# MarcoPolo/drand

Hardware: AMD Instinct MI355X
Metric: verified beacons/sec (whole node), quicknet G1 scheme (higher is better)
Workload: dtype u32 (Fp products on 14x28-bit limbs, 64-bit MAD accumulators; 12x32-bit Montgomery storage); 1 GPU; bls-unchained-g1-rfc9380 batch verify of a 1048576-round chain, 1048576 rounds per GPU; scheme=bls-unchained-g1-rfc9380, rounds_total=1048576, rounds_per_gpu=1048576, global_batch=1048576, parallelism=round-shard x1

## Files before the change

drand_amd/_lib.py:

```python
import ctypes
import os

HERE = os.path.dirname(os.path.abspath(__file__))
LIB_PATH = os.environ.get("DRANDHIP_LIB") or os.path.join(HERE, "libdrandhip.so")

DH_OK = 0
DH_EINVAL = -1
DH_EDEVICE = -2
DH_ENOMEM = -3
DH_EKEY = -4
DH_ERECOVER = -5
DH_EBUSY = -6
DH_EABANDONED = -7
DH_ECORRUPT = -8
DH_ENOBEACON = -9
DH_NODE_CHECKED = 2
DH_DEFERRED = 1
DH_STORE_TRIMMED, DH_STORE_UNTRIMMED, DH_STORE_AUTO = 0, 1, 2

_c = ctypes
_P = _c.c_void_p
SIGNATURES = {
    "dh_init": (_c.c_int, [_c.c_uint32]),
    "dh_shutdown": (None, []),
    "dh_scheme_from_name": (_c.c_int, [_c.c_char_p]),
    "dh_sig_len": (_c.c_int, [_c.c_int]),
    "dh_key_len": (_c.c_int, [_c.c_int]),
    "dh_verify_batch": (_c.c_int, [_c.c_int, _c.c_char_p, _c.c_size_t, _P, _P, _c.c_size_t, _P, _c.c_size_t, _P,
                                   _c.c_size_t, _P, _P, _c.c_uint64]),
    "dh_verify_batch_device": (_c.c_int, [_c.c_int, _c.c_char_p, _c.c_size_t, _P, _P, _c.c_size_t, _P, _c.c_size_t,
                                          _P, _c.c_size_t, _P, _P, _c.c_uint64, _P, _P]),
    "dh_verify_beacon": (_c.c_int, [_c.c_int, _c.c_char_p, _c.c_size_t, _c.c_uint64, _c.c_char_p, _c.c_size_t,
                                    _c.c_char_p, _c.c_size_t]),
    "dh_verify_recovered": (_c.c_int, [_c.c_int, _c.c_char_p, _c.c_size_t, _c.c_char_p, _c.c_char_p, _c.c_size_t]),
    "dh_verify_recovered_batch": (_c.c_int, [_c.c_int, _c.c_char_p, _c.c_size_t, _P, _P, _c.c_size_t, _c.c_size_t, _P,
                                             _c.c_uint64]),
    "dh_digest_batch": (_c.c_int, [_c.c_int, _P, _P, _c.c_size_t, _P, _c.c_size_t, _P]),
    "dh_randomness_batch": (_c.c_int, [_c.c_int, _P, _c.c_size_t, _c.c_size_t, _P]),
    "dh_recover_batch": (_c.c_int, [_c.c_int, _c.c_char_p, _c.c_int, _c.c_int, _P, _P, _P, _c.c_size_t, _P, _P]),
    "dh_verify_partials_batch": (_c.c_int, [_c.c_int, _c.c_char_p, _c.c_int, _c.c_int, _P, _P, _P, _c.c_size_t, _P]),
    "dh_bls_verify_batch": (_c.c_int, [_c.c_int, _P, _c.c_size_t, _P, _P, _P, _P, _c.c_size_t, _c.c_size_t, _P, _P,
                                       _c.c_uint64, _P]),
    "dh_identity_hash_batch": (_c.c_int, [_c.c_int, _P, _c.c_size_t, _P]),
    "dh_identity_verify_batch": (_c.c_int, [_c.c_int, _P, _P, _c.c_size_t, _c.c_size_t, _P]),
    "dh_schnorr_verify_batch": (_c.c_int, [_c.c_int, _P, _c.c_size_t, _P, _P, _P, _P, _c.c_size_t, _c.c_size_t, _P, _P]),
    "dh_schnorr_sig_len": (_c.c_int, [_c.c_int]),
    "dh_sign_batch": (_c.c_int, [_c.c_int, _c.c_char_p, _P, _P, _c.c_size_t, _P, _c.c_size_t, _P]),
    "dh_public_key": (_c.c_int, [_c.c_int, _c.c_char_p, _P]),
    "dh_partial_bytes": (_c.c_int, [_c.c_int]),
    "dh_set_split": (_c.c_int, [_c.c_uint64, _c.c_int]),
    "dh_hash_to_curve": (_c.c_int, [_c.c_int, _P, _P, _c.c_size_t, _c.c_char_p, _c.c_size_t, _P]),
    "dh_g1_round_prep_debug": (_c.c_int, [_P, _P, _c.c_size_t, _P, _P, _P]),
    "dh_batch_begin": (_c.c_int, [_c.c_int, _c.c_char_p, _c.c_size_t, _P, _P, _c.c_size_t, _P, _c.c_size_t, _P,
                                  _c.c_size_t, _P, _P, _c.c_uint64, _P, _c.POINTER(_P), _P]),
    "dh_batch_check": (_c.c_int, [_P, _P, _c.c_size_t, _P]),
    "dh_batch_stream": (_P, [_P]),
    "dh_check_partials": (_c.c_int, [_c.c_int, _c.c_char_p, _c.c_size_t, _P, _c.c_size_t, _c.POINTER(_c.c_int)]),
    "dh_batch_finish": (_c.c_int, [_P, _c.c_int, _P]),
    "dh_bolt_index": (_c.c_int, [_P, _c.c_size_t, _P, _P, _c.c_size_t, _P]),
    "dh_store_open_bolt": (_c.c_int, [_P, _c.c_size_t, _c.POINTER(_P)]),
    "dh_store_stat": (_c.c_int, [_P, _P]),
    "dh_store_columns_device": (_c.c_int, [_P, _c.c_uint64, _c.c_uint64, _c.c_size_t, _P, _P, _P, _c.c_size_t, _P, _P,
                                           _c.c_size_t, _P, _P]),
    "dh_store_check_past": (_c.c_int, [_P, _c.c_int, _c.c_char_p, _c.c_size_t, _c.c_uint64, _c.c_size_t, _c.c_uint64, _P,
                                       _c.c_size_t, _P, _P, _P]),
    "dh_store_close": (None, [_P]),
    "dh_store_open_bolt_format": (_c.c_int, [_P, _c.c_size_t, _c.c_int, _c.POINTER(_P)]),
    "dh_store_format_stat": (_c.c_int, [_P, _P]),
    "dh_store_beacons_device": (_c.c_int, [_P, _c.c_uint64, _c.c_uint64, _c.c_size_t, _c.c_size_t, _P, _P, _P, _P, _P, _P,
                                           _c.c_size_t, _P, _P, _c.c_size_t, _P, _P]),
    "dh_store_deferred": (_c.c_int, [_P, _c.c_uint64, _c.c_uint64, _P, _c.c_size_t, _P]),
    "dh_profile": (_c.c_int, [_c.c_int]),
    "dh_profile_read": (_c.c_int, [_c.c_char_p, _c.c_size_t]),
    "dh_last_error_string": (_c.c_char_p, []),
    "dh_version": (_c.c_char_p, []),
}

_lib = None


class LibraryMissing(RuntimeError):
    pass


def load():
    global _lib
    if _lib is not None:
        return _lib
    if not os.path.exists(LIB_PATH):
        raise LibraryMissing(
            "libdrandhip.so not found at %s: build it with `make -C drand_amd` or __graft_entry__.build()" % LIB_PATH)
    lib = ctypes.CDLL(LIB_PATH)
    for name, (res, args) in SIGNATURES.items():
        fn = getattr(lib, name)
        fn.restype = res
        fn.argtypes = args
    _lib = lib
    return lib


def last_error():
    return (load().dh_last_error_string() or b"").decode()
```

drand_amd/csrc/drandhip.cpp:

```cpp
#include <hip/hip_runtime.h>
#include <stdarg.h>
#include <stdio.h>
#include <string.h>
#include <sys/random.h>

#include <algorithm>
#include <atomic>
#include <condition_variable>
#include <cmath>
#include <functional>
#include <map>
#include <memory>
#include <chrono>
#include <mutex>
#include <string>
#include <thread>
#include <vector>

#include "../../include/drandhip.h"
#include "bolt.hpp"
#include "kernels.hpp"

namespace {

// ... 356 lines not shown
    v[12] ^= (uint64_t)done;
    if (last) v[14] = ~v[14];
    for (int r = 0; r < 12; r++) {
      const uint8_t* s = sigma[r];
      auto G = [&](int a, int b, int c, int d, uint64_t x, uint64_t y) {
        v[a] = v[a] + v[b] + x; v[d] = ror(v[d] ^ v[a], 32);
        v[c] = v[c] + v[d];     v[b] = ror(v[b] ^ v[c], 24);
        v[a] = v[a] + v[b] + y; v[d] = ror(v[d] ^ v[a], 16);
        v[c] = v[c] + v[d];     v[b] = ror(v[b] ^ v[c], 63);
      };
      G(0, 4, 8, 12, m[s[0]], m[s[1]]);
      G(1, 5, 9, 13, m[s[2]], m[s[3]]);
      G(2, 6, 10, 14, m[s[4]], m[s[5]]);
      G(3, 7, 11, 15, m[s[6]], m[s[7]]);
      G(0, 5, 10, 15, m[s[8]], m[s[9]]);
      G(1, 6, 11, 12, m[s[10]], m[s[11]]);
      G(2, 7, 8, 13, m[s[12]], m[s[13]]);
      G(3, 4, 9, 14, m[s[14]], m[s[15]]);
    }
    for (int i = 0; i < 8; i++) h[i] ^= v[i] ^ v[i + 8];
  }
  for (int i = 0; i < 32; i++) out[i] = (uint8_t)(h[i / 8] >> (8 * (i % 8)));
}

uint64_t splitmix64(uint64_t& x) {
  uint64_t z = (x += 0x9e3779b97f4a7c15ULL);
  z = (z ^ (z >> 30)) * 0xbf58476d1ce4e5b9ULL;
  z = (z ^ (z >> 27)) * 0x94d049bb133111ebULL;
  return z ^ (z >> 31);
}

int make_seed(uint64_t seed, uint32_t words[8]) {
  if (seed == 0) {
    uint8_t b[32];
    size_t got = 0;
    while (got < sizeof b) {
      ssize_t r = getrandom(b + got, sizeof b - got, 0);
      if (r <= 0) return fail(DH_EDEVICE, "getrandom failed");
      got += (size_t)r;
    }
    memcpy(words, b, 32);
  } else {
    uint64_t x = seed;
    for (int i = 0; i < 4; i++) {
      uint64_t v = splitmix64(x);
      words[2 * i] = (uint32_t)(v >> 32);
      words[2 * i + 1] = (uint32_t)v;
    }
  }
  return DH_OK;
}

static bool window_ok(int sbits, int c) {
  const int nw = (sbits + 1 + c - 1) / c, t = sbits - c * (nw - 1);
  return t >= c - 4;
}
dh::msm_geom geom_for(size_t gsize, int parts = 1) {
  const size_t npts = (size_t)parts * gsize;
  const int sbits = parts == 4 ? 31 : parts == 2 ? 63 : 127;
  int lg = 0;
  while (((size_t)1 << (lg + 1)) <= npts) lg++;
  int c = std::max(3, std::min(16, lg - 2));
  static const int c_env = [] {
    const char* e = getenv("DRANDHIP_MSM_C");
    const int v = e ? atoi(e) : 0;
    return v >= 4 && v <= 16 ? v : 0;
  }();
  if (c_env && gsize >= 65536) c = c_env;
  while (c > 3 && !window_ok(sbits, c)) c--;
  dh::msm_geom g;
  g.gsize = (uint32_t)gsize;
  g.c = c;
  g.nwin = (sbits + 1 + c - 1) / c;
  g.nbuck = (1u << (c - 1)) + 1;
  uint32_t nseg = std::max(1u, std::min(8192u, g.nbuck / 8));
  g.nseg = nseg;
  g.seglen = (g.nbuck - 1 + nseg - 1) / nseg;
  g.halves = (uint32_t)parts;
  g.half_stride = 0;
  return g;
}

static void fit_segments(dh::msm_geom& g, size_t ngroups, size_t nsets) {
  const size_t rows = std::max<size_t>(1, nsets * ngroups * (size_t)g.nwin);
  const size_t want = ((size_t)1 << 18) / rows + 1;
  size_t nseg = std::max<size_t>(1, std::min<size_t>({want, (size_t)g.nseg}));
  if (nseg > 512) nseg &= ~(size_t)511;
  g.nseg = (uint32_t)nseg;
  g.seglen = (g.nbuck - 1 + g.nseg - 1) / g.nseg;
}

constexpr size_t JAC_WORDS_G1 = 36, JAC_WORDS_G2 = 72;

struct prof_entry {
  uint64_t count = 0;
  double ms = 0;
  unsigned long long prods = 0;
};
struct prof_pending {
  const char* name;
  hipEvent_t a, b;
  unsigned long long prods;
};
struct profiler {
  std::mutex mu;
  std::atomic<bool> on{false};
  std::vector<std::pair<std::string, prof_entry>> table;
  std::vector<prof_pending> pending;
  void add(const char* name, float ms, unsigned long long prods = 0) {
    std::lock_guard<std::mutex> lk(mu);
    add_locked(name, ms, prods);
  }
  void add_locked(const char* name, float ms, unsigned long long prods) {
    for (auto& e : table)
      if (e.first == name) {
        e.second.count++;
        e.second.ms += ms;
        e.second.prods += prods;
        return;
      }
    prof_entry pe;
    pe.count = 1;
    pe.ms = ms;
    pe.prods = prods;
    table.emplace_back(name, pe);
  }
};
profiler g_prof;

static void prof_settle(const char* name, hipEvent_t a, hipEvent_t b, unsigned long long prods) {
  float ms = 0;
  if (hipEventSynchronize(b) == hipSuccess && hipEventElapsedTime(&ms, a, b) == hipSuccess) g_prof.add(name, ms, prods);
  (void)hipEventDestroy(a);
  (void)hipEventDestroy(b);
}
static void prof_drain_locked() {
  for (auto& r : g_prof.pending) {
    float ms = 0;
    if (hipEventSynchronize(r.b) == hipSuccess && hipEventElapsedTime(&ms, r.a, r.b) == hipSuccess)
      g_prof.add_locked(r.name, ms, r.prods);
    (void)hipEventDestroy(r.a);
    (void)hipEventDestroy(r.b);
  }
  g_prof.pending.clear();
}

#ifdef DH_COUNT_PRODUCTS
static unsigned long long count_take_all() {
  unsigned long long t = 0, v = 0;
  hipError_t (*take[])(unsigned long long*) = {dh::count_take_prep, dh::count_take_msm, dh::count_take_check,
                                               dh::count_take_sign, dh::count_take_recover, dh::count_take_vm,
                                               dh::count_take_schnorr};
  for (auto f : take)
    if (f(&v) == hipSuccess) t += v;
  return t;
}
#endif

struct timed_launches {
  struct rec {
    const char* name;
    hipEvent_t a, b;
    unsigned long long prods;
  };
  std::vector<rec> recs;
  hipStream_t st;
  explicit timed_launches(hipStream_t s) : st(s) {}
// ... 146 lines not shown
  if (gsize == m_prev && m_prev > 4096) return dense ? 256 : 1024;
  if (dense && (gsize == 256 || gsize == 32)) return gsize == 256 ? 32 : 4;
  if (dense && gsize == 4) return 1;
  const double f = (double)nfail / (double)ngroups;
  const double per_group = nfail == ngroups ? 5.0 : -std::log1p(-f);
  const double faults = std::max((double)nfail, per_group * (double)ngroups);
  const double density = std::min(1.0, faults / (double)std::max<size_t>(m_next, 1));
  size_t g = 1;
  descent_cost((double)m_next, density, gsize, &g);
  return g;
}

static bool prep_sync() {
  static const bool v = [] {
    const char* e = getenv("DRANDHIP_PREP_SYNC");
    return !(e && e[0] == '0');
  }();
  return v;
}

static bool skip_level0() {
  static const bool v = [] {
    const char* e = getenv("DRANDHIP_SKIP_LEVEL0");
    return !(e && e[0] == '0');
  }();
  return v;
}


enum verify_mode {
  VM_FULL = 0,
  VM_BEGIN = 1,
  VM_FINISH = 2,
  VM_FINISH_PASS = 3
};

struct prep_gate {
  hipEvent_t wait = nullptr;
  hipEvent_t done = nullptr;
  std::function<void()> recorded;
};

static bool subgroup_batch_on() {
  static const bool v = [] {
    const char* e = getenv("DRANDHIP_SUBGROUP_BATCH");
    return !(e && e[0] == '0');
  }();
  return v;
}
static size_t sub_batch_min() {
  static const size_t v = [] {
    const char* e = getenv("DRANDHIP_SUB_BATCH_MIN");
    const long long d = e ? atoll(e) : 0;
    return (size_t)(d >= 1 ? d : 131072);
  }();
  return v;
}
constexpr size_t SUB_BATCH_MIN_G2_DEFAULT = 393216;
static size_t sub_batch_min_g2() {
  static const size_t v = [] {
    const char* e = getenv("DRANDHIP_SUB_BATCH_MIN_G2");
    const long long d = e ? atoll(e) : 0;
    return (size_t)(d >= 1 ? d : SUB_BATCH_MIN_G2_DEFAULT);
  }();
  return v;
}
static int sub_backoff() {
  static const int v = [] {
    const char* e = getenv("DRANDHIP_SUB_BACKOFF");
    const long d = e ? atol(e) : -1;
    return (int)(d >= 0 && d <= 1 << 20 ? d : 15);
  }();
  return v;
}

static bool g1_ride_on() {
  static const bool v = [] {
    const char* e = getenv("DRANDHIP_G1_RIDE");
    return !(e && e[0] == '0');
  }();
  return v;
}

static int msm_workspace(worker* w, const dh::msm_geom& g, size_t m, size_t ngroups, size_t jw, dh::msm_ws& ws,
                         bool sub = false, bool g2 = false) {
  const size_t nk = ngroups * g.nwin * (size_t)g.nbuck;
  HIP_TRY(w->cnt.ensure(nk * 4));
  HIP_TRY(w->off.ensure((nk + 1) * 4));
  HIP_TRY(w->scan_tmp.ensure(((nk + 4095) / 4096 + 1) * 4));
  HIP_TRY(w->list.ensure(dh::msm_entries(g, m) * 4));
  HIP_TRY(w->buckets.ensure(2 * nk * jw * 4));
  const size_t segs_bytes = 2 * ngroups * g.nwin * g.nseg * jw * 4;
  HIP_TRY(w->segs.ensure(2 * segs_bytes));
  HIP_TRY(w->outA.ensure(ngroups * jw * 4));
  HIP_TRY(w->outB.ensure(ngroups * jw * 4));
  HIP_TRY(w->out2.ensure(2 * ngroups * jw * 4));
  HIP_TRY(w->pass.ensure(ngroups));
  HIP_TRY(w->part.ensure(dh::msm_part_bytes(dh::msm_entries(g, m), jw, 2)));
  HIP_TRY(w->meta.ensure(dh::msm_meta_bytes(dh::msm_entries(g, m))));
  ws = dh::msm_ws{w->cnt.as<uint32_t>(), w->off.as<uint32_t>(), w->scan_tmp.as<uint32_t>(), w->list.as<uint32_t>(),
                  w->buckets.as<uint32_t>(), w->segs.as<uint32_t>(), w->out2.as<uint32_t>(), w->part.as<uint32_t>(),
                  w->meta.as<uint32_t>(), 0, (uint32_t*)((uint8_t*)w->segs.p + segs_bytes)};
  if (sub) {
    HIP_TRY(w->sub_tmp.ensure(dh::sub_batch_tmp_bytes(g2, g)));
    HIP_TRY(w->sub_pass.ensure(8));
    ws.sub = w->sub_tmp.as<uint32_t>();
  }
  return DH_OK;
}

int verify_core(worker* w, int scheme, const uint8_t* pk, size_t pk_len, const uint64_t* d_rounds, const uint8_t* d_sigs,
                size_t sig_stride, const uint8_t* d_prevs, size_t prev_stride, const uint32_t* d_prev_lens, size_t n,
                uint8_t* d_verdict, uint8_t* d_rand, uint64_t seed, hipStream_t st, uint64_t* stats,
                const uint8_t* d_msgs32 = nullptr, int mode = VM_FULL, prep_gate* gate = nullptr) {
  const bool g2 = sig_on_g2(scheme);
  const int sig_len = g2 ? 96 : 48, key_len = g2 ? 48 : 96;
  if ((int)pk_len != key_len) return fail(DH_EINVAL, "public key must be %d bytes for scheme %d", key_len, scheme);
  if (sig_stride < (size_t)sig_len || sig_stride % 4) return fail(DH_EINVAL, "bad signature stride %zu", sig_stride);
  if (stats) memset(stats, 0, 4 * sizeof(uint64_t));
  if (n == 0) return DH_OK;
  const size_t jw = g2 ? JAC_WORDS_G2 : JAC_WORDS_G1;
  const size_t aw = jw * 2 / 3;
  const size_t wsw = g2 ? 96 : 48;

  timed_launches T(st);
  const bool one_stream = mode == VM_BEGIN && w->begin_one_stream;
  bool presorted = false;
  const bool skip0 = mode == VM_FULL && w->fault_density > 1.0 / 2000 && n > 4096 && skip_level0();
  const bool sub_eligible = mode == VM_FULL && !skip0 && n >= 2 && n >= (g2 ? sub_batch_min_g2() : sub_batch_min()) &&
                            subgroup_batch_on();
  const bool sub_batch = sub_eligible && w->sub_fused_left == 0;
  if (sub_eligible && w->sub_fused_left > 0) w->sub_fused_left--;
  const int parts = g2 && !sub_batch ? 4 : 2;
  if (n >= ((size_t)1 << 31) / parts) return fail(DH_EINVAL, "batch too large");
  dh::msm_geom g0{};
  dh::msm_ws ws0{};
  if (mode <= VM_BEGIN) {
    int rc = ensure_key(w, g2, pk, pk_len, st);
    if (rc) return rc;

    HIP_TRY(w->status.ensure(n));
    HIP_TRY(w->sig_aff.ensure(n * aw * 4));
    HIP_TRY(w->q_pts.ensure(n * jw * 4));
    HIP_TRY(w->scal.ensure(n * 16));
    HIP_TRY(w->entries.ensure(n * 4));
    uint32_t seedw[8];
    rc = make_seed(seed, seedw);
    if (rc) return rc;
    uint32_t* d_seed = (uint32_t*)((uint8_t*)w->key_ok.p + 32);
    presorted = w->tail && st == w->stream && !skip0 && !one_stream;
    if (presorted) {
      hipStream_t ts = w->tail;
      HIP_TRY(hipMemcpyAsync(d_seed, seedw, 32, hipMemcpyHostToDevice, ts));
      HIP_TRY(dh::launch_scalars(d_seed, n, nullptr, w->scal.as<uint4>(), parts, ts));
      HIP_TRY(dh::launch_iota(w->entries.as<uint32_t>(), n, ts));
      g0 = geom_for(n, parts);
      g0.half_stride = (uint32_t)n;
      rc = msm_workspace(w, g0, n, 1, wsw, ws0, sub_batch, g2);
      if (rc) return rc;
      HIP_TRY(dh::launch_msm_sort(g0, w->entries.as<uint32_t>(), nullptr, nullptr, n, 1, w->scal.as<uint4>(), ws0, ts));
    }
    if (gate && gate->wait) HIP_TRY(hipStreamWaitEvent(st, gate->wait, 0));
    const int chained = scheme == DH_SCHEME_CHAINED && d_prevs && !d_msgs32 ? 1 : 0;
    if (!g2 && sub_batch && g1_ride_on()) {
      HIP_TRY(T.run(d_msgs32 ? "k_prep_msg32<fp>" : "k_prep_msg<fp>", [&] {
        return dh::launch_round_g1_ride(d_rounds, d_prevs, prev_stride, d_prev_lens, d_msgs32, n, chained, dst_id(scheme), d_sigs,
                                        sig_stride, w->status.as<uint8_t>(), w->sig_aff.as<uint32_t>(), d_rand,
                                        w->q_pts.as<uint32_t>(), st);
      }));
    } else {
      HIP_TRY(T.run(g2 ? "k_prep_sig<fp2>" : "k_prep_sig<fp>", [&] {
        return dh::launch_prep(g2, d_sigs, sig_stride, n, w->status.as<uint8_t>(), w->sig_aff.as<uint32_t>(), d_rand, st,
                               sub_batch);
      }));
      HIP_TRY(w->h2c_tmp.ensure(dh::hash_tmp_bytes(g2, n)));
      HIP_TRY(T.run(d_msgs32 ? (g2 ? "k_prep_msg32<fp2>" : "k_prep_msg32<fp>") : (g2 ? "k_prep_msg<fp2>" : "k_prep_msg<fp>"), [&] {
        return dh::launch_hash(g2, d_rounds, d_prevs, prev_stride, d_prev_lens, d_msgs32, n, chained, dst_id(scheme),
                               w->status.as<uint8_t>(), w->q_pts.as<uint32_t>(), w->h2c_tmp.as<uint32_t>(), st);
      }));
    }
    if (!presorted) {
      HIP_TRY(hipMemcpyAsync(d_seed, seedw, 32, hipMemcpyHostToDevice, st));
      HIP_TRY(dh::launch_scalars(d_seed, n, w->status.as<uint8_t>(), w->scal.as<uint4>(), parts, st));
    }
    HIP_TRY(w->s28.ensure(parts * n * (g2 ? 64 : 32) * 4));
    HIP_TRY(w->q28.ensure(parts * n * (g2 ? 64 : 32) * 4));
    HIP_TRY(T.run(g2 ? "k_msm_prep28<fp2>" : "k_msm_prep28<fp>", [&] {
      return dh::launch_msm_prep28(g2, n, w->status.as<uint8_t>(), w->sig_aff.as<uint32_t>(), w->q_pts.as<uint32_t>(),
                                   w->s28.as<uint32_t>(), w->q28.as<uint32_t>(), st, 3, parts);
    }));
    HIP_TRY(hipMemsetAsync(d_verdict, 0, n, st));
    if (gate) {
      HIP_TRY(hipEventRecord(gate->done, st));
      gate->recorded();
    }
    if (mode == VM_FULL && w->tail && st == w->stream && !one_stream && prep_sync()) HIP_TRY(hipStreamSynchronize(st));
    if (!presorted) HIP_TRY(dh::launch_iota(w->entries.as<uint32_t>(), n, st));
  }
  if (w->tail && st == w->stream && !one_stream) {
    if (mode <= VM_BEGIN) {
      HIP_TRY(hipEventRecord(w->handoff, st));
      HIP_TRY(hipStreamWaitEvent(w->tail, w->handoff, 0));
    }
    st = w->tail;
    T.st = st;
  }

  size_t m = n;
  static const char* const msm_names[8] = {"msm_level0", "msm_bisect1", "msm_bisect2", "msm_bisect3",
                                           "msm_bisect4", "msm_bisect5", "msm_bisect6", "msm_bisect7+"};
  static const char* const chk_names[8] = {"k_group_check_level0", "k_group_check_bisect1", "k_group_check_bisect2",
                                           "k_group_check_bisect3", "k_group_check_bisect4", "k_group_check_bisect5",
                                           "k_group_check_bisect6", "k_group_check_bisect7+"};
  const std::vector<size_t>& fixed = fixed_ladder();
  size_t gsize = skip0 ? (fixed.empty() ? 256 : fixed[0]) : n;
  int level = skip0 ? 1 : 0;
  if (mode == VM_BEGIN && n < 2) {
    HIP_TRY(w->outA.ensure(jw * 4));
    HIP_TRY(w->outB.ensure(jw * 4));
    HIP_TRY(hipMemsetAsync(w->outA.p, 0, jw * 4, st));
    HIP_TRY(hipMemsetAsync(w->outB.p, 0, jw * 4, st));
    return DH_OK;
  }
  while (m > 0 && gsize > 1) {
    gsize = std::min(gsize, m);
    dh::msm_geom g = geom_for(gsize, parts);
    g.half_stride = (uint32_t)n;
    const size_t ngroups = (m + gsize - 1) / gsize;
    fit_segments(g, ngroups, 2);
    const bool pre = level == 0 && presorted;
    dh::msm_ws ws{};
    if (pre) {
      ws = ws0;
    } else {
      const int rc = msm_workspace(w, g, m, ngroups, wsw, ws, level == 0 && sub_batch, g2);
      if (rc) return rc;
    }
    if (!(level == 0 && mode >= VM_FINISH)) {
      HIP_TRY(T.run(msm_names[std::min(level, 7)], [&] {
        return dh::launch_msm28(g2, pre ? g0 : g, w->entries.as<uint32_t>(), m, ngroups, w->scal.as<uint4>(),
                                w->s28.as<uint32_t>(), w->q28.as<uint32_t>(), ws, w->outA.as<uint32_t>(),
                                w->outB.as<uint32_t>(), st, w->status.as<uint8_t>(), pre);
      }));
    }
    if (level == 0 && mode == VM_BEGIN) return DH_OK;
    if (level == 0 && mode == VM_FINISH_PASS) {
      HIP_TRY(hipMemsetAsync(w->pass.p, 1, 1, st));
    } else {
      HIP_TRY(T.run(chk_names[std::min(level, 7)], [&] {
        return group_check(w, g2, w->outA.as<uint32_t>(), w->outB.as<uint32_t>(), ngroups, w->key_cur, w->pass.as<uint8_t>(),
                           st, w->key_cur + 48);
      }));
    }
    const bool sub0 = level == 0 && sub_batch;
    if (sub0) {
      HIP_TRY(T.run("k_sub_batch_level0", [&] {
        return dh::launch_sub_batch(g2, pre ? g0 : g, ws, w->pass.as<uint8_t>(), w->sub_pass.as<uint8_t>(), st);
      }));
    }
    HIP_TRY(dh::launch_mark_groups(w->entries.as<uint32_t>(), m, gsize, w->pass.as<uint8_t>(), w->status.as<uint8_t>(),
                                   d_verdict, st));
    HIP_TRY(w->cflags.ensure(ngroups * 4));
    HIP_TRY(w->crank.ensure((ngroups + 1) * 4));
    HIP_TRY(w->cscan.ensure(((ngroups + 4095) / 4096 + 1) * 4));
    HIP_TRY(w->entries_alt.ensure(m * 4));
    HIP_TRY(dh::launch_compact_failing(w->entries.as<uint32_t>(), m, gsize, ngroups, w->pass.as<uint8_t>(),
                                       w->cflags.as<uint32_t>(), w->crank.as<uint32_t>(), w->cscan.as<uint32_t>(),
                                       w->entries_alt.as<uint32_t>(), st));
    uint32_t nfail32 = 0;
    uint8_t last_pass = 1;
    HIP_TRY(hipMemcpyAsync(&nfail32, w->crank.as<uint32_t>() + ngroups, 4, hipMemcpyDeviceToHost, st));
    HIP_TRY(hipMemcpyAsync(&last_pass, w->pass.as<uint8_t>() + ngroups - 1, 1, hipMemcpyDeviceToHost, st));
    uint8_t sub_pass = 1;
    if (sub0) HIP_TRY(hipMemcpyAsync(&sub_pass, w->sub_pass.p, 1, hipMemcpyDeviceToHost, st));
    HIP_TRY(hipStreamSynchronize(st));
    if (!sub_pass) {
      HIP_TRY(w->sub_bad.ensure(n));
      HIP_TRY(T.run("k_sub_exact", [&] {
        return dh::launch_sub_exact(g2, n, w->status.as<uint8_t>(), w->sig_aff.as<uint32_t>(), w->sub_bad.as<uint8_t>(),
                                    (uint32_t*)((uint8_t*)w->sub_pass.p + 4), st);
      }));
      uint32_t nbad = 0;
      HIP_TRY(hipMemcpyAsync(&nbad, (uint8_t*)w->sub_pass.p + 4, 4, hipMemcpyDeviceToHost, st));
      HIP_TRY(hipStreamSynchronize(st));
      if ((double)nbad * 2000 > (double)n) w->sub_fused_left = sub_backoff();
    }
    level++;
    const size_t nfail = nfail32;
    if (stats) stats[1] += nfail;
    if (level == 1 && nfail == 0) w->fault_density = 0;
    if (level == 2) {
      const double f = (double)nfail / (double)ngroups;
      w->fault_density = (f >= 1.0 ? 5.0 : -std::log1p(-f)) / (double)gsize;
    }
    if (nfail == 0) {
      m = 0;
      break;
    }
    std::swap(w->entries, w->entries_alt);
    const size_t m_prev = m;
    m = nfail * gsize - (last_pass ? 0 : ngroups * gsize - m_prev);
    gsize = fixed.empty() ? next_group_size(gsize, ngroups, nfail, m_prev, m, w->fault_density)
                          : (size_t)(level - 1 < (int)fixed.size() ? fixed[level - 1] : 1);
  }
  if (m > 0) {
    HIP_TRY(T.run("k_leaf_check", [&] {
      return leaf_check(w, g2, w->entries.as<uint32_t>(), m, w->sig_aff.as<uint32_t>(), w->q_pts.as<uint32_t>(),
                        w->key_cur, w->status.as<uint8_t>(), d_verdict, st, w->key_cur + 48);
    }));
    if (stats) stats[2] = m;
  }
  if (stats) {
    w->h_verdict.resize(n);
    HIP_TRY(hipMemcpyAsync(w->h_verdict.data(), d_verdict, n, hipMemcpyDeviceToHost, st));
  }
  HIP_TRY(hipStreamSynchronize(st));
  if (stats) {
    stats[0] = (uint64_t)level;
    size_t ok = 0;
    for (uint8_t v : w->h_verdict) ok += v ? 1 : 0;
    stats[3] = n - ok;
  }
  return DH_OK;
}

static size_t small_batch_max() {
  static const size_t v = [] {
    const char* e = getenv("DRANDHIP_SMALL_N");
    return e ? (size_t)atol(e) : (size_t)64;
  }();
  return v;
}

int verify_small(worker* w, int scheme, const uint8_t* pk, size_t pk_len, const uint64_t* d_rounds, const uint8_t* d_sigs,
                 size_t sig_stride, const uint8_t* d_prevs, size_t prev_stride, const uint32_t* d_prev_lens, size_t n,
                 uint8_t* d_verdict, uint8_t* d_rand, const uint8_t* d_msgs32, hipStream_t st, bool lens_checked) {
  const bool g2 = sig_on_g2(scheme);
  const int sig_len = g2 ? 96 : 48, key_len = g2 ? 48 : 96;
  if ((int)pk_len != key_len) return fail(DH_EINVAL, "public key must be %d bytes for scheme %d", key_len, scheme);
  if (sig_stride < (size_t)sig_len || sig_stride % 4) return fail(DH_EINVAL, "bad signature stride %zu", sig_stride);
  if (n == 0) return DH_OK;
  int rc = ensure_key(w, g2, pk, pk_len, st);
  if (rc) return rc;
  const size_t jw = g2 ? JAC_WORDS_G2 : JAC_WORDS_G1;
  const size_t aw = jw * 2 / 3;
  HIP_TRY(w->status.ensure(n));
  HIP_TRY(w->sig_aff.ensure(n * aw * 4));
  HIP_TRY(w->q_pts.ensure(n * jw * 4));
  HIP_TRY(w->entries.ensure(n * 4));
  HIP_TRY(w->h2c_tmp.ensure(dh::hash_small_tmp_bytes(g2, n)));
  const bool chained = scheme == DH_SCHEME_CHAINED && d_prevs && !d_msgs32;
  const bool fork = w->tail && !(chained && d_prev_lens && !lens_checked);
  HIP_TRY(w->sub_bad.ensure(n));
  hipStream_t hs = fork ? w->tail : st;
  if (fork) {
    HIP_TRY(hipEventRecord(w->handoff, st));
    HIP_TRY(hipStreamWaitEvent(hs, w->handoff, 0));
  }
  timed_launches T(st), TH(hs);
  HIP_TRY(T.run(g2 ? "k_dec_sig_small<fp2>" : "k_dec_sig_small<fp>", [&] {
    return dh::launch_dec_sig(g2, d_sigs, sig_stride, n, w->status.as<uint8_t>(), w->sig_aff.as<uint32_t>(), d_rand, st);
  }));
  if (fork) HIP_TRY(hipEventRecord(w->ev_dec, st));
  HIP_TRY(TH.run(d_msgs32 ? (g2 ? "k_prep_msg32<fp2>" : "k_prep_msg32<fp>") : (g2 ? "k_prep_msg<fp2>" : "k_prep_msg<fp>"), [&] {
    return dh::launch_hash_small(g2, d_rounds, d_prevs, prev_stride, d_prev_lens, d_msgs32, n, chained ? 1 : 0, dst_id(scheme),
                                 fork ? nullptr : w->status.as<uint8_t>(), w->q_pts.as<uint32_t>(), w->h2c_tmp.as<uint32_t>(), hs);
  }));
  HIP_TRY(T.run(g2 ? "k_sub_sig_small<fp2>" : "k_sub_sig_small<fp>", [&] {
// ... 1354 lines not shown
                          chained ? w->in_prevs.as<uint8_t>() : nullptr, prev_stride,
                          chained && prev_lens ? w->in_prev_lens.as<uint32_t>() : nullptr, nullptr, n, chained ? 1 : 0,
                          dst_id(scheme), w->in_sigs.as<uint8_t>(), w->q_pts.as<uint32_t>(), w->h2c_tmp.as<uint32_t>(), st));
  HIP_TRY(hipMemcpyAsync(sigs_out, w->in_sigs.p, n * sl, hipMemcpyDeviceToHost, st));
  HIP_TRY(hipStreamSynchronize(st));
  return DH_OK;
}

int dh_hash_to_curve(int group, const uint8_t* msgs, const uint32_t* msg_off, size_t n, const uint8_t* dst, size_t dst_len,
                     uint8_t* out) {
  if (group != 1 && group != 2) return fail(DH_EINVAL, "group must be 1 (G1) or 2 (G2)");
  if (!msg_off || !out || (n && !msgs) || !dst || dst_len == 0 || dst_len > 255)
    return fail(DH_EINVAL, "bad hash_to_curve arguments (DST must be 1..255 bytes)");
  if (n == 0) return DH_OK;
  size_t maxm = 0;
  for (size_t i = 0; i < n; i++) {
    if (msg_off[i + 1] < msg_off[i]) return fail(DH_EINVAL, "msg_off must be non-decreasing");
    maxm = std::max<size_t>(maxm, msg_off[i + 1] - msg_off[i]);
  }
  const size_t total = msg_off[n] - msg_off[0];
  const size_t stride = (64 + maxm + 4 + dst_len + 63) & ~(size_t)63;
  const size_t outlen = group == 1 ? 48 : 96;
  std::vector<uint32_t> off(n + 1);
  for (size_t i = 0; i <= n; i++) off[i] = msg_off[i] - msg_off[0];
  lease L;
  if (L.rc) return L.rc;
  worker* w = L.w;
  int rc = set_device_and_stream(w);
  if (rc) return rc;
  hipStream_t st = w->stream;
  HIP_TRY(w->in_sigs.ensure(total + 4));
  HIP_TRY(w->in_prev_lens.ensure((n + 1) * 4));
  HIP_TRY(w->key_raw.ensure(256));
  HIP_TRY(w->h2c_tmp.ensure(n * stride));
  HIP_TRY(w->out_rand.ensure(n * outlen));
  if (total) HIP_TRY(hipMemcpyAsync(w->in_sigs.p, msgs + msg_off[0], total, hipMemcpyHostToDevice, st));
  HIP_TRY(hipMemcpyAsync(w->in_prev_lens.p, off.data(), (n + 1) * 4, hipMemcpyHostToDevice, st));
  HIP_TRY(hipMemcpyAsync(w->key_raw.p, dst, dst_len, hipMemcpyHostToDevice, st));
  HIP_TRY(dh::launch_h2c_generic(group == 2, w->in_sigs.as<uint8_t>(), w->in_prev_lens.as<uint32_t>(), n,
                                 w->key_raw.as<uint8_t>(), (uint32_t)dst_len, w->h2c_tmp.as<uint8_t>(), stride,
                                 w->out_rand.as<uint8_t>(), st));
  HIP_TRY(hipMemcpyAsync(out, w->out_rand.p, n * outlen, hipMemcpyDeviceToHost, st));
  HIP_TRY(hipStreamSynchronize(st));
  return DH_OK;
}

static bool fp_bytes_canonical(const uint8_t* b) {
  static const uint8_t P[48] = {0x1a, 0x01, 0x11, 0xea, 0x39, 0x7f, 0xe6, 0x9a, 0x4b, 0x1b, 0xa7, 0xb6, 0x43, 0x4b, 0xac, 0xd7,
                                0x64, 0x77, 0x4b, 0x84, 0xf3, 0x85, 0x12, 0xbf, 0x67, 0x30, 0xd2, 0xa0, 0xf6, 0xb0, 0xf6, 0x24,
                                0x1e, 0xab, 0xff, 0xfe, 0xb1, 0x53, 0xff, 0xff, 0xb9, 0xfe, 0xff, 0xff, 0xff, 0xff, 0xaa, 0xab};
  return memcmp(b, P, 48) < 0;
}

int dh_g1_round_prep_debug(const uint8_t* us, const uint8_t* sigs, size_t n, uint8_t* status_out, uint8_t* sig_out,
                           uint8_t* hash_out) {
  if (!us || !sigs || !status_out || !sig_out || !hash_out) return fail(DH_EINVAL, "null argument");
  if (n == 0) return DH_OK;
  for (size_t i = 0; i < 2 * n; i++)
    if (!fp_bytes_canonical(us + 48 * i)) return fail(DH_EINVAL, "field element %zu is not below p", i);
  lease L;
  if (L.rc) return L.rc;
  worker* w = L.w;
  int rc = set_device_and_stream(w);
  if (rc) return rc;
  hipStream_t st = w->stream;
  HIP_TRY(w->in_prevs.ensure(n * 96));
  HIP_TRY(w->in_sigs.ensure(n * 48));
  HIP_TRY(w->status.ensure(n));
  HIP_TRY(w->sig_aff.ensure(n * JAC_WORDS_G1 * 2 / 3 * 4));
  HIP_TRY(w->q_pts.ensure(n * JAC_WORDS_G1 * 4));
  HIP_TRY(w->out_rand.ensure(n * 192));
  HIP_TRY(hipMemcpyAsync(w->in_prevs.p, us, n * 96, hipMemcpyHostToDevice, st));
  HIP_TRY(hipMemcpyAsync(w->in_sigs.p, sigs, n * 48, hipMemcpyHostToDevice, st));
  uint8_t* out = w->out_rand.as<uint8_t>();
  HIP_TRY(dh::launch_round_g1_ride_debug(w->in_prevs.as<uint8_t>(), w->in_sigs.as<uint8_t>(), n, w->status.as<uint8_t>(),
                                         w->sig_aff.as<uint32_t>(), w->q_pts.as<uint32_t>(), out, out + n * 96, st));
  HIP_TRY(hipMemcpyAsync(status_out, w->status.p, n, hipMemcpyDeviceToHost, st));
  HIP_TRY(hipMemcpyAsync(sig_out, out, n * 96, hipMemcpyDeviceToHost, st));
  HIP_TRY(hipMemcpyAsync(hash_out, out + n * 96, n * 96, hipMemcpyDeviceToHost, st));
  HIP_TRY(hipStreamSynchronize(st));
  return DH_OK;
}

int dh_public_key(int scheme, const uint8_t* sk32, uint8_t* key_out) {
  int kl = dh_key_len(scheme);
  if (kl < 0) return kl;
  if (!sk32 || !key_out) return fail(DH_EINVAL, "null argument");
  lease L;
  if (L.rc) return L.rc;
  worker* w = L.w;
  int rc = set_device_and_stream(w);
  if (rc) return rc;
  hipStream_t st = w->stream;
  uint32_t skw[8];
  sk_words(sk32, skw);
  HIP_TRY(w->key_ok.ensure(64));
  HIP_TRY(w->key_raw.ensure(96));
  HIP_TRY(hipMemcpyAsync(w->key_ok.p, skw, 32, hipMemcpyHostToDevice, st));
  HIP_TRY(dh::launch_pubkey(kl == 96, w->key_ok.as<uint32_t>(), w->key_raw.as<uint8_t>(), st));
  HIP_TRY(hipMemcpyAsync(key_out, w->key_raw.p, kl, hipMemcpyDeviceToHost, st));
  HIP_TRY(hipStreamSynchronize(st));
  return DH_OK;
}

}


static size_t store_max_bytes() {
  const char* e = getenv("DRANDHIP_STORE_MAX_BYTES");
  const long long v = e ? atoll(e) : 0;
  return v > 0 ? (size_t)v : (size_t)16 << 30;
}

struct prof_wall {
  const char* name;
  std::chrono::steady_clock::time_point t0;
  explicit prof_wall(const char* n) : name(n), t0(std::chrono::steady_clock::now()) {}
  ~prof_wall() {
    if (g_prof.on.load(std::memory_order_relaxed))
      g_prof.add(name, std::chrono::duration<float, std::milli>(std::chrono::steady_clock::now() - t0).count());
  }
};

struct dh_store {
  std::mutex mu;
  std::atomic<bool> retire{false};
  bool dead = false;
  size_t len = 0;
  uint32_t page_size = 0;
  uint64_t stat[6] = {0, 0, 0, 0, 0, 0};
  int format = DH_STORE_TRIMMED;
  uint64_t jstat[3] = {0, 0, 0};
  std::vector<dh::bolt::leaf_json> jinfo;
  std::vector<dh::bolt::leaf_info> info;
  std::vector<uint32_t> rleaf;
  hipStream_t st = nullptr;
  dbuf d_file, d_leaves, d_info, err, cnt, base, scan_tmp, rounds, rows, lens, miss_prev, gap, moff, missing, verdict, bad;
  dbuf d_jinfo, prevs, prev_lens, defer;
  std::vector<uint8_t> h_defer;
  std::vector<uint8_t> h_bad;
  std::vector<uint64_t> h_rounds, h_missing;
  void release() {
    for (dbuf* b : {&d_file, &d_leaves, &d_info, &err, &cnt, &base, &scan_tmp, &rounds, &rows, &lens, &miss_prev, &gap, &moff,
                    &missing, &verdict, &bad, &d_jinfo, &prevs, &prev_lens, &defer})
      b->release();
    if (st) (void)hipStreamDestroy(st);
    st = nullptr;
    dead = true;
  }
};
static std::mutex g_stores_mu;
static std::vector<dh_store*> g_stores;

static void stores_shutdown() {
  std::lock_guard<std::mutex> lk(g_stores_mu);
  for (dh_store* s : g_stores) {
    if (s->mu.try_lock()) {
      s->release();
      s->mu.unlock();
    } else {
      s->retire = true;
    }
  }
}

static int store_enter(dh_store* s) {
// ... 597 lines not shown
```

drand_amd/csrc/fp28.hpp:

```cpp
#pragma once
#include "fp.hpp"

namespace dh {

struct f28 {
  uint32_t l[14];
};

#define DH_FP28_CALL_CLOBBERS                                                                                  \
  "v32", "v33", "v34", "v35", "v36", "v37", "v38", "v39", "v48", "v49", "v50", "v51", "v52", "v53", "s0", "s1", \
      "s2", "s3", "s4", "s5", "s6", "s7", "s8", "s9", "s10", "s11", "s12", "s13", "s14", "s15", "s16", "s17", "s30", \
      "s31", "vcc", "scc"

DH_DEV fp28vec f28_vec(const f28& a) {
  fp28vec v;
#pragma unroll
  for (int i = 0; i < 14; i++) v[i] = a.l[i];
  v[14] = v[15] = 0;
  return v;
}
DH_DEV f28 f28_unvec(const fp28vec& v) {
  f28 a;
#pragma unroll
  for (int i = 0; i < 14; i++) a.l[i] = v[i];
// ... 128 lines not shown
    d |= r.l[i] ^ m28::P[i];
  }
  return z == 0 || d == 0;
}

DH_DEV f28 f28_from_fp(const fp& x) {
  f28 a, c;
  m28::split<0>(a.l, x.v);
  const uint32_t k[14] = {0x80e6299u, 0x3500034u, 0xeb12856u, 0xdeb2699u, 0xc988670u, 0x4ef6697u, 0x70983e8u,
                          0xa4e6fe9u, 0x3e8a053u, 0xecf271eu, 0xc20d323u, 0x6eb6385u, 0x47f1286u, 0x00156dau};
#pragma unroll
  for (int i = 0; i < 14; i++) c.l[i] = k[i];
  return f28_mul(a, c);
}

DH_DEV fp f28_to_fp(const f28& a) {
  f28 c;
  const uint32_t k[14] = {0x002fffdu, 0x0900000u, 0xc000276u, 0x000bc40u, 0x8baebf4u, 0x5753c75u, 0x55f4898u,
                          0x7052574u, 0x7ce5853u, 0x56ec6d7u, 0x71a97a2u, 0xe4935c0u, 0xec3fa80u, 0x0015f65u};
#pragma unroll
  for (int i = 0; i < 14; i++) c.l[i] = k[i];
  const f28 r = f28_mul(a, c);
  fp o;
  m28::join(o.v, r.l);
  m28::final_sub(o.v);
  return o;
}

DH_DEV f28 f28_c(const uint32_t* c) {
  f28 r;
#pragma unroll
  for (int i = 0; i < 14; i++) r.l[i] = c[i];
  return r;
}

struct j28 {
  f28 x, y, z;
  bool inf;
};

DH_DEV f28 f28_mul_inl(const f28& a, const f28& b) {
  DH_COUNT_PROD();
  f28 r;
  m28::mont_mul(r.l, a.l, b.l);
  return r;
}
DH_DEV f28 f28_sqr_inl(const f28& a) {
  DH_COUNT_PROD();
  f28 r;
  m28::mont_sqr(r.l, a.l);
  return r;
}

template <bool INL = false>
DH_DEV j28 j28_dbl(const j28& p) {
  auto sq = [](const f28& x) { return INL ? f28_sqr_inl(x) : f28_sqr(x); };
  auto mu = [](const f28& x, const f28& y) { return INL ? f28_mul_inl(x, y) : f28_mul(x, y); };
  const f28 a = sq(p.x);
  const f28 b = sq(p.y);
  const f28 c = sq(b);
  const f28 t = sq(INL ? f28_add_nc(p.x, b) : f28_add(p.x, b));
  const f28 d = f28_lin3<8>(t, 2, a, -2, c, -2);
  const f28 e = f28_scale(a, 3);
  const f28 f = sq(e);
  j28 r;
  r.x = f28_lin<24>(f, 1, d, -2);
  const f28 m = mu(e, INL ? f28_sub_nc<kp_above(26)>(d, r.x) : f28_sub<26>(d, r.x));
  r.y = f28_lin<16>(m, 1, c, -8);
  r.z = f28_scale(mu(p.y, p.z), 2);
  r.inf = p.inf;
  return r;
}

DH_DEV j28 j28_inf() {
  j28 r;
  r.x = f28_one();
  r.y = f28_one();
#pragma unroll
  for (int i = 0; i < 14; i++) r.z.l[i] = 0;
  r.inf = true;
  return r;
}

DH_DEV j28 j28_madd(const j28& p, const f28& qx, const f28& qy) {
  if (p.inf) return j28{qx, qy, f28_one(), false};
  const f28 z1z1 = f28_sqr(p.z);
  const f28 u2 = f28_mul(qx, z1z1);
  const f28 s2 = f28_mul(f28_mul(qy, p.z), z1z1);
  const f28 h = f28_sub<26>(u2, p.x);
  const f28 rr = f28_sub<18>(s2, p.y);
  if (f28_zero(h)) {
    if (f28_zero(rr)) return j28_dbl(p);
    return j28_inf();
  }
  const f28 hh = f28_sqr(h);
  const f28 i = f28_scale(hh, 4);
  const f28 j = f28_mul(h, i);
  const f28 r2 = f28_scale(rr, 2);
  const f28 v = f28_mul(p.x, i);
  j28 r;
  r.inf = false;
  r.x = f28_lin3<6>(f28_sqr(r2), 1, j, -1, v, -2);
  const f28 m = f28_mul(r2, f28_sub<8>(v, r.x));
  r.y = f28_lin<4>(m, 1, f28_mul(p.y, j), -2);
  r.z = f28_lin3<4>(f28_sqr(f28_add(p.z, h)), 1, z1z1, -1, hh, -1);
  return r;
}

DH_DEV j28 j28_add(const j28& p, const j28& q) {
  if (p.inf) return q;
  if (q.inf) return p;
  const f28 z1z1 = f28_sqr(p.z), z2z2 = f28_sqr(q.z);
  const f28 u1 = f28_mul(p.x, z2z2), u2 = f28_mul(q.x, z1z1);
  const f28 s1 = f28_mul(f28_mul(p.y, q.z), z2z2);
  const f28 s2 = f28_mul(f28_mul(q.y, p.z), z1z1);
  const f28 h = f28_sub<2>(u2, u1);
  const f28 rr = f28_sub<2>(s2, s1);
  if (f28_zero(h)) {
    if (f28_zero(rr)) return j28_dbl(p);
    return j28_inf();
  }
  const f28 i = f28_sqr(f28_scale(h, 2));
  const f28 j = f28_mul(h, i);
  const f28 r2 = f28_scale(rr, 2);
  const f28 v = f28_mul(u1, i);
  j28 r;
  r.inf = false;
  r.x = f28_lin3<6>(f28_sqr(r2), 1, j, -1, v, -2);
  const f28 m = f28_mul(r2, f28_sub<8>(v, r.x));
  r.y = f28_lin<4>(m, 1, f28_mul(s1, j), -2);
  const f28 zz = f28_lin3<4>(f28_sqr(f28_add(p.z, q.z)), 1, z1z1, -1, z2z2, -1);
  r.z = f28_mul(zz, h);
  return r;
}

DH_DEV j28 j28_madd_fast(const j28& p, const f28& qx, const f28& qy) {
  if (p.inf) return j28{qx, qy, f28_one(), false};
  const f28 z1z1 = f28_sqr(p.z);
  const f28 u2 = f28_mul(qx, z1z1);
  const f28 s2 = f28_mul(f28_mul(qy, p.z), z1z1);
  const f28 h = f28_sub<26>(u2, p.x);
  const f28 rr = f28_sub<18>(s2, p.y);
  const f28 hh = f28_sqr(h);
  const f28 i = f28_scale(hh, 4);
  const f28 j = f28_mul(h, i);
  const f28 r2 = f28_scale(rr, 2);
  const f28 v = f28_mul(p.x, i);
  j28 r;
  r.inf = false;
  r.x = f28_lin3<6>(f28_sqr(r2), 1, j, -1, v, -2);
  const f28 m = f28_mul(r2, f28_sub<8>(v, r.x));
  r.y = f28_lin<4>(m, 1, f28_mul(p.y, j), -2);
  r.z = f28_lin3<4>(f28_sqr(f28_add(p.z, h)), 1, z1z1, -1, hh, -1);
  return r;
}
DH_DEV j28 j28_add_fast(const j28& p, const j28& q) {
  if (p.inf) return q;
  if (q.inf) return p;
  const f28 z1z1 = f28_sqr(p.z), z2z2 = f28_sqr(q.z);
  const f28 u1 = f28_mul(p.x, z2z2), u2 = f28_mul(q.x, z1z1);
  const f28 s1 = f28_mul(f28_mul(p.y, q.z), z2z2);
  const f28 s2 = f28_mul(f28_mul(q.y, p.z), z1z1);
  const f28 h = f28_sub<2>(u2, u1);
  const f28 rr = f28_sub<2>(s2, s1);
  const f28 i = f28_sqr(f28_scale(h, 2));
  const f28 j = f28_mul(h, i);
  const f28 r2 = f28_scale(rr, 2);
  const f28 v = f28_mul(u1, i);
  j28 r;
  r.inf = false;
  r.x = f28_lin3<6>(f28_sqr(r2), 1, j, -1, v, -2);
  const f28 m = f28_mul(r2, f28_sub<8>(v, r.x));
  r.y = f28_lin<4>(m, 1, f28_mul(s1, j), -2);
  const f28 zz = f28_lin3<4>(f28_sqr(f28_add(p.z, q.z)), 1, z1z1, -1, z2z2, -1);
  r.z = f28_mul(zz, h);
  return r;
}
DH_DEV bool j28_poisoned(const j28& p) { return !p.inf && f28_zero(p.z); }
DH_DEV f28 f28_neg2(const f28& y) { return f28_lin<2>(y, -1, y, 0); }

template <class LD>
DH_DEV bool g1_in_subgroup28(LD ld) {
  j28 t;
  {
    const aff<fp> p = ld();
    const f28 x = f28_from_fp(p.x), y = f28_from_fp(p.y);
    j28 acc{x, y, f28_one(), false};
#pragma unroll 1
    for (int b = 62; b >= 0; b--) {
      acc = j28_dbl<true>(acc);
      if ((cst::U_ABS >> b) & 1) acc = j28_madd(acc, x, y);
    }
    t = acc;
  }
  j28 acc = t;
#pragma unroll 1
  for (int b = 62; b >= 0; b--) {
    acc = j28_dbl<true>(acc);
    if ((cst::U_ABS >> b) & 1) acc = j28_add(acc, t);
  }
  if (acc.inf) return false;
  asm volatile("" ::: "memory");
// ... 34 lines not shown
```

drand_amd/csrc/h2c.hpp:

```cpp
#pragma once
#include "curve.hpp"
#include "sha256.hpp"
#include "fp28.hpp"

namespace dh {

DH_DEV fp fp_from_be512(const uint32_t hi[8], const uint32_t lo[8]) {
  fp h, l;
#pragma unroll
  for (int k = 0; k < 8; k++) {
    h.v[k] = hi[7 - k];
    l.v[k] = lo[7 - k];
  }
#pragma unroll
  for (int k = 8; k < 12; k++) h.v[k] = l.v[k] = 0;
  return fp_add(fp_mul(h, fp_c(cst::K256R)), fp_mul(l, fp_c(cst::R2)));
}

DH_DEV bool fp_sqrt_ratio(fp& y, const fp& u, const fp& v) {
  fp tv1 = fp_sqr(v);
  fp tv2 = fp_mul(u, v);
  tv1 = fp_mul(tv1, tv2);
  fp y1 = fp_pow_sched(tv1, cst::SCHED_SR1_C1, cst::SCHED_SR1_C1_LEN);
  y1 = fp_mul(y1, tv2);
// ... 47 lines not shown
    if (j < ISO11_XNUM_LEN) xn = f28_add(f28_mul(xn, X), f28_mul(f28_c(ISO11_XNUM_28[ISO11_XNUM_LEN - 1 - j]), zp));
    if (j < ISO11_H_LEN) {
      const f28 t = f28_mul(f28_c(ISO11_H_28[ISO11_H_LEN - 1 - j]), zp);
      h = f28_add(j > 1 ? f28_mul(h, X) : h, t);
    }
  }
  jac<fp> r;
  r.x = f28_to_fp(xn);
  r.y = f28_to_fp(f28_mul(f28_from_fp(p.y), yn));
  r.z = f28_to_fp(f28_mul(Zp, h));
  return r;
}

template <class F>
DH_DEV jac<F> swu_jac(const swu_out<F>& s) {
  jac<F> r;
  r.z = s.xd;
  r.x = f_mul(s.xn, s.xd);
  r.y = f_mul(s.y, f_mul(f_sqr(s.xd), s.xd));
  return r;
}

template <class F>
DH_DEV bool jac_add_distinct(jac<F>& r, const jac<F>& p, const jac<F>& q) {
  F z1z1 = f_sqr(p.z);
  F z2z2 = f_sqr(q.z);
  F u1 = f_mul(p.x, z2z2);
  F u2 = f_mul(q.x, z1z1);
  F s1 = f_mul(f_mul(p.y, q.z), z2z2);
  F s2 = f_mul(f_mul(q.y, p.z), z1z1);
  F h = f_sub(u2, u1);
  if (f_is_zero(h)) return false;
  F rr = f_dbl(f_sub(s2, s1));
  F i = f_sqr(f_dbl(h));
  F j = f_mul(h, i);
  F v = f_mul(u1, i);
  r.x = f_sub(f_sub(f_sqr(rr), j), f_dbl(v));
  r.y = f_sub(f_mul(rr, f_sub(v, r.x)), f_dbl(f_mul(s1, j)));
  r.z = f_mul(f_sub(f_sub(f_sqr(f_add(p.z, q.z)), z1z1), z2z2), h);
  return true;
}

DH_DEV jac<fp> h2c_g1_map(const fp& u0, const fp& u1) {
  const jac<fp> p0 = swu_jac(sswu_g1(u0));
  const jac<fp> p1 = swu_jac(sswu_g1(u1));
  jac<fp> s;
  if (jac_add_distinct(s, p0, p1)) return iso11_jac(s);
  return jac_add(iso11_jac(p0), iso11_jac(p1));
}

DH_DEV bool fp_sqrt_ride(fp& y, fp& inv_c, const fp& a, const fp& c) {
  const fp ac = fp_mul(a, c);
  const fp w = fp_pow_sched(fp_mul(ac, c), cst::SCHED_SR1_C1, cst::SCHED_SR1_C1_LEN);
  y = fp_mul(w, ac);
  const fp ic = fp_mul(fp_sqr(w), ac);
  const bool qr = fp_eq(fp_sqr(y), a);
  inv_c = fp_select(qr, ic, fp_neg(ic));
  return qr;
}

struct g1_sum_mid {
  fp n, s, a, dyd2, y0;
};
DH_DEV bool g1_sum_pre(g1_sum_mid& m, fp& c, const swu_out<fp>& p0, const swu_out<fp>& p1) {
  m.a = fp_mul(p0.xn, p1.xd);
  const fp b = fp_mul(p1.xn, p0.xd);
  const fp d = fp_mul(p0.xd, p1.xd);
  m.n = fp_sub(b, m.a);
  m.s = fp_add(b, m.a);
  c = fp_mul(m.n, d);
  m.dyd2 = fp_mul(fp_sub(p1.y, p0.y), fp_sqr(d));
  m.y0 = p0.y;
  return !fp_is_zero(m.n);
}
DH_DEV aff<fp> g1_sum_post(const g1_sum_mid& m, const fp& inv_c) {
  const fp inv_d = fp_mul(m.n, inv_c);
  const fp lam = fp_mul(m.dyd2, inv_c);
  aff<fp> r;
  r.x = fp_sub(fp_sqr(lam), fp_mul(m.s, inv_d));
  r.y = fp_sub(fp_mul(lam, fp_sub(fp_mul(m.a, inv_d), r.x)), m.y0);
  return r;
}

DH_DEV jac<fp> iso11_aff(const aff<fp>& p) {
  using namespace cst;
  const f28 X = f28_from_fp(p.x);
  f28 xn = f28_c(ISO11_XNUM_28[ISO11_XNUM_LEN - 1]);
  f28 yn = f28_c(ISO11_YNUM_28[ISO11_YNUM_LEN - 1]);
  f28 h = X;
#pragma unroll 1
  for (int j = 1; j < ISO11_YNUM_LEN; j++) {
    yn = f28_add(f28_mul(yn, X), f28_c(ISO11_YNUM_28[ISO11_YNUM_LEN - 1 - j]));
    if (j < ISO11_XNUM_LEN) xn = f28_add(f28_mul(xn, X), f28_c(ISO11_XNUM_28[ISO11_XNUM_LEN - 1 - j]));
    if (j < ISO11_H_LEN) h = f28_add(j > 1 ? f28_mul(h, X) : h, f28_c(ISO11_H_28[ISO11_H_LEN - 1 - j]));
  }
  jac<fp> r;
  r.x = f28_to_fp(xn);
  r.y = f28_to_fp(f28_mul(f28_from_fp(p.y), yn));
  r.z = f28_to_fp(h);
  return r;
}

DH_DEV jac<fp> h2c_g1_noclear(const sha_h& digest, int dst_id) {
  uint32_t b[4][8];
  xmd32<4>(b, digest, dst_id);
  return h2c_g1_map(fp_from_be512(b[0], b[1]), fp_from_be512(b[2], b[3]));
}

DH_DEV jac<fp> h2c_clear_g1(const jac<fp>& p) { return jac_add(jac_mul_uabs_j(p), p); }

DH_DEV swu_out<fp2> sswu_g2(const fp2& u) {
  const fp2 A = fp2_c(cst::SSWU2_A), B = fp2_c(cst::SSWU2_B), Z = fp2_c(cst::SSWU2_Z);
  fp2 tv1 = fp2_mul(Z, fp2_sqr(u));
  fp2 tv2 = fp2_add(fp2_sqr(tv1), tv1);
  fp2 tv3 = fp2_mul(B, fp2_add(tv2, fp2_one()));
  fp2 tv4 = fp2_mul(A, fp2_select(fp2_is_zero(tv2), Z, fp2_neg(tv2)));
  fp2 t2 = fp2_sqr(tv3);
  fp2 tv6 = fp2_sqr(tv4);
  t2 = fp2_add(t2, fp2_mul(A, tv6));
  t2 = fp2_mul(t2, tv3);
  tv6 = fp2_mul(tv6, tv4);
  t2 = fp2_add(t2, fp2_mul(B, tv6));
  fp2 x = fp2_mul(tv1, tv3);
  fp2 y1;
  bool gx1_sq = fp2_sqrt_ratio_cm(y1, t2, tv6);
  fp2 y = fp2_mul(fp2_mul(tv1, u), y1);
  x = fp2_select(gx1_sq, tv3, x);
  y = fp2_select(gx1_sq, y1, y);
  bool e1 = fp2_sgn0(u) == fp2_sgn0(y);
  y = fp2_select(e1, y, fp2_neg(y));
  return {x, tv4, y};
}

DH_DEV jac<fp2> iso3_jac(const jac<fp2>& p) {
  using namespace cst;
  static_assert(ISO3_XNUM_LEN == ISO3_YNUM_LEN && ISO3_H_LEN == 2, "iso3_jac: degrees 3, 3 and 1");
  const fp2 D = fp2_sqr(p.z);
  fp2 xn = fp2_c(ISO3_XNUM[ISO3_XNUM_LEN - 1]);
  fp2 yn = fp2_c(ISO3_YNUM[ISO3_YNUM_LEN - 1]);
  fp2 zp = D;
#pragma unroll 1
  for (int j = 1; j < ISO3_YNUM_LEN; j++) {
    if (j > 1) zp = fp2_mul(zp, D);
    yn = fp2_add(fp2_mul(yn, p.x), fp2_mul(fp2_c(ISO3_YNUM[ISO3_YNUM_LEN - 1 - j]), zp));
    xn = fp2_add(fp2_mul(xn, p.x), fp2_mul(fp2_c(ISO3_XNUM[ISO3_XNUM_LEN - 1 - j]), zp));
  }
  jac<fp2> r;
  r.x = xn;
  r.y = fp2_mul(p.y, yn);
  r.z = fp2_mul(p.z, fp2_add(p.x, fp2_mul(fp2_c(ISO3_H[0]), D)));
  return r;
}
DH_DEV jac<fp2> iso3_jac_lean(const jac<fp2>& p) { return iso3_jac(p); }

DH_DEV jac<fp2> h2c_g2_map(const fp2& u0, const fp2& u1) {
  const jac<fp2> p0 = swu_jac(sswu_g2(u0));
  const jac<fp2> p1 = swu_jac(sswu_g2(u1));
  jac<fp2> s;
  if (jac_add_distinct(s, p0, p1)) return iso3_jac(s);
  return jac_add(iso3_jac(p0), iso3_jac(p1));
}

DH_DEV jac<fp2> h2c_g2_noclear(const sha_h& digest, int dst_id) {
  uint32_t b[8][8];
  xmd32<8>(b, digest, dst_id);
  return h2c_g2_map({fp_from_be512(b[0], b[1]), fp_from_be512(b[2], b[3])}, {fp_from_be512(b[4], b[5]), fp_from_be512(b[6], b[7])});
// ... 27 lines not shown
```

drand_amd/csrc/k_msm.hip:

```cpp
#include "kcommon.hpp"

namespace dh {

DH_DEV uint32_t scalar_digit(const uint4& s, int bit, int c) {
  const uint32_t w[4] = {s.x, s.y, s.z, s.w};
  int wi = bit >> 5, sh = bit & 31;
  uint64_t lo = wi < 4 ? w[wi] : 0;
  uint64_t hi = wi + 1 < 4 ? w[wi + 1] : 0;
  uint64_t v = (lo | (hi << 32)) >> sh;
  return (uint32_t)v & ((1u << c) - 1);
}

constexpr uint32_t NEG_BIT = 0x80000000u;
DH_DEV int32_t signed_digit(const uint4& s, int w, const msm_geom& g, uint32_t& carry) {
  const uint32_t v = scalar_digit(s, w * g.c, g.c) + carry;
  const uint32_t half = 1u << (g.c - 1);
  if (w + 1 < g.nwin && v >= half) {
    carry = 1;
    return (int32_t)v - (int32_t)(1u << g.c);
  }
  carry = 0;
  return (int32_t)v;
}

DH_DEV size_t entry_group(const uint32_t* grp, size_t e, uint32_t gsize) { return grp ? grp[e] : e / gsize; }

DH_DEV uint4 half_scalar(const uint4& s, uint32_t h, const msm_geom& g) {
  if (g.halves == 1) return s;
  if (g.halves == 4) return make_uint4(h == 0 ? s.x : h == 1 ? s.y : h == 2 ? s.z : s.w, 0, 0, 0);
  return h ? make_uint4(s.z, s.w, 0, 0) : make_uint4(s.x, s.y, 0, 0);
}
DH_DEV uint32_t round_of(uint32_t idx, uint32_t nround) { return idx < nround ? idx : idx % nround; }

__global__ void k_msm_hist(const uint32_t* __restrict__ pidx, const uint32_t* __restrict__ sidx,
                           const uint32_t* __restrict__ grp, size_t m, const uint4* __restrict__ scal, msm_geom g,
                           uint32_t* __restrict__ cnt) {
  size_t e = gtid();
  if (e >= m) return;
  const uint4 s = scal[sidx ? sidx[e] : pidx[e]];
  const size_t gi = entry_group(grp, e, g.gsize);
  for (uint32_t h = 0; h < g.halves; h++) {
    const uint4 sh = half_scalar(s, h, g);
    uint32_t carry = 0;
    for (int w = 0; w < g.nwin; w++) {
      const int32_t d = signed_digit(sh, w, g, carry);
      if (d) atomicAdd(&cnt[(gi * g.nwin + w) * g.nbuck + (uint32_t)(d < 0 ? -d : d)], 1u);
    }
  }
}

__global__ void k_msm_scatter(const uint32_t* __restrict__ pidx, const uint32_t* __restrict__ sidx,
                              const uint32_t* __restrict__ grp, size_t m, const uint4* __restrict__ scal, msm_geom g,
                              uint32_t* __restrict__ cursor, uint32_t* __restrict__ list) {
  size_t e = gtid();
  if (e >= m) return;
  const uint32_t idx0 = pidx[e];
  const uint4 s = scal[sidx ? sidx[e] : idx0];
  const size_t gi = entry_group(grp, e, g.gsize);
  for (uint32_t h = 0; h < g.halves; h++) {
    const uint4 sh = half_scalar(s, h, g);
    const uint32_t idx = idx0 + h * g.half_stride;
    uint32_t carry = 0;
    for (int w = 0; w < g.nwin; w++) {
      const int32_t d = signed_digit(sh, w, g, carry);
      if (d) {
        uint32_t pos = atomicAdd(&cursor[(gi * g.nwin + w) * g.nbuck + (uint32_t)(d < 0 ? -d : d)], 1u);
        list[pos] = d < 0 ? (idx | NEG_BIT) : idx;
      }
    }
  }
}

constexpr uint32_t SORT_T = 1024, SLAB_MAX = 36864;

template <bool SCATTER>
__global__ __launch_bounds__(SORT_T) void k_msm_sort_lds(const uint32_t* __restrict__ pidx, const uint32_t* __restrict__ sidx,
                                                         const uint32_t* __restrict__ grp, size_t m, const uint4* __restrict__ scal,
                                                         msm_geom g, size_t nk, uint32_t tile, uint32_t slab,
                                                         uint32_t* __restrict__ gcnt, uint32_t* __restrict__ list) {
  extern __shared__ uint32_t h[];
  const size_t e0 = (size_t)blockIdx.x * tile, e1 = min(m, e0 + tile);
  const size_t rowkeys = (size_t)g.nwin * g.nbuck;
  const size_t kb = grp ? 0 : (e0 / g.gsize) * rowkeys, ke = grp ? nk : min(nk, ((e1 - 1) / g.gsize + 1) * rowkeys);
  const size_t K0 = kb + (size_t)blockIdx.y * slab;
  if (K0 >= ke) return;
  const uint32_t ns = (uint32_t)min((size_t)slab, ke - K0);
  for (uint32_t k = threadIdx.x; k < ns; k += SORT_T) h[k] = 0;
  __syncthreads();
  auto each = [&](auto&& f) {
    for (size_t e = e0 + threadIdx.x; e < e1; e += SORT_T) {
      const uint32_t idx0 = pidx[e];
      const uint4 s = scal[sidx ? sidx[e] : idx0];
      const size_t gi = entry_group(grp, e, g.gsize);
      for (uint32_t hh = 0; hh < g.halves; hh++) {
        const uint4 sh = half_scalar(s, hh, g);
        const uint32_t idx = idx0 + hh * g.half_stride;
        uint32_t carry = 0;
        for (int w = 0; w < g.nwin; w++) {
          const int32_t d = signed_digit(sh, w, g, carry);
          const size_t key = (gi * g.nwin + w) * g.nbuck + (uint32_t)(d < 0 ? -d : d);
          if (d && key - K0 < ns) f((uint32_t)(key - K0), d < 0 ? (idx | NEG_BIT) : idx);
        }
      }
    }
  };
  each([&](uint32_t k, uint32_t) { atomicAdd(&h[k], 1u); });
  __syncthreads();
  if constexpr (!SCATTER) {
    for (uint32_t k = threadIdx.x; k < ns; k += SORT_T)
      if (h[k]) atomicAdd(&gcnt[K0 + k], h[k]);
  } else {
    for (uint32_t k = threadIdx.x; k < ns; k += SORT_T)
      if (h[k]) h[k] = atomicAdd(&gcnt[K0 + k], h[k]);
    __syncthreads();
    each([&](uint32_t k, uint32_t v) { list[atomicAdd(&h[k], 1u)] = v; });
  }
}

constexpr int SCAN_T = 256, SCAN_I = 16, SCAN_B = SCAN_T * SCAN_I;

__global__ __launch_bounds__(SCAN_T) void k_scan_reduce(const uint32_t* __restrict__ in, size_t n,
                                                        uint32_t* __restrict__ block_sums) {
  __shared__ uint32_t sh[SCAN_T];
  size_t base = (size_t)blockIdx.x * SCAN_B + threadIdx.x * SCAN_I;
  uint32_t s = 0;
  for (int k = 0; k < SCAN_I; k++)
    if (base + k < n) s += in[base + k];
  sh[threadIdx.x] = s;
  __syncthreads();
  for (int off = SCAN_T / 2; off > 0; off >>= 1) {
    if (threadIdx.x < off) sh[threadIdx.x] += sh[threadIdx.x + off];
    __syncthreads();
  }
  if (threadIdx.x == 0) block_sums[blockIdx.x] = sh[0];
}

__global__ __launch_bounds__(SCAN_T) void k_scan_small(uint32_t* __restrict__ a, size_t n, uint32_t* __restrict__ total) {
  __shared__ uint32_t sh[SCAN_T];
  uint32_t v[SCAN_I];
  size_t base = threadIdx.x * SCAN_I;
  uint32_t s = 0;
  for (int k = 0; k < SCAN_I; k++) {
    v[k] = base + k < n ? a[base + k] : 0;
    s += v[k];
  }
  sh[threadIdx.x] = s;
  __syncthreads();
  for (int off = 1; off < SCAN_T; off <<= 1) {
    uint32_t t = threadIdx.x >= off ? sh[threadIdx.x - off] : 0;
    __syncthreads();
    sh[threadIdx.x] += t;
    __syncthreads();
  }
  uint32_t run = sh[threadIdx.x] - s;
  for (int k = 0; k < SCAN_I; k++) {
    if (base + k < n) a[base + k] = run;
    run += v[k];
  }
  if (threadIdx.x == SCAN_T - 1 && total) *total = sh[SCAN_T - 1];
}

__global__ __launch_bounds__(SCAN_T) void k_scan_final(const uint32_t* __restrict__ in, size_t n,
                                                       const uint32_t* __restrict__ block_off, uint32_t* __restrict__ out) {
  __shared__ uint32_t sh[SCAN_T];
  size_t base = (size_t)blockIdx.x * SCAN_B + threadIdx.x * SCAN_I;
  uint32_t v[SCAN_I];
  uint32_t s = 0;
  for (int k = 0; k < SCAN_I; k++) {
    v[k] = base + k < n ? in[base + k] : 0;
    s += v[k];
  }
  sh[threadIdx.x] = s;
  __syncthreads();
  for (int off = 1; off < SCAN_T; off <<= 1) {
    uint32_t t = threadIdx.x >= off ? sh[threadIdx.x - off] : 0;
    __syncthreads();
    sh[threadIdx.x] += t;
    __syncthreads();
  }
  uint32_t run = block_off[blockIdx.x] + sh[threadIdx.x] - s;
  for (int k = 0; k < SCAN_I; k++) {
    if (base + k < n) out[base + k] = run;
    run += v[k];
  }
}

constexpr uint32_t NO_KEY = 0xffffffffu;

template <class F>
__global__ __launch_bounds__(64) void k_sum_partials(const uint32_t* __restrict__ parts, size_t k, size_t rec_words,
                                                     uint32_t* __restrict__ outA, uint32_t* __restrict__ outB,
                                                     uint8_t* __restrict__ flag) {
  const int t = threadIdx.x;
  constexpr size_t JW = 3 * npw<F>::N;
  if (t == 2) {
    uint32_t any = 0;
    for (size_t i = 0; i < k; i++) any |= parts[i * rec_words + 2 * JW];
    if (flag) flag[0] = any ? 1 : 0;
  }
  if (t > 1) return;
  jac<F> acc = jac_inf<F>();
  for (size_t i = 0; i < k; i++) acc = jac_add(acc, ld_jac_aos<F>(parts + i * rec_words, t));
  st_jac_aos<F>(t ? outB : outA, 0, acc);
}

hipError_t launch_sum_partials(int sig_g2, const uint32_t* parts, size_t k, size_t rec_words, uint32_t* outA, uint32_t* outB,
                               uint8_t* flag, hipStream_t st) {
  if (sig_g2) hipLaunchKernelGGL(k_sum_partials<fp2>, dim3(1), dim3(64), 0, st, parts, k, rec_words, outA, outB, flag);
  else hipLaunchKernelGGL(k_sum_partials<fp>, dim3(1), dim3(64), 0, st, parts, k, rec_words, outA, outB, flag);
  return hipGetLastError();
}

__global__ void k_node_mark(size_t n, uint8_t* __restrict__ res, const uint8_t* __restrict__ status,
                            uint8_t* __restrict__ verdict) {
  const size_t i = gtid();
  const uint8_t r = res[0] ? 2 : (res[1] == 1 ? 1 : 0);
  if (i == 0) res[2] = r;
  if (i < n && r == 1) verdict[i] = status[i] == DEC_OK ? 1 : 0;
}

hipError_t launch_node_mark(size_t n, uint8_t* res, const uint8_t* status, uint8_t* verdict, hipStream_t st) {
  hipLaunchKernelGGL(k_node_mark, dim3(nblk(n ? n : 1, 256)), dim3(256), 0, st, n, res, status, verdict);
  return hipGetLastError();
}

__global__ void k_mark_groups(const uint32_t* __restrict__ entries, size_t m, size_t gsize, const uint8_t* __restrict__ pass,
                              const uint8_t* __restrict__ status, uint8_t* __restrict__ verdict) {
  size_t e = gtid();
  if (e >= m) return;
  uint32_t i = entries[e];
  if (pass[e / gsize]) verdict[i] = status[i] == DEC_OK ? 1 : 0;
}

__global__ void k_iota(uint32_t* __restrict__ v, size_t n) {
  size_t i = gtid();
  if (i < n) v[i] = (uint32_t)i;
}


hipError_t launch_iota(uint32_t* v, size_t n, hipStream_t st) {
  if (!n) return hipSuccess;
  hipLaunchKernelGGL(k_iota, dim3(nblk(n, 256)), dim3(256), 0, st, v, n);
  return hipGetLastError();
}


hipError_t launch_scan(const uint32_t* cnt, size_t nk, uint32_t* off, uint32_t* tmp, hipStream_t st) {
  size_t nb = (nk + SCAN_B - 1) / SCAN_B;
  if (nb > (size_t)SCAN_B) return hipErrorInvalidValue;
  hipLaunchKernelGGL(k_scan_reduce, dim3((unsigned)nb), dim3(SCAN_T), 0, st, cnt, nk, tmp);
  hipLaunchKernelGGL(k_scan_small, dim3(1), dim3(SCAN_T), 0, st, tmp, nb, off + nk);
  hipLaunchKernelGGL(k_scan_final, dim3((unsigned)nb), dim3(SCAN_T), 0, st, cnt, nk, tmp, off);
  return hipGetLastError();
}


hipError_t launch_msm_sort(const msm_geom& g, const uint32_t* pidx, const uint32_t* sidx, const uint32_t* grp, size_t m,
                           size_t ngroups, const uint4* scal, msm_ws& ws, hipStream_t st) {
  size_t nk = ngroups * g.nwin * (size_t)g.nbuck;
  ws.max_entries = msm_entries(g, m);
  hipError_t e = hipMemsetAsync(ws.cnt, 0, nk * sizeof(uint32_t), st);
  if (e != hipSuccess) return e;
  static const bool global_env = [] {
    const char* v = getenv("DRANDHIP_SORT_GLOBAL");
    return v && atoi(v) == 1;
  }();
  const bool global_sort = global_env || (grp && nk > 16 * (size_t)SLAB_MAX);
  dim3 grid;
  uint32_t tile = 0, slab = 0;
  if (m && !global_sort) {
    static const size_t density = [] {
      const char* v = getenv("DRANDHIP_SORT_DENSITY");
      const long d = v ? atol(v) : 0;
      return (size_t)(d >= 1 && d <= 256 ? d : 8);
    }();
    const size_t digits = (size_t)g.halves * g.nwin, rowkeys = (size_t)g.nwin * g.nbuck;
    static const size_t slab_max = [] {
      const char* v = getenv("DRANDHIP_SORT_SLAB");
      const long d = v ? atol(v) : 0;
      return (size_t)(d >= 1024 && d <= SLAB_MAX ? d : SLAB_MAX);
    }();
    static const hipError_t lds_attr = [] {
      hipError_t a = hipFuncSetAttribute((const void*)k_msm_sort_lds<false>, hipFuncAttributeMaxDynamicSharedMemorySize, SLAB_MAX * 4);
      hipError_t b = hipFuncSetAttribute((const void*)k_msm_sort_lds<true>, hipFuncAttributeMaxDynamicSharedMemorySize, SLAB_MAX * 4);
      return a != hipSuccess ? a : b;
    }();
    if (lds_attr != hipSuccess) return lds_attr;
    const size_t t = std::min(m, std::max<size_t>(SORT_T, density * std::min<size_t>(nk, slab_max) / digits));
    const size_t span = grp ? nk : std::min(nk, std::min<size_t>(ngroups, (t - 1) / g.gsize + 2) * rowkeys);
    const size_t nslab = (span + slab_max - 1) / slab_max;
    tile = (uint32_t)t;
    slab = (uint32_t)((span + nslab - 1) / nslab);
    grid = dim3((unsigned)((m + t - 1) / t), (unsigned)nslab);
  }
  if (m && global_sort) hipLaunchKernelGGL(k_msm_hist, dim3(nblk(m, 256)), dim3(256), 0, st, pidx, sidx, grp, m, scal, g, ws.cnt);
  if (m && !global_sort)
    hipLaunchKernelGGL(k_msm_sort_lds<false>, grid, dim3(SORT_T), slab * 4, st, pidx, sidx, grp, m, scal, g, nk, tile, slab, ws.cnt, ws.list);
  if ((e = launch_scan(ws.cnt, nk, ws.off, ws.scan_tmp, st)) != hipSuccess) return e;
  if ((e = hipMemcpyAsync(ws.cnt, ws.off, nk * sizeof(uint32_t), hipMemcpyDeviceToDevice, st)) != hipSuccess) return e;
  if (m && global_sort)
    hipLaunchKernelGGL(k_msm_scatter, dim3(nblk(m, 256)), dim3(256), 0, st, pidx, sidx, grp, m, scal, g, ws.cnt, ws.list);
  if (m && !global_sort)
    hipLaunchKernelGGL(k_msm_sort_lds<true>, grid, dim3(SORT_T), slab * 4, st, pidx, sidx, grp, m, scal, g, nk, tile, slab, ws.cnt, ws.list);
  return hipGetLastError();
}

constexpr int W28 = 16;
DH_DEV f28 ld28(const uint32_t* p) {
  const uint4* q = (const uint4*)p;
  f28 a;
#pragma unroll
  for (int i = 0; i < 4; i++) {
    const uint4 t = q[i];
    a.l[4 * i] = t.x;
    a.l[4 * i + 1] = t.y;
    if (4 * i + 2 < 14) a.l[4 * i + 2] = t.z;
    if (4 * i + 3 < 14) a.l[4 * i + 3] = t.w;
  }
  return a;
}
DH_DEV void st28(uint32_t* p, const f28& a) {
  uint4* q = (uint4*)p;
#pragma unroll
  for (int i = 0; i < 4; i++)
    q[i] = make_uint4(a.l[4 * i], a.l[4 * i + 1], 4 * i + 2 < 14 ? a.l[4 * i + 2] : 0u, 4 * i + 3 < 14 ? a.l[4 * i + 3] : 0u);
}
DH_DEV void ld28(f28& a, const uint32_t* p) { a = ld28(p); }
DH_DEV void st28(uint32_t* p, const f28& a, int) { st28(p, a); }
DH_DEV void ld28(f228& a, const uint32_t* p) {
  a.c0 = ld28(p);
  a.c1 = ld28(p + W28);
}
DH_DEV void st28(uint32_t* p, const f228& a, int) {
  st28(p, a.c0);
  st28(p + W28, a.c1);
}
DH_DEV bool z_all_zero(const f28& z) {
  uint32_t nz = 0;
#pragma unroll
  for (int k = 0; k < 14; k++) nz |= z.l[k];
  return nz == 0;
}
DH_DEV bool z_all_zero(const f228& z) { return z_all_zero(z.c0) && z_all_zero(z.c1); }
DH_DEV void set_zero(f28& z) {
#pragma unroll
  for (int k = 0; k < 14; k++) z.l[k] = 0;
}
DH_DEV void set_zero(f228& z) {
  set_zero(z.c0);
  set_zero(z.c1);
}

struct c28_g1 {
  static constexpr int OCC = 2;
  static constexpr bool IS_G2 = false;
  static constexpr int PARTS = 2;
  static constexpr size_t LCAP = 32;
  using E = f28;
  using P = j28;
  using F = fp;
  static constexpr int EW = W28;
  DH_DEV static P inf() { return j28_inf(); }
  DH_DEV static P madd_fast(const P& a, const E& x, const E& y) { return j28_madd_fast(a, x, y); }
  DH_DEV static P madd(const P& a, const E& x, const E& y) { return j28_madd(a, x, y); }
  DH_DEV static P add_fast(const P& a, const P& b) { return j28_add_fast(a, b); }
  DH_DEV static P add(const P& a, const P& b) { return j28_add(a, b); }
  template <bool EXACT>
  DH_DEV static P add_mem(const P& a, const uint32_t* q) {
    j28 b;
    b.x = ld28(q);
    b.y = ld28(q + W28);
    b.z = ld28(q + 2 * W28);
    b.inf = z_all_zero(b.z);
    return EXACT ? j28_add(a, b) : j28_add_fast(a, b);
  }
  template <bool EXACT>
  DH_DEV static P addx(const P& a, const P& b) { return EXACT ? j28_add(a, b) : j28_add_fast(a, b); }
  DH_DEV static P dbl(const P& a) { return j28_dbl(a); }
  DH_DEV static bool poisoned(const P& a) { return j28_poisoned(a); }
  DH_DEV static E neg(const E& y) { return f28_neg2(y); }
  DH_DEV static fp out(const E& a) { return f28_to_fp(a); }
  DH_DEV static E in(const fp& a) { return f28_from_fp(a); }
  DH_DEV static E mulr(const E& a, const E& b) { return f28_mul(a, b); }
  DH_DEV static E sqrr(const E& a) { return f28_sqr(a); }
  DH_DEV static E one() { return f28_one(); }
  DH_DEV static E inv(const E& a) { return f28_from_fp(fp_inv_vt(f28_to_fp(a))); }
  DH_DEV static bool is_zero(const fp& a) { return fp_is_zero(a); }
  DH_DEV static E endo_x(const E& x);
  DH_DEV static E endo_y(const E& y) { return y; }
};
struct c28_g2 {
  static constexpr int OCC = 1;
  static constexpr bool IS_G2 = true;
  static constexpr int PARTS = 4;
  static constexpr size_t LCAP = 64;
  using E = f228;
  using P = j228;
  using F = fp2;
  static constexpr int EW = 2 * W28;
  DH_DEV static P inf() { return j228_inf(); }
  DH_DEV static P madd_fast(const P& a, const E& x, const E& y) { return j228_madd<false, true>(a, x, y); }
  DH_DEV static P madd(const P& a, const E& x, const E& y) { return j228_madd<true>(a, x, y); }
  DH_DEV static P add_fast(const P& a, const P& b) { return j228_add<false>(a, b); }
  DH_DEV static P add(const P& a, const P& b) { return j228_add<true>(a, b); }
  template <bool EXACT>
  DH_DEV static P add_mem(const P& a, const uint32_t* q) {
    f228 z;
    ld28(z, q + 2 * EW);
    return j228_add_ld<EXACT>(a, z_all_zero(z), [&](int k) { f228 c; ld28(c, q + k * EW); return c; });
  }
  template <bool EXACT>
  DH_DEV static P addx(const P& a, const P& b) { return j228_add<EXACT>(a, b); }
  DH_DEV static P dbl(const P& a) { return j228_dbl(a); }
  DH_DEV static bool poisoned(const P& a) { return j228_poisoned(a); }
  DH_DEV static E neg(const E& y) { return f2_neg3(y); }
  DH_DEV static fp2 out(const E& a) { return f2_to_fp2(a); }
  DH_DEV static E in(const fp2& a) { return f2_from_fp2(a); }
  DH_DEV static E mulr(const E& a, const E& b) { return f2_red(f2_mul(a, b)); }
  DH_DEV static E sqrr(const E& a) { return f2_red(f2_sqr<2>(a)); }
  DH_DEV static E one() { return f2_one(); }
  DH_DEV static E inv(const E& a) { return f2_from_fp2(fp2_inv_vt(f2_to_fp2(a))); }
  DH_DEV static bool is_zero(const fp2& a) { return fp2_is_zero(a); }
  DH_DEV static E endo_x(const E& x) { return f2_red(f2_mul(f2_conj(x), f2_c28(PSI_X28))); }
  DH_DEV static E endo_y(const E& y) { return f2_red(f2_mul(f2_conj(y), f2_c28(PSI_Y28))); }
  DH_DEV static E psi2_x(const E& x) { return f2_red({f28_mul(x.c0, f28_c(PSI2_X28)), f28_mul(x.c1, f28_c(PSI2_X28))}); }
  DH_DEV static E psi2_y(const E& y) { return f2_red({f28_mul(y.c0, f28_c(PSI2_Y28)), f28_mul(y.c1, f28_c(PSI2_Y28))}); }
};

template <class C>
DH_DEV typename C::P ldj28(const uint32_t* base, size_t i) {
  const uint32_t* p = base + (size_t)3 * C::EW * i;
  typename C::P r;
  ld28(r.x, p);
  ld28(r.y, p + C::EW);
  ld28(r.z, p + 2 * C::EW);
  r.inf = z_all_zero(r.z);
  return r;
}
template <class C>
DH_DEV void stj28(uint32_t* base, size_t i, const typename C::P& a) {
  uint32_t* p = base + (size_t)3 * C::EW * i;
  st28(p, a.x, 0);
  st28(p + C::EW, a.y, 0);
  typename C::E z = a.z;
  if (a.inf) set_zero(z);
  st28(p + 2 * C::EW, z, 0);
}

__device__ __constant__ uint32_t BETA28[14] = {0xa75929au, 0x681b798u, 0x22a3e9du, 0xabc02bfu, 0x4e5bb45u, 0x55e6e7eu, 0x4814117u,
                                               0x6d04f1bu, 0xae3387du, 0x54acb0cu, 0x0a4c74bu, 0x56138b5u, 0xb64e066u, 0x00076f2u};

DH_DEV f28 c28_g1::endo_x(const f28& x) { return f28_mul(x, f28_c(BETA28)); }

constexpr uint32_t PREP28_KMAX = 16;
template <class C>
DH_DEV void prep28_images(uint32_t* __restrict__ out, size_t n, size_t i, const typename C::E& x, const typename C::E& y,
                          uint32_t parts) {
  constexpr int EW = C::EW;
  st28(out + 2 * EW * (n + i), C::endo_x(x), 0);
  st28(out + 2 * EW * (n + i) + EW, C::endo_y(y), 0);
  if constexpr (C::PARTS == 4) {
    if (parts != 4) return;
    const typename C::E x2 = C::psi2_x(x), y2 = C::psi2_y(y);
    st28(out + 2 * EW * (2 * n + i), x2, 0);
    st28(out + 2 * EW * (2 * n + i) + EW, y2, 0);
    st28(out + 2 * EW * (3 * n + i), C::endo_x(x2), 0);
    st28(out + 2 * EW * (3 * n + i) + EW, C::endo_y(y2), 0);
  }
}
static uint32_t prep28_k(size_t n) {
  uint32_t k = 1;
  while (k < PREP28_KMAX && n / (2 * k) >= 131072) k *= 2;
  return k;
}
template <class C, bool BACK>
DH_DEV typename C::E block_product_scan(typename C::E v, typename C::E* sh) {
  const int t = threadIdx.x;
#pragma unroll 1
  for (int off = 1; off < 256; off <<= 1) {
    sh[t] = v;
    __syncthreads();
    const int src = BACK ? t + off : t - off;
    const bool has = BACK ? src < 256 : src >= 0;
    typename C::E o;
    if (has) o = sh[src];
    __syncthreads();
    if (has) v = C::mulr(v, o);
  }
  return v;
}
template <class C>
__global__ __launch_bounds__(256, 2) void k_msm_prep28(size_t n, uint32_t K, uint8_t* __restrict__ status,
                                                       const uint32_t* __restrict__ sig_aff, const uint32_t* __restrict__ q_pts,
                                                       uint32_t* __restrict__ S, uint32_t* __restrict__ Q, uint32_t sets,
                                                       uint32_t parts) {
  using E = typename C::E;
  using F = typename C::F;
  constexpr int EW = C::EW, FW = npw<F>::N;
  __shared__ E sh[256];
  const size_t lo = gtid() * K;
  const size_t hi = lo < n ? min(n, lo + K) : lo;
#pragma unroll 1
  for (size_t i = lo; i < hi && (sets & 1); i++) {
    if (status[i] != DEC_OK) continue;
    const aff<F> a = ld_aff_aos<F>(sig_aff, i);
    const E x = C::in(a.x), y = C::in(a.y);
    st28(S + 2 * EW * i, x, 0);
    st28(S + 2 * EW * i + EW, y, 0);
    prep28_images<C>(S, n, i, x, y, parts);
  }
// ... 147 lines not shown
  typename C::P acc = fix_run<C, false>(part, meta, t, nch);
  if (C::poisoned(acc)) acc = fix_run<C, true>(part, meta, t, nch);
  stj28<C>(buckets, key, acc);
}

template <class C, bool EXACT>
DH_DEV void seg_run(const uint32_t* __restrict__ buckets, const uint32_t* __restrict__ off, size_t krow, size_t brow, uint32_t a,
                    uint32_t last, typename C::P& run, typename C::P& tot) {
  run = C::inf();
  tot = C::inf();
#pragma unroll 1
  for (int d = (int)last - 1; d >= (int)a; d--) {
    if (off[krow + d + 1] != off[krow + d]) run = C::template add_mem<EXACT>(run, buckets + (size_t)3 * C::EW * (brow + d));
    tot = C::template addx<EXACT>(tot, run);
  }
}
DH_DEV void lds_put(uint32_t* buf, int nthr, int i, int k0, const f28& a) {
#pragma unroll
  for (int k = 0; k < 14; k++) buf[(k0 + k) * nthr + i] = a.l[k];
}
DH_DEV void lds_get(const uint32_t* buf, int nthr, int i, int k0, f28& a) {
#pragma unroll
  for (int k = 0; k < 14; k++) a.l[k] = buf[(k0 + k) * nthr + i];
}
DH_DEV void lds_put(uint32_t* buf, int nthr, int i, int k0, const f228& a) {
  lds_put(buf, nthr, i, k0, a.c0);
  lds_put(buf, nthr, i, k0 + 14, a.c1);
}
DH_DEV void lds_get(const uint32_t* buf, int nthr, int i, int k0, f228& a) {
  lds_get(buf, nthr, i, k0, a.c0);
  lds_get(buf, nthr, i, k0 + 14, a.c1);
}
template <class C>
constexpr int lds_words() { return 3 * 14 * (C::EW / W28); }
template <class C>
DH_DEV void lds_put_pt(uint32_t* buf, int nthr, int i, const typename C::P& a) {
  constexpr int EL = 14 * (C::EW / W28);
  lds_put(buf, nthr, i, 0, a.x);
  lds_put(buf, nthr, i, EL, a.y);
  typename C::E z = a.z;
  if (a.inf) set_zero(z);
  lds_put(buf, nthr, i, 2 * EL, z);
}
template <class C>
DH_DEV typename C::P lds_get_pt(const uint32_t* buf, int nthr, int i) {
  constexpr int EL = 14 * (C::EW / W28);
  typename C::P r;
  lds_get(buf, nthr, i, 0, r.x);
  lds_get(buf, nthr, i, EL, r.y);
  lds_get(buf, nthr, i, 2 * EL, r.z);
  r.inf = z_all_zero(r.z);
  return r;
}
template <class C, bool EXACT>
DH_DEV typename C::P add_lds(const typename C::P& a, const uint32_t* buf, int nthr, int i) {
  if constexpr (C::IS_G2) {
    constexpr int EL = 28;
    f228 z;
    lds_get(buf, nthr, i, 2 * EL, z);
    return j228_add_ld<EXACT>(a, z_all_zero(z), [&](int k) { f228 c; lds_get(buf, nthr, i, k * EL, c); return c; });
  } else {
    return C::template addx<EXACT>(a, lds_get_pt<C>(buf, nthr, i));
  }
}
template <class C, bool EXACT>
DH_DEV typename C::P run_mem(const uint32_t* __restrict__ p, uint32_t cnt) {
  typename C::P acc = C::inf();
#pragma unroll 1
  for (uint32_t k = 0; k < cnt; k++) acc = C::template add_mem<EXACT>(acc, p + (size_t)3 * C::EW * k);
  return acc;
}
template <class C, bool EXACT>
DH_DEV typename C::P run_mem(const uint32_t* __restrict__ base, size_t first, uint32_t parts) {
  typename C::P acc = C::inf();
#pragma unroll 1
  for (uint32_t k = threadIdx.x; k < parts; k += 64) acc = C::template add_mem<EXACT>(acc, base + (size_t)3 * C::EW * (first + k));
  return acc;
}
template <class C>
__attribute__((noinline)) DH_DEV typename C::P add_lds_exact(const uint32_t* buf, int nthr, int i, int j) {
  return add_lds<C, true>(lds_get_pt<C>(buf, nthr, i), buf, nthr, j);
}
template <class C>
DH_DEV typename C::P wave_tree(typename C::P acc, uint32_t* buf, uint32_t span) {
  const int nthr = blockDim.x, i = threadIdx.x, lane = i & 63;
#pragma unroll 1
  for (uint32_t step = 1; step < span; step <<= 1) {
    if ((lane & (step - 1)) == 0) lds_put_pt<C>(buf, nthr, i, acc);
    __syncthreads();
    if ((lane & (2 * step - 1)) == 0) {
      typename C::P s = add_lds<C, false>(acc, buf, nthr, i + (int)step);
      if (C::poisoned(s)) {
        if constexpr (C::IS_G2) s = add_lds_exact<C>(buf, nthr, i, i + (int)step);
        else s = add_lds<C, true>(lds_get_pt<C>(buf, nthr, i), buf, nthr, i + (int)step);
      }
      acc = s;
    }
    __syncthreads();
  }
  return acc;
}

template <class C>
__global__ __launch_bounds__(256, C::OCC) void k_msm_segsum28(const uint32_t* __restrict__ buckets, const uint32_t* __restrict__ off,
                                                              msm_geom g, size_t ngw, size_t rows_per_set, uint32_t* __restrict__ segs,
                                                              uint32_t* __restrict__ runs) {
  const size_t t = gtid();
  if (t >= ngw * g.nseg) return;
  const size_t gw = t / g.nseg;
  const uint32_t s = t % g.nseg;
  const uint32_t a = 1 + s * g.seglen;
  uint32_t last = a + g.seglen;
  if (last > g.nbuck) last = g.nbuck;
  const size_t krow = (gw % rows_per_set) * g.nbuck, brow = gw * g.nbuck;
  typename C::P run, tot;
  seg_run<C, false>(buckets, off, krow, brow, a, last, run, tot);
  if (C::poisoned(run) || C::poisoned(tot)) seg_run<C, true>(buckets, off, krow, brow, a, last, run, tot);
  stj28<C>(segs, t, tot);
  stj28<C>(runs, t, run);
}
template <class C, bool EXACT>
DH_DEV typename C::P seg_off(const uint32_t* __restrict__ run, uint32_t k, const uint32_t* __restrict__ tot) {
  typename C::P acc = C::inf();
#pragma unroll 1
  for (int bit = 31 - __builtin_clz(k); bit >= 0; bit--) {
    acc = C::dbl(acc);
    if ((k >> bit) & 1) acc = C::template add_mem<EXACT>(acc, run);
  }
  return C::template add_mem<EXACT>(acc, tot);
}
template <class C>
__global__ __launch_bounds__(256, C::OCC) void k_msm_segoff28(msm_geom g, size_t ngw, uint32_t* __restrict__ segs,
                                                              const uint32_t* __restrict__ runs) {
  const size_t t = gtid();
  if (t >= ngw * g.nseg) return;
  const uint32_t k = (t % g.nseg) * g.seglen;
  if (!k) return;
  const uint32_t* run = runs + (size_t)3 * C::EW * t;
  if (ldj28<C>(runs, t).inf) return;
  uint32_t* tot = segs + (size_t)3 * C::EW * t;
  typename C::P r = seg_off<C, false>(run, k, tot);
  if (C::poisoned(r)) r = seg_off<C, true>(run, k, tot);
  stj28<C>(segs, t, r);
}

template <class C>
__global__ __launch_bounds__(256, C::OCC) void k_msm_rowtree28(const uint32_t* __restrict__ segs, uint32_t nseg, uint32_t G,
                                                               size_t ngw, uint32_t lpr, uint32_t span, uint32_t* __restrict__ out) {
  __shared__ uint32_t buf[lds_words<C>() * 256];
  const size_t t = gtid();
  typename C::P acc = C::inf();
  if (t < ngw * lpr) {
    const size_t row = t / lpr;
    const uint32_t s0 = (uint32_t)(t % lpr) * G;
    const uint32_t* p = segs + (size_t)3 * C::EW * (row * nseg + s0);
    const uint32_t cnt = s0 >= nseg ? 0 : min(G, nseg - s0);
    acc = run_mem<C, false>(p, cnt);
    if (C::poisoned(acc)) acc = run_mem<C, true>(p, cnt);
  }
  acc = wave_tree<C>(acc, buf, span);
  if (t < ngw * lpr && (t & (span - 1)) == 0) stj28<C>(out, t / span, acc);
}
template <class C>
__global__ __launch_bounds__(64) void k_msm_rowred28(const uint32_t* __restrict__ parts_in, uint32_t parts, uint32_t span,
                                                     uint32_t* __restrict__ rowsum) {
  __shared__ uint32_t buf[lds_words<C>() * 64];
  const size_t row = blockIdx.x;
  typename C::P acc = run_mem<C, false>(parts_in, row * parts, parts);
  if (C::poisoned(acc)) acc = run_mem<C, true>(parts_in, row * parts, parts);
  acc = wave_tree<C>(acc, buf, span);
  if (threadIdx.x == 0) stj28<C>(rowsum, row, acc);
}

template <class C, bool EXACT>
DH_DEV typename C::P horner28(const uint32_t* __restrict__ rowsum, const msm_geom& g, size_t t) {
  typename C::P acc = ldj28<C>(rowsum, t * g.nwin + g.nwin - 1);
#pragma unroll 1
  for (int w = g.nwin - 2; w >= 0; w--) {
#pragma unroll 1
    for (int k = 0; k < g.c; k++) acc = C::dbl(acc);
    acc = C::template add_mem<EXACT>(acc, rowsum + (size_t)3 * C::EW * (t * g.nwin + w));
  }
  return acc;
}

template <class C>
__global__ __launch_bounds__(64) void k_msm_windows28(const uint32_t* __restrict__ rowsum, msm_geom g, size_t ngroups,
                                                      uint32_t* __restrict__ out) {
  const size_t t = gtid();
  if (t >= ngroups) return;
  typename C::P acc = horner28<C, false>(rowsum, g, t);
  if (C::poisoned(acc)) acc = horner28<C, true>(rowsum, g, t);
  jac<typename C::F> r = jac_inf<typename C::F>();
  if (!acc.inf) {
    r.x = C::out(acc.x);
    r.y = C::out(acc.y);
    r.z = C::out(acc.z);
  }
  st_jac_aos<typename C::F>(out, t, r);
}

hipError_t launch_msm_prep28(int sig_g2, size_t n, uint8_t* status, const uint32_t* sig_aff, const uint32_t* q_pts,
                             uint32_t* S, uint32_t* Q, hipStream_t st, uint32_t sets, int parts) {
  if (!n) return hipSuccess;
  if (parts == 0) parts = sig_g2 ? c28_g2::PARTS : c28_g1::PARTS;
  if (parts != 2 && !(sig_g2 && parts == 4)) return hipErrorInvalidValue;
  const uint32_t K = prep28_k(n);
  const size_t nt = (n + K - 1) / K;
  if (sig_g2)
    hipLaunchKernelGGL(k_msm_prep28<c28_g2>, dim3(nblk(nt, 256)), dim3(256), 0, st, n, K, status, sig_aff, q_pts, S, Q, sets,
                       (uint32_t)parts);
  else
    hipLaunchKernelGGL(k_msm_prep28<c28_g1>, dim3(nblk(nt, 256)), dim3(256), 0, st, n, K, status, sig_aff, q_pts, S, Q, sets,
                       (uint32_t)parts);
  return hipGetLastError();
}

static unsigned few_waves_block(size_t nthreads) { return nthreads <= 256 * 64 ? 64u : 256u; }

template <class C>
static hipError_t msm28(const msm_geom& g, size_t ngroups, const uint32_t* S, const uint32_t* Q, msm_ws& ws, hipStream_t st,
                        const uint8_t* skip, int nsets = 2) {
  const size_t nk = ngroups * g.nwin * (size_t)g.nbuck;
  constexpr size_t jw = 3 * C::EW;
  uint32_t* bB = ws.buckets + nk * jw;
  uint32_t* pB = ws.part + msm_nchunks(ws.max_entries) * 2 * jw;
  if (ws.max_entries) {
    const uint32_t L = msm_chunk_len(ws.max_entries, C::LCAP, (size_t)C::OCC * 131072);
    const size_t nch = (ws.max_entries + L - 1) / L;
    hipLaunchKernelGGL((k_msm_bucket28<C, true>), dim3(nblk(nch, 256)), dim3(256), 0, st, ws.off, ws.list, nk, L, S, ws.buckets,
                       ws.part, ws.meta, skip, g.half_stride);
    hipLaunchKernelGGL(k_msm_bucket_fix28<C>, dim3(nblk(nch, 256)), dim3(256), 0, st, ws.off, nk, L, ws.meta, ws.part, ws.buckets);
    if (nsets == 2) {
      hipLaunchKernelGGL((k_msm_bucket28<C, true>), dim3(nblk(nch, 256)), dim3(256), 0, st, ws.off, ws.list, nk, L, Q, bB, pB,
                         ws.meta, skip, g.half_stride);
      hipLaunchKernelGGL(k_msm_bucket_fix28<C>, dim3(nblk(nch, 256)), dim3(256), 0, st, ws.off, nk, L, ws.meta, pB, bB);
    }
  }
  const size_t rows = ngroups * g.nwin, ngw = (size_t)nsets * rows;
  const unsigned sb = few_waves_block(ngw * g.nseg);
  hipLaunchKernelGGL(k_msm_segsum28<C>, dim3(nblk(ngw * g.nseg, sb)), dim3(sb), 0, st, ws.buckets, ws.off, g, ngw, rows, ws.segs,
                     ws.runs);
  if (g.nseg > 1)
    hipLaunchKernelGGL(k_msm_segoff28<C>, dim3(nblk(ngw * g.nseg, sb)), dim3(sb), 0, st, g, ngw, ws.segs, ws.runs);
  uint32_t G = g.nseg <= 64 ? 1 : (ngw * g.nseg >= ((size_t)1 << 17) ? 8 : 2);
  if (G == 2 && g.nseg / 2 > 64 && (g.nseg / 2) % 64) G = 8;
  uint32_t lpr = (g.nseg + G - 1) / G, span = 64;
  if (lpr <= 64) {
    for (span = 1; span < lpr;) span *= 2;
    lpr = span;
  } else if (lpr % 64) {
    lpr = (lpr + 63) / 64 * 64;
  }
  const uint32_t* rowsum = ws.runs;
  if (g.nseg > 1)
    hipLaunchKernelGGL(k_msm_rowtree28<C>, dim3(nblk(ngw * lpr, few_waves_block(ngw * lpr))), dim3(few_waves_block(ngw * lpr)), 0,
                       st, ws.segs, g.nseg, G, ngw, lpr, span, ws.runs);
  else
    rowsum = ws.segs;
  if (lpr > 64) {
    const uint32_t parts = lpr / 64;
    uint32_t pspan = 1;
    while (pspan < parts) pspan *= 2;
    hipLaunchKernelGGL(k_msm_rowred28<C>, dim3((unsigned)ngw), dim3(64), 0, st, ws.runs, parts, pspan, ws.segs);
    rowsum = ws.segs;
  }
  hipLaunchKernelGGL(k_msm_windows28<C>, dim3(nblk(nsets * ngroups, 64)), dim3(64), 0, st, rowsum, g, nsets * ngroups, ws.out2);
  return hipGetLastError();
}

hipError_t launch_msm28(int sig_g2, const msm_geom& g, const uint32_t* entries, size_t m, size_t ngroups, const uint4* scal,
                        const uint32_t* S, const uint32_t* Q, msm_ws& ws, uint32_t* outA, uint32_t* outB, hipStream_t st,
                        const uint8_t* skip, bool presorted) {
  hipError_t e = hipSuccess;
  if (!presorted && (e = launch_msm_sort(g, entries, nullptr, nullptr, m, ngroups, scal, ws, st)) != hipSuccess) return e;
  e = sig_g2 ? msm28<c28_g2>(g, ngroups, S, Q, ws, st, skip) : msm28<c28_g1>(g, ngroups, S, Q, ws, st, skip);
  if (e != hipSuccess) return e;
  const size_t ow = sig_g2 ? 72 : 36, bytes = ngroups * ow * 4;
  if ((e = hipMemcpyAsync(outA, ws.out2, bytes, hipMemcpyDeviceToDevice, st)) != hipSuccess) return e;
  return hipMemcpyAsync(outB, ws.out2 + ngroups * ow, bytes, hipMemcpyDeviceToDevice, st);
}

hipError_t launch_msm28_set(int sig_g2, const msm_geom& g, const uint32_t* pidx, const uint32_t* sidx, const uint32_t* grp,
                            size_t m, size_t ngroups, const uint4* scal, const uint32_t* P, msm_ws& ws, uint32_t* out,
                            hipStream_t st) {
  hipError_t e = launch_msm_sort(g, pidx, sidx, grp, m, ngroups, scal, ws, st);
  if (e != hipSuccess) return e;
  e = sig_g2 ? msm28<c28_g2>(g, ngroups, P, nullptr, ws, st, nullptr, 1) : msm28<c28_g1>(g, ngroups, P, nullptr, ws, st, nullptr, 1);
  if (e != hipSuccess) return e;
  return hipMemcpyAsync(out, ws.out2, ngroups * (sig_g2 ? 72 : 36) * 4, hipMemcpyDeviceToDevice, st);
}

constexpr uint32_t SUB_G = 8;
DH_DEV uint32_t sub_digit(uint32_t j, uint32_t b) { return ((j >> b) << (b + 1)) | (1u << b) | (j & ((1u << b) - 1)); }
template <class C, bool EXACT>
DH_DEV typename C::P sub_run(const uint32_t* __restrict__ buckets, const uint32_t* __restrict__ off, size_t row0, uint32_t b,
                             uint32_t j0, uint32_t j1) {
  typename C::P acc = C::inf();
#pragma unroll 1
  for (uint32_t j = j0; j < j1; j++) {
    const size_t k = row0 + sub_digit(j, b);
    if (off[k + 1] != off[k]) acc = C::template add_mem<EXACT>(acc, buckets + (size_t)3 * C::EW * k);
  }
  return acc;
}
template <class C>
__global__ __launch_bounds__(256, C::OCC) void k_sub_bits28(const uint32_t* __restrict__ buckets, const uint32_t* __restrict__ off,
                                                            msm_geom g, uint32_t lpp, uint32_t* __restrict__ out) {
  __shared__ uint32_t buf[lds_words<C>() * 256];
  const size_t t = gtid();
  const size_t nlanes = (size_t)g.nwin * g.c * lpp;
  typename C::P acc = C::inf();
  if (t < nlanes) {
    const uint32_t pair = (uint32_t)(t / lpp), w = pair / g.c, b = pair % g.c;
    const uint32_t cnt = b + 1 == (uint32_t)g.c ? 1u : 1u << (g.c - 2);
    const uint32_t j0 = min(cnt, (uint32_t)(t % lpp) * SUB_G), j1 = min(cnt, j0 + SUB_G);
    const size_t row0 = (size_t)w * g.nbuck;
    acc = sub_run<C, false>(buckets, off, row0, b, j0, j1);
    if (C::poisoned(acc)) acc = sub_run<C, true>(buckets, off, row0, b, j0, j1);
  }
  acc = wave_tree<C>(acc, buf, 64);
  if (t < nlanes && (t & 63) == 0) stj28<C>(out, t / 64, acc);
}
template <class C>
__global__ __launch_bounds__(64) void k_sub_test28(const uint32_t* __restrict__ tpts, uint32_t npairs, uint8_t* __restrict__ pass,
                                                   uint8_t* __restrict__ sub_pass) {
  const size_t i = gtid();
  if (i >= npairs) return;
  bool in;
  if constexpr (C::IS_G2) in = g2_jac_in_subgroup28([&] { return ldj28<C>(tpts, i); });
  else in = g1_jac_in_subgroup28([&] { return ldj28<C>(tpts, i); }, f28_c(BETA28));
  if (!in) {
    pass[0] = 0;
    sub_pass[0] = 0;
  }
}

static uint32_t sub_lanes_per_pair(const msm_geom& g) {
  const uint32_t cnt = 1u << (g.c - 2);
  return ((cnt + SUB_G - 1) / SUB_G + 63) / 64 * 64;
}
size_t sub_batch_tmp_bytes(int sig_g2, const msm_geom& g) {
  const size_t npairs = (size_t)g.nwin * g.c;
  return (npairs * (sub_lanes_per_pair(g) / 64) + npairs) * 3 * (sig_g2 ? c28_g2::EW : c28_g1::EW) * 4;
}
template <class C>
static hipError_t sub_batch(const msm_geom& g, const msm_ws& ws, uint8_t* pass, uint8_t* sub_pass, hipStream_t st) {
  if (g.c < 3 || g.halves != 2 || !ws.sub) return hipErrorInvalidValue;
  hipError_t e = hipMemsetAsync(sub_pass, 1, 1, st);
  if (e != hipSuccess) return e;
  const uint32_t npairs = (uint32_t)g.nwin * g.c, lpp = sub_lanes_per_pair(g), parts = lpp / 64;
  uint32_t* tpts = ws.sub + (size_t)npairs * parts * 3 * C::EW;
  const size_t nlanes = (size_t)npairs * lpp;
  const unsigned blk = few_waves_block(nlanes);
  hipLaunchKernelGGL(k_sub_bits28<C>, dim3(nblk(nlanes, blk)), dim3(blk), 0, st, ws.buckets, ws.off, g, lpp, ws.sub);
  uint32_t pspan = 1;
  while (pspan < parts) pspan *= 2;
  hipLaunchKernelGGL(k_msm_rowred28<C>, dim3(npairs), dim3(64), 0, st, ws.sub, parts, pspan, tpts);
  hipLaunchKernelGGL(k_sub_test28<C>, dim3(nblk(npairs, 64)), dim3(64), 0, st, tpts, npairs, pass, sub_pass);
  return hipGetLastError();
}
hipError_t launch_sub_batch(int sig_g2, const msm_geom& g, const msm_ws& ws, uint8_t* pass, uint8_t* sub_pass, hipStream_t st) {
  return sig_g2 ? sub_batch<c28_g2>(g, ws, pass, sub_pass, st) : sub_batch<c28_g1>(g, ws, pass, sub_pass, st);
}

__global__ void k_fail_flags(const uint8_t* __restrict__ pass, size_t ngroups, uint32_t* __restrict__ flags) {
  const size_t g = gtid();
  if (g < ngroups) flags[g] = pass[g] ? 0u : 1u;
}
__global__ void k_compact_failing(const uint32_t* __restrict__ entries, size_t m, size_t gsize, const uint8_t* __restrict__ pass,
                                  const uint32_t* __restrict__ rank, uint32_t* __restrict__ out) {
  const size_t e = gtid();
  if (e >= m) return;
  const size_t g = e / gsize;
  if (!pass[g]) out[(size_t)rank[g] * gsize + (e - g * gsize)] = entries[e];
}
hipError_t launch_compact_failing(const uint32_t* entries, size_t m, size_t gsize, size_t ngroups, const uint8_t* pass,
                                  uint32_t* flags, uint32_t* rank, uint32_t* scan_tmp, uint32_t* out, hipStream_t st) {
  if (!m) return hipSuccess;
  hipLaunchKernelGGL(k_fail_flags, dim3(nblk(ngroups, 256)), dim3(256), 0, st, pass, ngroups, flags);
  hipError_t e = launch_scan(flags, ngroups, rank, scan_tmp, st);
  if (e != hipSuccess) return e;
  hipLaunchKernelGGL(k_compact_failing, dim3(nblk(m, 256)), dim3(256), 0, st, entries, m, gsize, pass, rank, out);
  return hipGetLastError();
}

hipError_t launch_mark_groups(const uint32_t* entries, size_t m, size_t gsize, const uint8_t* pass, const uint8_t* status,
                              uint8_t* verdict, hipStream_t st) {
  if (!m) return hipSuccess;
  hipLaunchKernelGGL(k_mark_groups, dim3(nblk(m, 256)), dim3(256), 0, st, entries, m, gsize, pass, status, verdict);
  return hipGetLastError();
}


DH_COUNTER_ACCESSOR(msm)

}
```

drand_amd/csrc/k_prep.hip:

```cpp
#include "kcommon.hpp"

namespace dh {

template <class F>
__global__ __launch_bounds__(256, occ<F>::W) void k_prep_sig(const uint8_t* __restrict__ sigs, size_t stride, size_t n,
                                                  uint8_t* __restrict__ status, uint32_t* __restrict__ sig_aff,
                                                  uint8_t* __restrict__ rand_out) {
  size_t i = gtid();
  if (i >= n) return;
  const uint8_t* s = sigs + i * stride;
  aff<F> a;
  uint8_t st;
  if constexpr (sizeof(F) == sizeof(fp)) {
    st = g1_decompress(a, s, false);
    if (st == DEC_OK) st_aff_aos<F>(sig_aff, i, a);
    if (rand_out) st_digest(rand_out + 32 * i, sha256_aligned<48>(s));
    if (st == DEC_OK && !g1_in_subgroup28([&] { return ld_aff_aos<fp>(sig_aff, i); })) st = DEC_BAD;
    if (st == DEC_OK) {
      status[i] = st;
      return;
    }
  } else {
    st = g2_decompress(a, s, true);
    if (rand_out) st_digest(rand_out + 32 * i, sha256_aligned<96>(s));
// ... 104 lines not shown
  if (sub_bad[i]) verdict[i] = 0;
}

__global__ __launch_bounds__(64) void k_h2f_g1_small(const uint64_t* __restrict__ rounds, const uint8_t* __restrict__ prevs,
                                                     size_t prev_stride, const uint32_t* __restrict__ prev_lens,
                                                     const uint8_t* __restrict__ msgs32, size_t n, int chained, int dst_id,
                                                     uint8_t* __restrict__ status, uint32_t* __restrict__ u_out) {
  const size_t i = gtid();
  if (i >= n) return;
  const sha_h d = message_of(rounds, prevs, prev_stride, prev_lens, msgs32, chained, i, status);
  uint32_t b[4][8];
  xmd32<4>(b, d, dst_id);
  st_f<fp>(u_out + 24 * i, fp_from_be512(b[0], b[1]));
  st_f<fp>(u_out + 24 * i + 12, fp_from_be512(b[2], b[3]));
}

__global__ __launch_bounds__(64) void k_sswu_g1_small(const uint32_t* __restrict__ u, size_t m, uint32_t* __restrict__ pts) {
  const size_t j = blockIdx.x;
  if (j >= m || threadIdx.x) return;
  fp x;
  ld_f<fp>(x, u + 12 * j);
  st_jac_aos<fp>(pts, j, swu_jac(sswu_g1(x)));
}

__global__ __launch_bounds__(64) void k_add_iso_g1_small(const uint32_t* __restrict__ pts, size_t n, uint32_t* __restrict__ q_out) {
  const size_t i = gtid();
  if (i >= n) return;
  const jac<fp> p0 = ld_jac_aos<fp>(pts, 2 * i), p1 = ld_jac_aos<fp>(pts, 2 * i + 1);
  jac<fp> s;
  const jac<fp> q = jac_add_distinct(s, p0, p1) ? iso11_jac(s) : jac_add(iso11_jac(p0), iso11_jac(p1));
  st_jac_aos<fp>(q_out, i, q);
}

size_t hash_small_tmp_bytes(int sig_g2, size_t n) {
  return sig_g2 ? hash_tmp_bytes(1, n) : n * (24 + 72) * 4;
}

hipError_t launch_hash_small(int sig_g2, const uint64_t* rounds, const uint8_t* prevs, size_t prev_stride, const uint32_t* prev_lens,
                             const uint8_t* msgs32, size_t n, int chained, int dst_id, uint8_t* status, uint32_t* q_out,
                             uint32_t* tmp, hipStream_t st) {
  if (!n) return hipSuccess;
  if (sig_g2) return launch_hash(1, rounds, prevs, prev_stride, prev_lens, msgs32, n, chained, dst_id, status, q_out, tmp, st);
  uint32_t* pts = tmp + 24 * n;
  hipLaunchKernelGGL(k_h2f_g1_small, dim3(nblk(n, 64)), dim3(64), 0, st, rounds, prevs, prev_stride, prev_lens, msgs32, n,
                     chained, dst_id, status, tmp);
  hipLaunchKernelGGL(k_sswu_g1_small, dim3((unsigned)(2 * n)), dim3(64), 0, st, (const uint32_t*)tmp, 2 * n, pts);
  hipLaunchKernelGGL(k_add_iso_g1_small, dim3(nblk(n, 64)), dim3(64), 0, st, (const uint32_t*)pts, n, q_out);
  return hipGetLastError();
}

hipError_t launch_dec_sig(int sig_g2, const uint8_t* sigs, size_t stride, size_t n, uint8_t* status, uint32_t* sig_aff,
                          uint8_t* rand_out, hipStream_t st) {
  if (!n) return hipSuccess;
  if (sig_g2)
    hipLaunchKernelGGL(k_dec_sig_g2, dim3(nblk(n, 256)), dim3(256), 0, st, sigs, stride, n, status, sig_aff, rand_out);
  else
    hipLaunchKernelGGL(k_dec_sig_g1, dim3(nblk(n, 64)), dim3(64), 0, st, sigs, stride, n, status, sig_aff, rand_out);
  return hipGetLastError();
}

hipError_t launch_sub_flag(int sig_g2, size_t n, const uint8_t* status, const uint32_t* sig_aff, uint8_t* sub_bad, hipStream_t st) {
  if (!n) return hipSuccess;
  if (sig_g2) hipLaunchKernelGGL(k_sub_flag<fp2>, dim3(nblk(n, 64)), dim3(64), 0, st, n, status, sig_aff, sub_bad);
  else hipLaunchKernelGGL(k_sub_flag<fp>, dim3(nblk(n, 64)), dim3(64), 0, st, n, status, sig_aff, sub_bad);
  return hipGetLastError();
}

hipError_t launch_and_subgroup(size_t n, const uint8_t* sub_bad, uint8_t* verdict, hipStream_t st) {
  if (!n) return hipSuccess;
  hipLaunchKernelGGL(k_and_subgroup, dim3(nblk(n, 64)), dim3(64), 0, st, n, sub_bad, verdict);
  return hipGetLastError();
}

__global__ __launch_bounds__(256, occ<fp>::W) void k_prep_msg_g1(const uint64_t* __restrict__ rounds, const uint8_t* __restrict__ prevs,
                                                            size_t prev_stride, const uint32_t* __restrict__ prev_lens,
                                                            const uint8_t* __restrict__ msgs32, size_t n, int chained, int dst_id,
                                                            uint8_t* __restrict__ status, uint32_t* __restrict__ q_out) {
  size_t i = gtid();
  if (i >= n) return;
  const sha_h d = message_of(rounds, prevs, prev_stride, prev_lens, msgs32, chained, i, status);
  st_jac_aos<fp>(q_out, i, h2c_g1_noclear(d, dst_id));
}

DH_DEV void round_g1_ride(const fp& u0, const fp& u1, bool msg_ok, const uint8_t* __restrict__ s, size_t i,
                          uint8_t* __restrict__ status, uint32_t* __restrict__ sig_aff, uint8_t* __restrict__ rand_out,
                          uint32_t* __restrict__ q_out) {
  st_f<fp>(q_out + 36 * i, u0);
  st_f<fp>(q_out + 36 * i + 12, u1);
  g1_sum_mid m;
  fp c;
  const bool distinct = g1_sum_pre(m, c, sswu_g1(u0), sswu_g1(u1));
  c = fp_select(distinct, c, fp_one());
  fp inv_c;
  {
    aff<fp> a;
    uint8_t st = g1_decompress_ride(a, inv_c, s, c);
    if (rand_out) st_digest(rand_out + 32 * i, sha256_aligned<48>(s));
    if (st != DEC_OK) {
      a.x = fp{};
      a.y = fp{};
      st = DEC_BAD;
    }
    status[i] = msg_ok ? st : (uint8_t)DEC_BAD;
    st_aff_aos<fp>(sig_aff, i, a);
  }
  if (distinct) {
    st_jac_aos<fp>(q_out, i, iso11_aff(g1_sum_post(m, inv_c)));
  } else {
    fp v0, v1;
    ld_f<fp>(v0, q_out + 36 * i);
    ld_f<fp>(v1, q_out + 36 * i + 12);
    st_jac_aos<fp>(q_out, i, h2c_g1_map(v0, v1));
  }
}

__global__ __launch_bounds__(256, occ<fp>::W) void k_round_g1_ride(const uint64_t* __restrict__ rounds, const uint8_t* __restrict__ prevs,
                                                              size_t prev_stride, const uint32_t* __restrict__ prev_lens,
                                                              const uint8_t* __restrict__ msgs32, size_t n, int chained, int dst_id,
                                                              const uint8_t* __restrict__ sigs, size_t stride,
                                                              uint8_t* __restrict__ status, uint32_t* __restrict__ sig_aff,
                                                              uint8_t* __restrict__ rand_out, uint32_t* __restrict__ q_out) {
  size_t i = gtid();
  if (i >= n) return;
  sha_h d;
  bool msg_ok = true;
  if (msgs32) d = message_of(nullptr, nullptr, 0, nullptr, msgs32, 0, i, nullptr);
  else msg_ok = beacon_digest(d, rounds, prevs, prev_stride, prev_lens, chained, i);
  uint32_t b[4][8];
  xmd32<4>(b, d, dst_id);
  round_g1_ride(fp_from_be512(b[0], b[1]), fp_from_be512(b[2], b[3]), msg_ok, sigs + i * stride, i, status, sig_aff, rand_out,
                q_out);
}

__global__ __launch_bounds__(256, occ<fp>::W) void k_round_g1_ride_debug(const uint8_t* __restrict__ u, size_t n,
                                                                    const uint8_t* __restrict__ sigs, size_t stride,
                                                                    uint8_t* __restrict__ status, uint32_t* __restrict__ sig_aff,
                                                                    uint32_t* __restrict__ q_out) {
  size_t i = gtid();
  if (i >= n) return;
  fp u0, u1;
  be48_words(u0.v, u + 96 * i, false);
  be48_words(u1.v, u + 96 * i + 48, false);
  round_g1_ride(fp_to_mont(u0), fp_to_mont(u1), true, sigs + i * stride, i, status, sig_aff, nullptr, q_out);
}
__global__ __launch_bounds__(64) void k_round_g1_debug_out(size_t n, const uint32_t* __restrict__ sig_aff,
                                                           const uint32_t* __restrict__ q_pts, uint8_t* __restrict__ sig_out,
                                                           uint8_t* __restrict__ q_out) {
  size_t i = gtid();
  if (i >= n) return;
  const aff<fp> s = ld_aff_aos<fp>(sig_aff, i);
  st_be48(sig_out + 96 * i, fp_from_mont(s.x));
  st_be48(sig_out + 96 * i + 48, fp_from_mont(s.y));
  const jac<fp> q = ld_jac_aos<fp>(q_pts, i);
  aff<fp> a{fp{}, fp{}};
  if (!jac_is_inf(q)) a = jac_to_aff(q);
  st_be48(q_out + 96 * i, fp_from_mont(a.x));
  st_be48(q_out + 96 * i + 48, fp_from_mont(a.y));
}

__global__ __launch_bounds__(256) void k_h2f_g2(const uint64_t* __restrict__ rounds, const uint8_t* __restrict__ prevs,
                                                size_t prev_stride, const uint32_t* __restrict__ prev_lens,
                                                const uint8_t* __restrict__ msgs32, size_t n, int chained, int dst_id,
                                                uint8_t* __restrict__ status, uint32_t* __restrict__ u_out) {
  size_t i = gtid();
  if (i >= n) return;
  const sha_h d = message_of(rounds, prevs, prev_stride, prev_lens, msgs32, chained, i, status);
  uint32_t b[8][8];
  xmd32<8>(b, d, dst_id);
  const fp2 u0 = {fp_from_be512(b[0], b[1]), fp_from_be512(b[2], b[3])};
  const fp2 u1 = {fp_from_be512(b[4], b[5]), fp_from_be512(b[6], b[7])};
  st_f<fp2>(u_out + 48 * i, u0);
  st_f<fp2>(u_out + 48 * i + 24, u1);
}

__global__ __launch_bounds__(256, 2) void k_sswu_g2(const uint32_t* __restrict__ u, size_t m, uint32_t* __restrict__ pts) {
  size_t j = gtid();
  if (j >= m) return;
  fp2 x;
  ld_f<fp2>(x, u + 24 * j);
  st_jac_aos<fp2>(pts, j, swu_jac(sswu_g2(x)));
}

__global__ __launch_bounds__(256, 2) void k_add_iso_g2(const uint32_t* __restrict__ pts, size_t n, uint32_t* __restrict__ q_out,
                                                       uint32_t* __restrict__ exc) {
  size_t i = gtid();
  if (i >= n) return;
  jac<fp2> s;
  if (!jac_add_distinct_mem(s, pts + 144 * i, pts + 144 * i + 72)) {
    exc[1 + atomicAdd(exc, 1u)] = (uint32_t)i;
    return;
  }
  st_jac_aos<fp2>(q_out, i, iso3_jac_lean(s));
}

constexpr unsigned EXC_THREADS = 64;
__global__ __launch_bounds__(EXC_THREADS, 1) void k_add_iso_g2_exc(const uint32_t* __restrict__ pts, const uint32_t* __restrict__ exc,
                                                                   uint32_t* __restrict__ q_out) {
  const uint32_t cnt = exc[0];
  for (uint32_t k = threadIdx.x; k < cnt; k += EXC_THREADS) {
    const uint32_t i = exc[1 + k];
    const jac<fp2> p0 = ld_jac_aos<fp2>(pts, 2 * (size_t)i), p1 = ld_jac_aos<fp2>(pts, 2 * (size_t)i + 1);
    st_jac_aos<fp2>(q_out, i, jac_add(iso3_jac(p0), iso3_jac(p1)));
  }
}

__global__ __launch_bounds__(256, occ<fp>::W) void k_prep_msgv_g1(const uint8_t* __restrict__ msgs, const uint32_t* __restrict__ msg_off,
                                                             size_t n, int dst_id, uint32_t* __restrict__ q_out) {
  size_t i = gtid();
  if (i >= n) return;
  const uint32_t lo = msg_off[i];
  uint32_t b[4][8];
  xmd_any<4>(b, msgs + lo, msg_off[i + 1] - lo, dst_id);
  st_jac_aos<fp>(q_out, i, h2c_g1_map(fp_from_be512(b[0], b[1]), fp_from_be512(b[2], b[3])));
}

__global__ __launch_bounds__(256) void k_h2fv_g2(const uint8_t* __restrict__ msgs, const uint32_t* __restrict__ msg_off, size_t n,
                                                 int dst_id, uint32_t* __restrict__ u_out) {
  size_t i = gtid();
  if (i >= n) return;
  const uint32_t lo = msg_off[i];
  uint32_t b[8][8];
  xmd_any<8>(b, msgs + lo, msg_off[i + 1] - lo, dst_id);
  const fp2 u0 = {fp_from_be512(b[0], b[1]), fp_from_be512(b[2], b[3])};
  const fp2 u1 = {fp_from_be512(b[4], b[5]), fp_from_be512(b[6], b[7])};
  st_f<fp2>(u_out + 48 * i, u0);
  st_f<fp2>(u_out + 48 * i + 24, u1);
}

__global__ __launch_bounds__(256) void k_scalars(const uint32_t* __restrict__ seed_words, size_t n,
                                                 const uint8_t* __restrict__ status, int parts, uint4* __restrict__ scal) {
  size_t i = gtid();
  if (i >= n) return;
  uint32_t w[16];
#pragma unroll
  for (int j = 0; j < 8; j++) w[j] = seed_words[j];
  w[8] = (uint32_t)((uint64_t)i >> 32);
  w[9] = (uint32_t)i;
  w[10] = 0x80000000u;
#pragma unroll
  for (int j = 11; j < 15; j++) w[j] = 0;
// ... 45 lines not shown
  }
  __syncthreads();
  if (t == 0) {
    const uint8_t st = (uint8_t)st_sh == DEC_OK && !sub_sh ? (uint8_t)DEC_BAD : (uint8_t)st_sh;
    *ok = st;
    if (st != DEC_OK) st_aff_aos<K>(key_aff, 0, aff<K>{K{}, K{}});
  }
}


hipError_t launch_prep(int sig_g2, const uint8_t* sigs, size_t stride, size_t n, uint8_t* status, uint32_t* sig_aff,
                       uint8_t* rand_out, hipStream_t st, bool defer_sub) {
  if (!n) return hipSuccess;
  if (sig_g2) {
    hipLaunchKernelGGL(k_dec_sig_g2, dim3(nblk(n, 256)), dim3(256), 0, st, sigs, stride, n, status, sig_aff, rand_out);
    if (!defer_sub) hipLaunchKernelGGL(k_sub_sig_g2, dim3(nblk(n, 256)), dim3(256), 0, st, n, status, sig_aff);
  } else if (defer_sub)
    hipLaunchKernelGGL(k_dec_sig_g1_batch, dim3(nblk(n, 256)), dim3(256), 0, st, sigs, stride, n, status, sig_aff, rand_out);
  else
    hipLaunchKernelGGL(k_prep_sig<fp>, dim3(nblk(n, 256)), dim3(256), 0, st, sigs, stride, n, status, sig_aff, rand_out);
  return hipGetLastError();
}

hipError_t launch_sub_exact(int sig_g2, size_t n, uint8_t* status, uint32_t* sig_aff, uint8_t* sub_bad, uint32_t* nbad,
                            hipStream_t st) {
  hipError_t e = hipMemsetAsync(nbad, 0, 4, st);
  if (e != hipSuccess || !n) return e;
  if (sig_g2) {
    hipLaunchKernelGGL(k_sub_flag_batch_g2, dim3(nblk(n, 256)), dim3(256), 0, st, n, (const uint8_t*)status,
                       (const uint32_t*)sig_aff, sub_bad);
    hipLaunchKernelGGL(k_sub_reject<fp2>, dim3(nblk(n, 256)), dim3(256), 0, st, n, (const uint8_t*)sub_bad, status, sig_aff, nbad);
    return hipGetLastError();
  }
  hipLaunchKernelGGL(k_sub_flag_batch, dim3(nblk(n, 256)), dim3(256), 0, st, n, (const uint8_t*)status, (const uint32_t*)sig_aff,
                     sub_bad);
  hipLaunchKernelGGL(k_sub_reject<fp>, dim3(nblk(n, 256)), dim3(256), 0, st, n, (const uint8_t*)sub_bad, status, sig_aff, nbad);
  return hipGetLastError();
}


hipError_t launch_scalars(const uint32_t* seed_words, size_t n, const uint8_t* status, uint4* scal, int parts, hipStream_t st) {
  if (!n) return hipSuccess;
  hipLaunchKernelGGL(k_scalars, dim3(nblk(n, 256)), dim3(256), 0, st, seed_words, n, status, parts, scal);
  return hipGetLastError();
}

hipError_t launch_decode_key(int key_g2, const uint8_t* pk, uint32_t* key_aff, uint8_t* ok, hipStream_t st) {
  if (key_g2) hipLaunchKernelGGL(k_decode_key<fp2>, dim3(1), dim3(128), 0, st, pk, key_aff, ok);
  else hipLaunchKernelGGL(k_decode_key<fp>, dim3(1), dim3(128), 0, st, pk, key_aff, ok);
  return hipGetLastError();
}


size_t hash_tmp_bytes(int sig_g2, size_t n) { return sig_g2 ? n * 2 * 72 * 4 + (n + 1) * 4 : 0; }

static hipError_t hash_g2_map(size_t n, uint32_t* q_out, uint32_t* tmp, hipStream_t st) {
  hipLaunchKernelGGL(k_sswu_g2, dim3(nblk(2 * n, 256)), dim3(256), 0, st, (const uint32_t*)q_out, 2 * n, tmp);
  uint32_t* exc = tmp + n * 2 * 72;
  hipError_t e = hipMemsetAsync(exc, 0, 4, st);
  if (e != hipSuccess) return e;
  hipLaunchKernelGGL(k_add_iso_g2, dim3(nblk(n, 256)), dim3(256), 0, st, (const uint32_t*)tmp, n, q_out, exc);
  hipLaunchKernelGGL(k_add_iso_g2_exc, dim3(1), dim3(EXC_THREADS), 0, st, (const uint32_t*)tmp, (const uint32_t*)exc, q_out);
  return hipGetLastError();
}

hipError_t launch_hash(int sig_g2, const uint64_t* rounds, const uint8_t* prevs, size_t prev_stride, const uint32_t* prev_lens,
                       const uint8_t* msgs32, size_t n, int chained, int dst_id, uint8_t* status, uint32_t* q_out, uint32_t* tmp,
                       hipStream_t st) {
  if (!n) return hipSuccess;
  if (!sig_g2) {
    hipLaunchKernelGGL(k_prep_msg_g1, dim3(nblk(n, 256)), dim3(256), 0, st, rounds, prevs, prev_stride, prev_lens, msgs32, n,
                       chained, dst_id, status, q_out);
    return hipGetLastError();
  }
  hipLaunchKernelGGL(k_h2f_g2, dim3(nblk(n, 256)), dim3(256), 0, st, rounds, prevs, prev_stride, prev_lens, msgs32, n, chained,
                     dst_id, status, q_out);
  return hash_g2_map(n, q_out, tmp, st);
}

hipError_t launch_round_g1_ride(const uint64_t* rounds, const uint8_t* prevs, size_t prev_stride, const uint32_t* prev_lens,
                                const uint8_t* msgs32, size_t n, int chained, int dst_id, const uint8_t* sigs, size_t stride,
                                uint8_t* status, uint32_t* sig_aff, uint8_t* rand_out, uint32_t* q_out, hipStream_t st) {
  if (!n) return hipSuccess;
  hipLaunchKernelGGL(k_round_g1_ride, dim3(nblk(n, 256)), dim3(256), 0, st, rounds, prevs, prev_stride, prev_lens, msgs32, n,
                     chained, dst_id, sigs, stride, status, sig_aff, rand_out, q_out);
  return hipGetLastError();
}

hipError_t launch_round_g1_ride_debug(const uint8_t* u, const uint8_t* sigs, size_t n, uint8_t* status, uint32_t* sig_aff,
                                      uint32_t* q_pts, uint8_t* sig_out, uint8_t* q_out, hipStream_t st) {
  if (!n) return hipSuccess;
  hipLaunchKernelGGL(k_round_g1_ride_debug, dim3(nblk(n, 256)), dim3(256), 0, st, u, n, sigs, (size_t)48, status, sig_aff, q_pts);
  hipLaunchKernelGGL(k_round_g1_debug_out, dim3(nblk(n, 64)), dim3(64), 0, st, n, (const uint32_t*)sig_aff,
                     (const uint32_t*)q_pts, sig_out, q_out);
  return hipGetLastError();
}

hipError_t launch_hash_var(int sig_g2, const uint8_t* msgs, const uint32_t* msg_off, size_t n, int dst_id, uint32_t* q_out,
                           uint32_t* tmp, hipStream_t st) {
  if (!n) return hipSuccess;
  if (!sig_g2) {
    hipLaunchKernelGGL(k_prep_msgv_g1, dim3(nblk(n, 256)), dim3(256), 0, st, msgs, msg_off, n, dst_id, q_out);
    return hipGetLastError();
  }
  hipLaunchKernelGGL(k_h2fv_g2, dim3(nblk(n, 256)), dim3(256), 0, st, msgs, msg_off, n, dst_id, q_out);
  return hash_g2_map(n, q_out, tmp, st);
}

DH_COUNTER_ACCESSOR(prep)

}
```

drand_amd/csrc/kcommon.hpp:

```cpp
#pragma once
#include <hip/hip_runtime.h>
#include "pairing.hpp"
#include "h2c.hpp"
#include "codec.hpp"
#include "kernels.hpp"

namespace dh {

template <class F>
struct npw {
  static constexpr int N = limbs_of<F>::N;
};

template <class F>
DH_DEV void ld_f(F& a, const uint32_t* p);
template <>
DH_DEV void ld_f<fp>(fp& a, const uint32_t* p) {
  const uint4* q = (const uint4*)p;
#pragma unroll
  for (int i = 0; i < 3; i++) {
    uint4 t = q[i];
    a.v[4 * i] = t.x; a.v[4 * i + 1] = t.y; a.v[4 * i + 2] = t.z; a.v[4 * i + 3] = t.w;
  }
}
template <>
DH_DEV void ld_f<fp2>(fp2& a, const uint32_t* p) {
  ld_f<fp>(a.c0, p);
  ld_f<fp>(a.c1, p + 12);
}
template <class F>
DH_DEV void st_f(uint32_t* p, const F& a);
template <>
DH_DEV void st_f<fp>(uint32_t* p, const fp& a) {
  uint4* q = (uint4*)p;
#pragma unroll
  for (int i = 0; i < 3; i++) q[i] = make_uint4(a.v[4 * i], a.v[4 * i + 1], a.v[4 * i + 2], a.v[4 * i + 3]);
}
template <>
DH_DEV void st_f<fp2>(uint32_t* p, const fp2& a) {
  st_f<fp>(p, a.c0);
  st_f<fp>(p + 12, a.c1);
}
template <class F>
DH_DEV jac<F> ld_jac_aos(const uint32_t* base, size_t i) {
  constexpr int N = npw<F>::N;
  const uint32_t* p = base + (size_t)3 * N * i;
  jac<F> r;
  ld_f<F>(r.x, p);
  ld_f<F>(r.y, p + N);
  ld_f<F>(r.z, p + 2 * N);
  return r;
}
template <class F>
DH_DEV void st_jac_aos(uint32_t* base, size_t i, const jac<F>& a) {
  constexpr int N = npw<F>::N;
  uint32_t* p = base + (size_t)3 * N * i;
  st_f<F>(p, a.x);
  st_f<F>(p + N, a.y);
  st_f<F>(p + 2 * N, a.z);
}
template <class F>
DH_DEV aff<F> ld_aff_aos(const uint32_t* base, size_t i) {
  constexpr int N = npw<F>::N;
  const uint32_t* p = base + (size_t)2 * N * i;
  aff<F> r;
  ld_f<F>(r.x, p);
  ld_f<F>(r.y, p + N);
  return r;
}
template <class F>
DH_DEV void st_aff_aos(uint32_t* base, size_t i, const aff<F>& a) {
  constexpr int N = npw<F>::N;
  uint32_t* p = base + (size_t)2 * N * i;
  st_f<F>(p, a.x);
  st_f<F>(p + N, a.y);
}

DH_DEV bool jac_add_distinct_mem(jac<fp2>& r, const uint32_t* P, const uint32_t* Q) {
  fp2 c1, c2, zz, u1, h;
  {
    fp2 z1, z2;
    ld_f<fp2>(z1, P + 48);
    ld_f<fp2>(z2, Q + 48);
    const fp2 z1z1 = fp2_sqr(z1), z2z2 = fp2_sqr(z2);
    c1 = fp2_mul(z1, z1z1);
    c2 = fp2_mul(z2, z2z2);
    zz = fp2_mul(z1, z2);
    fp2 x;
    ld_f<fp2>(x, P);
    u1 = fp2_mul(x, z2z2);
    ld_f<fp2>(x, Q);
    h = fp2_sub(fp2_mul(x, z1z1), u1);
  }
  if (fp2_is_zero(h)) return false;
  fp2 s1, rr;
  {
    fp2 y;
    ld_f<fp2>(y, P + 24);
    s1 = fp2_mul(y, c2);
    ld_f<fp2>(y, Q + 24);
    rr = fp2_dbl(fp2_sub(fp2_mul(y, c1), s1));
  }
  const fp2 i = fp2_sqr(fp2_dbl(h));
  const fp2 j = fp2_mul(h, i);
  const fp2 v = fp2_mul(u1, i);
  r.x = fp2_sub(fp2_sub(fp2_sqr(rr), j), fp2_dbl(v));
  r.y = fp2_sub(fp2_mul(rr, fp2_sub(v, r.x)), fp2_dbl(fp2_mul(s1, j)));
  r.z = fp2_dbl(fp2_mul(zz, h));
  return true;
}

template <class F>
struct other;
template <>
struct other<fp> {
  using T = fp2;
};
template <>
struct other<fp2> {
  using T = fp;
};

template <class F>
struct occ {
  static constexpr int W = 2;
};
template <>
struct occ<fp2> {
  static constexpr int W = 2;
};

DH_DEV size_t gtid() { return (size_t)blockIdx.x * blockDim.x + threadIdx.x; }

DH_DEV jac<fp> g1_gen() { return {fp_c(cst::G1X), fp_c(cst::G1Y), fp_one()}; }
DH_DEV jac<fp2> g2_gen() { return {fp2_c(cst::G2X), fp2_c(cst::G2Y), fp2_one()}; }

static inline unsigned nblk(size_t n, unsigned t) { return (unsigned)((n + t - 1) / t); }

DH_DEV bool beacon_digest(sha_h& d, const uint64_t* __restrict__ rounds, const uint8_t* __restrict__ prevs, size_t prev_stride,
                          const uint32_t* __restrict__ prev_lens, int chained, size_t i) {
  if (!chained) {
    d = digest_unchained(rounds[i]);
    return true;
  }
  const uint64_t pl = prev_lens ? (uint64_t)prev_lens[i] : (uint64_t)prev_stride;
  if (pl > prev_stride) {
    d = digest_unchained(rounds[i]);
    return false;
  }
  const uint8_t* p = prevs + i * prev_stride;
  if (pl <= 96 && (pl & 3) == 0 && (((uintptr_t)p) & 3) == 0) d = digest_chained(p, (uint32_t)pl, rounds[i]);
  else d = digest_chained_any(p, (uint32_t)pl, rounds[i]);
  return true;
}

DH_DEV sha_h message_of(const uint64_t* __restrict__ rounds, const uint8_t* __restrict__ prevs, size_t prev_stride,
                        const uint32_t* __restrict__ prev_lens, const uint8_t* __restrict__ msgs32, int chained, size_t i,
                        uint8_t* __restrict__ status) {
// ... 13 lines not shown
```

drand_amd/csrc/kernels.hpp:

```cpp
#pragma once
#include <cstdlib>
#include <hip/hip_runtime.h>
#include <stddef.h>
#include <stdint.h>

namespace dh {

struct msm_geom {
  uint32_t gsize;
  int c;
  int nwin;
  uint32_t nbuck;
  uint32_t nseg;
  uint32_t seglen;
  uint32_t halves;
  uint32_t half_stride;
};
inline size_t msm_entries(const msm_geom& g, size_t m) { return m * (size_t)g.nwin * g.halves; }

struct msm_ws {
  uint32_t* cnt;
  uint32_t* off;
  uint32_t* scan_tmp;
  uint32_t* list;
  uint32_t* buckets;
  uint32_t* segs;
  uint32_t* out2;
  uint32_t* part;
  uint32_t* meta;
  size_t max_entries;
  uint32_t* runs = nullptr;
  uint32_t* sub = nullptr;
};

inline uint32_t msm_chunk_len(size_t max_entries, size_t cap = 32, size_t target_chunks = 262144) {
  static const size_t lmin = [] {
    const char* e = getenv("DRANDHIP_MSM_LMIN");
    const long v = e ? atol(e) : 0;
    return (size_t)(v >= 1 && v <= 64 ? v : 8);
  }();
  size_t L = max_entries / target_chunks;
  if (L < lmin) L = lmin;
  return (uint32_t)(L > cap ? cap : L);
}
inline size_t msm_nchunks(size_t max_entries) { return max_entries / msm_chunk_len(max_entries) + 2; }
inline size_t msm_part_bytes(size_t max_entries, size_t jac_words, int nsets) {
  return msm_nchunks(max_entries) * 2 * jac_words * 4 * (size_t)nsets;
}
inline size_t msm_meta_bytes(size_t max_entries) { return msm_nchunks(max_entries) * 2 * 4; }

hipError_t launch_prep(int sig_g2, const uint8_t* sigs, size_t stride, size_t n, uint8_t* status, uint32_t* sig_aff,
                       uint8_t* rand_out, hipStream_t st, bool defer_sub = false);
hipError_t launch_sub_exact(int sig_g2, size_t n, uint8_t* status, uint32_t* sig_aff, uint8_t* sub_bad, uint32_t* nbad, hipStream_t st);
hipError_t launch_dec_sig(int sig_g2, const uint8_t* sigs, size_t stride, size_t n, uint8_t* status, uint32_t* sig_aff,
                          uint8_t* rand_out, hipStream_t st);
hipError_t launch_sub_flag(int sig_g2, size_t n, const uint8_t* status, const uint32_t* sig_aff, uint8_t* sub_bad, hipStream_t st);
hipError_t launch_and_subgroup(size_t n, const uint8_t* sub_bad, uint8_t* verdict, hipStream_t st);
size_t hash_small_tmp_bytes(int sig_g2, size_t n);
hipError_t launch_hash_small(int sig_g2, const uint64_t* rounds, const uint8_t* prevs, size_t prev_stride, const uint32_t* prev_lens,
                             const uint8_t* msgs32, size_t n, int chained, int dst_id, uint8_t* status, uint32_t* q_out,
                             uint32_t* tmp, hipStream_t st);
size_t hash_tmp_bytes(int sig_g2, size_t n);
hipError_t launch_hash(int sig_g2, const uint64_t* rounds, const uint8_t* prevs, size_t prev_stride, const uint32_t* prev_lens,
                       const uint8_t* msgs32, size_t n, int chained, int dst_id, uint8_t* status, uint32_t* q_out, uint32_t* tmp,
                       hipStream_t st);
hipError_t launch_round_g1_ride(const uint64_t* rounds, const uint8_t* prevs, size_t prev_stride, const uint32_t* prev_lens,
                                const uint8_t* msgs32, size_t n, int chained, int dst_id, const uint8_t* sigs, size_t stride,
                                uint8_t* status, uint32_t* sig_aff, uint8_t* rand_out, uint32_t* q_out, hipStream_t st);
hipError_t launch_round_g1_ride_debug(const uint8_t* u, const uint8_t* sigs, size_t n, uint8_t* status, uint32_t* sig_aff,
                                      uint32_t* q_pts, uint8_t* sig_out, uint8_t* q_out, hipStream_t st);
hipError_t launch_hash_var(int sig_g2, const uint8_t* msgs, const uint32_t* msg_off, size_t n, int dst_id, uint32_t* q_out,
                           uint32_t* tmp, hipStream_t st);
hipError_t launch_scalars(const uint32_t* seed_words, size_t n, const uint8_t* status, uint4* scal, int parts, hipStream_t st);
hipError_t launch_decode_key(int key_g2, const uint8_t* pk, uint32_t* key_aff, uint8_t* ok, hipStream_t st);
hipError_t launch_iota(uint32_t* v, size_t n, hipStream_t st);
hipError_t launch_scan(const uint32_t* cnt, size_t nk, uint32_t* off, uint32_t* tmp, hipStream_t st);
hipError_t launch_msm_prep28(int sig_g2, size_t n, uint8_t* status, const uint32_t* sig_aff, const uint32_t* q_pts,
                             uint32_t* S, uint32_t* Q, hipStream_t st, uint32_t sets = 3, int parts = 0);
hipError_t launch_msm28_set(int sig_g2, const msm_geom& g, const uint32_t* pidx, const uint32_t* sidx, const uint32_t* grp,
                            size_t m, size_t ngroups, const uint4* scal, const uint32_t* P, msm_ws& ws, uint32_t* out,
                            hipStream_t st);
hipError_t launch_msm28(int sig_g2, const msm_geom& g, const uint32_t* entries, size_t m, size_t ngroups, const uint4* scal,
                        const uint32_t* S, const uint32_t* Q, msm_ws& ws, uint32_t* outA, uint32_t* outB, hipStream_t st,
                        const uint8_t* skip, bool presorted);
size_t sub_batch_tmp_bytes(int sig_g2, const msm_geom& g);
hipError_t launch_sub_batch(int sig_g2, const msm_geom& g, const msm_ws& ws, uint8_t* pass, uint8_t* sub_pass, hipStream_t st);
hipError_t launch_msm_sort(const msm_geom& g, const uint32_t* pidx, const uint32_t* sidx, const uint32_t* grp, size_t m,
                           size_t ngroups, const uint4* scal, msm_ws& ws, hipStream_t st);
hipError_t launch_group_check(int sig_g2, const uint32_t* A, const uint32_t* B, size_t ngroups, const uint32_t* key_aff,
                              uint8_t* pass, hipStream_t st);
hipError_t launch_sum_partials(int sig_g2, const uint32_t* parts, size_t k, size_t rec_words, uint32_t* outA, uint32_t* outB,
                               uint8_t* flag, hipStream_t st);
hipError_t launch_node_mark(size_t n, uint8_t* res, const uint8_t* status, uint8_t* verdict, hipStream_t st);
hipError_t launch_mark_groups(const uint32_t* entries, size_t m, size_t gsize, const uint8_t* pass, const uint8_t* status,
                              uint8_t* verdict, hipStream_t st);
hipError_t launch_compact_failing(const uint32_t* entries, size_t m, size_t gsize, size_t ngroups, const uint8_t* pass,
                                  uint32_t* flags, uint32_t* rank, uint32_t* scan_tmp, uint32_t* out, hipStream_t st);
hipError_t launch_leaf_check(int sig_g2, const uint32_t* entries, size_t m, const uint32_t* sig_aff, const uint32_t* q_pts,
                             const uint32_t* key_aff, const uint8_t* status, uint8_t* verdict, hipStream_t st);

hipError_t launch_group_check_vm(int sig_g2, const uint32_t* A, const uint32_t* B, size_t ngroups, const uint32_t* key_aff,
                                 const uint32_t* key_h,
                                 uint32_t* pairs, uint8_t* live, uint8_t* pass, hipStream_t st);
size_t group_check_c_pair_words();
hipError_t launch_group_check_vm_c(const uint32_t* A, const uint32_t* B, size_t ngroups, const uint32_t* key_aff, uint32_t* pairs,
                                   uint8_t* live, uint8_t* done, uint8_t* pass, hipStream_t st);
hipError_t launch_leaf_check_vm(int sig_g2, const uint32_t* entries, size_t m, const uint32_t* sig_aff, const uint32_t* q_pts,
                                const uint32_t* key_aff, const uint32_t* key_h, const uint8_t* status, uint32_t* pairs,
                                uint8_t* live, uint8_t* done, uint8_t* verdict, hipStream_t st);

hipError_t launch_leaf_check_vm_c(const uint32_t* entries, size_t m, const uint32_t* sig_aff, const uint32_t* q_pts,
                                  const uint32_t* key_aff, const uint8_t* status, uint32_t* pairs, uint8_t* live, uint8_t* done,
                                  uint8_t* verdict, hipStream_t st);

hipError_t launch_group_check_g1j(const uint32_t* A, const uint32_t* B, size_t ngroups, const uint32_t* key_h, uint8_t* pass,
                                  hipStream_t st);
hipError_t launch_leaf_check_g1j(const uint32_t* entries, size_t m, const uint32_t* sig_aff, const uint32_t* q_pts,
                                 const uint32_t* key_h, const uint8_t* status, uint8_t* verdict, hipStream_t st);

hipError_t launch_multi_pairing_vm(const uint32_t* P, const uint32_t* Q, size_t n, uint32_t* pairs, uint8_t* live,
                                   uint32_t* f_tmp, uint8_t* pass, hipStream_t st);

hipError_t launch_sign(int sig_g2, const uint32_t* sk, const uint64_t* rounds, const uint8_t* prevs, size_t prev_stride,
                       const uint32_t* prev_lens, const uint8_t* msgs32, size_t n, int chained, int dst_id, uint8_t* out,
                       uint32_t* q_tmp, uint32_t* h_tmp, hipStream_t st);
hipError_t launch_h2c_generic(int g2, const uint8_t* msgs, const uint32_t* off, size_t n, const uint8_t* dst, uint32_t dlen,
                              uint8_t* scratch, size_t sstride, uint8_t* out, hipStream_t st);
hipError_t launch_pubkey(int key_g2, const uint32_t* sk, uint8_t* out, hipStream_t st);

hipError_t launch_repack_partials(const uint8_t* raw, size_t n, int sig_len, uint8_t* sigs, uint32_t* idx, hipStream_t st);
hipError_t launch_pubpoly_eval(int key_g2, const uint32_t* commits, int t, int n_nodes, uint32_t* out, hipStream_t st);
hipError_t launch_pair_check(const uint32_t* P, const uint32_t* Q, size_t npairs, int clear_p, int clear_q,
                             const uint8_t* live, uint32_t* f_tmp, uint8_t* skip_tmp, uint8_t* pass, hipStream_t st);
hipError_t launch_partial_leaf(int sig_g2, const uint32_t* list, size_t m, const uint32_t* sig_aff, const uint8_t* status,
                               const uint32_t* share_idx, const uint32_t* round_of, const uint32_t* q_pts,
                               const uint32_t* shares, int n_nodes, uint8_t* ok_out, hipStream_t st);
hipError_t launch_partial_meta(const uint32_t* off, size_t n_rounds, const uint32_t* share_idx, int n_nodes, uint32_t* round_of,
                               uint8_t* status, hipStream_t st);
hipError_t launch_clamp_group(const uint32_t* share_idx, size_t np, uint32_t hi, uint32_t* grp, hipStream_t st);
hipError_t launch_ok_from_status(const uint8_t* status, size_t np, uint8_t* ok, hipStream_t st);
size_t lam_words();
hipError_t launch_select_lagrange(const uint32_t* off, const uint8_t* ok, const uint32_t* share_idx, int t, size_t n_rounds,
                                  uint32_t* sel, uint32_t* key, uint32_t* den, uint32_t* lam, uint32_t* lam_set, uint8_t* rok,
                                  uint32_t* own, int g1, hipStream_t st);
hipError_t launch_mark_selected(const uint32_t* sel, const uint8_t* rok, int t, size_t n_rounds, size_t np, uint8_t* need,
                                hipStream_t st);
hipError_t launch_wnaf_table_g2(const uint32_t* paff, const uint8_t* ok, size_t n, int entries, uint32_t* tbl, uint32_t* zs,
                                hipStream_t st);
size_t wnaf_table_scratch_bytes(size_t n, int entries);
hipError_t launch_lagrange(int sig_g2, const uint32_t* sel, const uint32_t* lam, const uint32_t* lam_set, const uint8_t* ok,
                           int t, size_t n_rounds, const uint32_t* sig_aff, const uint32_t* tbl, int entries, uint32_t* out,
                           uint32_t* tmp, hipStream_t st);
size_t lagrange_tmp_bytes(int sig_g2);
// ... 61 lines not shown
```

include/drandhip.h:

```cpp
#ifndef DRANDHIP_H
#define DRANDHIP_H

#include <stddef.h>
#include <stdint.h>

#ifdef __cplusplus
extern "C" {
#endif

#define DH_OK 0
#define DH_EINVAL (-1)
#define DH_EDEVICE (-2)
#define DH_ENOMEM (-3)
#define DH_EKEY (-4)
#define DH_ERECOVER (-5)
#define DH_EBUSY (-6)
#define DH_EABANDONED (-7)
#define DH_ECORRUPT (-8)
#define DH_ENOBEACON (-9)

#define DH_SCHEME_CHAINED 0
#define DH_SCHEME_UNCHAINED 1
#define DH_SCHEME_G1_LEGACY 2
#define DH_SCHEME_G1_RFC9380 3
// ... 19 lines not shown
int dh_verify_beacon(int scheme, const uint8_t* pk, size_t pk_len, uint64_t round, const uint8_t* sig, size_t sig_len,
                     const uint8_t* prev, size_t prev_len);

int dh_verify_recovered(int scheme, const uint8_t* pk, size_t pk_len, const uint8_t* msg32, const uint8_t* sig,
                        size_t sig_len);

int dh_verify_recovered_batch(int scheme, const uint8_t* pk, size_t pk_len, const uint8_t* msgs32, const uint8_t* sigs,
                              size_t sig_stride, size_t n, uint8_t* verdict_out, uint64_t seed);

int dh_digest_batch(int scheme, const uint64_t* rounds, const uint8_t* prevs, size_t prev_stride,
                    const uint32_t* prev_lens, size_t n, uint8_t* out);

int dh_randomness_batch(int scheme, const uint8_t* sigs, size_t sig_stride, size_t n, uint8_t* out);

int dh_recover_batch(int scheme, const uint8_t* commits, int t, int n_nodes, const uint8_t* msgs32,
                     const uint8_t* partials, const uint32_t* part_off, size_t n_rounds, uint8_t* sig_out,
                     uint8_t* status_out);

int dh_verify_partials_batch(int scheme, const uint8_t* commits, int t, int n_nodes, const uint8_t* msgs32,
                             const uint8_t* partials, const uint32_t* part_off, size_t n_rounds, uint8_t* ok_out);

int dh_bls_verify_batch(int scheme, const uint8_t* keys, size_t n_keys, const uint32_t* key_idx, const uint8_t* msgs,
                        const uint32_t* msg_off, const uint8_t* sigs, size_t sig_stride, size_t n, uint8_t* verdict_out,
                        uint8_t* key_ok_out, uint64_t seed, uint64_t stats_out[4]);

int dh_identity_hash_batch(int scheme, const uint8_t* keys, size_t n, uint8_t* out32);

int dh_identity_verify_batch(int scheme, const uint8_t* keys, const uint8_t* sigs, size_t sig_stride, size_t n,
                             uint8_t* verdict_out);

int dh_schnorr_verify_batch(int scheme, const uint8_t* keys, size_t n_keys, const uint32_t* key_idx, const uint8_t* msgs,
                            const uint32_t* msg_off, const uint8_t* sigs, size_t sig_stride, size_t n, uint8_t* verdict_out,
                            uint8_t* key_ok_out);
int dh_schnorr_sig_len(int scheme);

typedef struct dh_batch dh_batch;
#define DH_NODE_CHECKED 2
int dh_partial_bytes(int scheme);
int dh_batch_begin(int scheme, const uint8_t* pk, size_t pk_len, const uint64_t* d_rounds, const uint8_t* d_sigs,
                   size_t sig_stride, const uint8_t* d_prevs, size_t prev_stride, const uint32_t* d_prev_lens, size_t n,
                   uint8_t* d_verdict_out, uint8_t* d_rand_out, uint64_t seed, void* hip_stream, dh_batch** batch_out,
                   uint8_t* d_partials_out);
void* dh_batch_stream(dh_batch* batch);
int dh_batch_check(dh_batch* batch, const uint8_t* d_partials, size_t k, void* hip_stream);
int dh_check_partials(int scheme, const uint8_t* pk, size_t pk_len, const uint8_t* d_partials, size_t k, int* pass_out);
int dh_batch_finish(dh_batch* batch, int node_pass, uint64_t stats_out[4]);

int dh_bolt_index(const uint8_t* file, size_t len, uint32_t* page_size_out, uint64_t* leaf_off_out, size_t cap,
                  size_t* n_leaves_out);

typedef struct dh_store dh_store;
int dh_store_open_bolt(const uint8_t* file, size_t len, dh_store** out);
int dh_store_stat(const dh_store* store, uint64_t out[6]);
int dh_store_columns_device(dh_store* store, uint64_t first, uint64_t last, size_t row_stride, uint64_t* d_rounds,
                            uint8_t* d_rows, uint32_t* d_lens, size_t cap_rows, size_t* n_rows_out, uint64_t* d_missing,
                            size_t cap_missing, size_t* n_missing_out, void* hip_stream);
int dh_store_check_past(dh_store* store, int scheme, const uint8_t* pk, size_t pk_len, uint64_t up_to, size_t window,
                        uint64_t seed, uint64_t* faulty_out, size_t cap, size_t* n_faulty_out,
                        void (*cb)(uint64_t round, uint64_t up_to, void* arg), void* cb_arg);
void dh_store_close(dh_store* store);

#define DH_STORE_TRIMMED 0
#define DH_STORE_UNTRIMMED 1
#define DH_STORE_AUTO 2
#define DH_DEFERRED 1
int dh_store_open_bolt_format(const uint8_t* file, size_t len, int format, dh_store** out);
int dh_store_format_stat(const dh_store* store, uint64_t out[4]);
int dh_store_beacons_device(dh_store* store, uint64_t first, uint64_t last, size_t sig_stride, size_t prev_stride,
                            uint64_t* d_rounds, uint8_t* d_sigs, uint32_t* d_sig_lens, uint8_t* d_prevs, uint32_t* d_prev_lens,
                            uint8_t* d_deferred, size_t cap_rows, size_t* n_rows_out, uint64_t* d_missing, size_t cap_missing,
                            size_t* n_missing_out, void* hip_stream);
int dh_store_deferred(dh_store* store, uint64_t first, uint64_t last, uint64_t* out, size_t cap, size_t* n_out);

int dh_sign_batch(int scheme, const uint8_t* sk32, const uint64_t* rounds, const uint8_t* prevs, size_t n,
                  const uint32_t* prev_lens, size_t prev_stride, uint8_t* sigs_out);
int dh_public_key(int scheme, const uint8_t* sk32, uint8_t* key_out);

int dh_hash_to_curve(int group, const uint8_t* msgs, const uint32_t* msg_off, size_t n, const uint8_t* dst, size_t dst_len,
                     uint8_t* out);

int dh_g1_round_prep_debug(const uint8_t* us, const uint8_t* sigs, size_t n, uint8_t* status_out, uint8_t* sig_out,
                           uint8_t* hash_out);

int dh_profile(int enable);
int dh_profile_read(char* buf, size_t cap);

const char* dh_last_error_string(void);

const char* dh_version(void);

#ifdef __cplusplus
}
#endif
#endif
```

Measured before the change: 49.86 million beacons/s.

## Defer G1 11-isogeny past the batch MSM by bucketing hashes on isogenous curve

After: 51.36 million beacons/s, median of 6. 1.03x the previous value.

```diff
diff --git a/drand_amd/_lib.py b/drand_amd/_lib.py
--- a/drand_amd/_lib.py
+++ b/drand_amd/_lib.py
@@ -51,6 +51,7 @@
     "dh_set_split": (_c.c_int, [_c.c_uint64, _c.c_int]),
     "dh_hash_to_curve": (_c.c_int, [_c.c_int, _P, _P, _c.c_size_t, _c.c_char_p, _c.c_size_t, _P]),
     "dh_g1_round_prep_debug": (_c.c_int, [_P, _P, _c.c_size_t, _P, _P, _P]),
+    "dh_g1_round_prep_late_debug": (_c.c_int, [_P, _P, _c.c_size_t, _P, _P, _P]),
     "dh_batch_begin": (_c.c_int, [_c.c_int, _c.c_char_p, _c.c_size_t, _P, _P, _c.c_size_t, _P, _c.c_size_t, _P,
                                   _c.c_size_t, _P, _P, _c.c_uint64, _P, _c.POINTER(_P), _P]),
     "dh_batch_check": (_c.c_int, [_P, _P, _c.c_size_t, _P]),
diff --git a/drand_amd/csrc/drandhip.cpp b/drand_amd/csrc/drandhip.cpp
--- a/drand_amd/csrc/drandhip.cpp
+++ b/drand_amd/csrc/drandhip.cpp
@@ -462,7 +462,7 @@
 }
 
 static void fit_segments(dh::msm_geom& g, size_t ngroups, size_t nsets) {
-  const size_t rows = std::max<size_t>(1, nsets * ngroups * (size_t)g.nwin);
+  const size_t rows = std::max<size_t>(1, nsets * ngroups * (size_t)dh::msm_rows(g));
   const size_t want = ((size_t)1 << 18) / rows + 1;
   size_t nseg = std::max<size_t>(1, std::min<size_t>({want, (size_t)g.nseg}));
   if (nseg > 512) nseg &= ~(size_t)511;
@@ -775,15 +775,23 @@
   return v;
 }
 
+static bool g1_iso_late_on() {
+  static const bool v = [] {
+    const char* e = getenv("DRANDHIP_G1_ISO_LATE");
+    return !(e && e[0] == '0');
+  }();
+  return v;
+}
+
 static int msm_workspace(worker* w, const dh::msm_geom& g, size_t m, size_t ngroups, size_t jw, dh::msm_ws& ws,
                          bool sub = false, bool g2 = false) {
-  const size_t nk = ngroups * g.nwin * (size_t)g.nbuck;
+  const size_t nk = ngroups * dh::msm_rows(g) * (size_t)g.nbuck;
   HIP_TRY(w->cnt.ensure(nk * 4));
   HIP_TRY(w->off.ensure((nk + 1) * 4));
   HIP_TRY(w->scan_tmp.ensure(((nk + 4095) / 4096 + 1) * 4));
   HIP_TRY(w->list.ensure(dh::msm_entries(g, m) * 4));
   HIP_TRY(w->buckets.ensure(2 * nk * jw * 4));
-  const size_t segs_bytes = 2 * ngroups * g.nwin * g.nseg * jw * 4;
+  const size_t segs_bytes = 2 * ngroups * dh::msm_rows(g) * g.nseg * jw * 4;
   HIP_TRY(w->segs.ensure(2 * segs_bytes));
   HIP_TRY(w->outA.ensure(ngroups * jw * 4));
   HIP_TRY(w->outB.ensure(ngroups * jw * 4));
@@ -825,6 +833,8 @@
   const bool sub_batch = sub_eligible && w->sub_fused_left == 0;
   if (sub_eligible && w->sub_fused_left > 0) w->sub_fused_left--;
   const int parts = g2 && !sub_batch ? 4 : 2;
+  const bool g1_ride = !g2 && sub_batch && g1_ride_on();
+  const bool iso_late = g1_ride && g1_iso_late_on();
   if (n >= ((size_t)1 << 31) / parts) return fail(DH_EINVAL, "batch too large");
   dh::msm_geom g0{};
   dh::msm_ws ws0{};
@@ -849,13 +859,22 @@
       HIP_TRY(dh::launch_iota(w->entries.as<uint32_t>(), n, ts));
       g0 = geom_for(n, parts);
       g0.half_stride = (uint32_t)n;
+      g0.split = iso_late ? 1 : 0;
       rc = msm_workspace(w, g0, n, 1, wsw, ws0, sub_batch, g2);
       if (rc) return rc;
       HIP_TRY(dh::launch_msm_sort(g0, w->entries.as<uint32_t>(), nullptr, nullptr, n, 1, w->scal.as<uint4>(), ws0, ts));
     }
     if (gate && gate->wait) HIP_TRY(hipStreamWaitEvent(st, gate->wait, 0));
     const int chained = scheme == DH_SCHEME_CHAINED && d_prevs && !d_msgs32 ? 1 : 0;
-    if (!g2 && sub_batch && g1_ride_on()) {
+    HIP_TRY(w->s28.ensure(parts * n * (g2 ? 64 : 32) * 4));
+    HIP_TRY(w->q28.ensure(parts * n * (g2 ? 64 : 32) * 4));
+    if (iso_late) {
+      HIP_TRY(T.run(d_msgs32 ? "k_prep_msg32<fp>" : "k_prep_msg<fp>", [&] {
+        return dh::launch_round_g1_ride_late(d_rounds, d_prevs, prev_stride, d_prev_lens, d_msgs32, n, chained, dst_id(scheme),
+                                             d_sigs, sig_stride, w->status.as<uint8_t>(), w->sig_aff.as<uint32_t>(), d_rand,
+                                             w->q_pts.as<uint32_t>(), w->s28.as<uint32_t>(), w->q28.as<uint32_t>(), st);
+      }));
+    } else if (g1_ride) {
       HIP_TRY(T.run(d_msgs32 ? "k_prep_msg32<fp>" : "k_prep_msg<fp>", [&] {
         return dh::launch_round_g1_ride(d_rounds, d_prevs, prev_stride, d_prev_lens, d_msgs32, n, chained, dst_id(scheme), d_sigs,
                                         sig_stride, w->status.as<uint8_t>(), w->sig_aff.as<uint32_t>(), d_rand,
@@ -876,12 +895,12 @@
       HIP_TRY(hipMemcpyAsync(d_seed, seedw, 32, hipMemcpyHostToDevice, st));
       HIP_TRY(dh::launch_scalars(d_seed, n, w->status.as<uint8_t>(), w->scal.as<uint4>(), parts, st));
     }
-    HIP_TRY(w->s28.ensure(parts * n * (g2 ? 64 : 32) * 4));
-    HIP_TRY(w->q28.ensure(parts * n * (g2 ? 64 : 32) * 4));
-    HIP_TRY(T.run(g2 ? "k_msm_prep28<fp2>" : "k_msm_prep28<fp>", [&] {
-      return dh::launch_msm_prep28(g2, n, w->status.as<uint8_t>(), w->sig_aff.as<uint32_t>(), w->q_pts.as<uint32_t>(),
-                                   w->s28.as<uint32_t>(), w->q28.as<uint32_t>(), st, 3, parts);
-    }));
+    if (!iso_late) {
+      HIP_TRY(T.run(g2 ? "k_msm_prep28<fp2>" : "k_msm_prep28<fp>", [&] {
+        return dh::launch_msm_prep28(g2, n, w->status.as<uint8_t>(), w->sig_aff.as<uint32_t>(), w->q_pts.as<uint32_t>(),
+                                     w->s28.as<uint32_t>(), w->q28.as<uint32_t>(), st, 3, parts);
+      }));
+    }
     HIP_TRY(hipMemsetAsync(d_verdict, 0, n, st));
     if (gate) {
       HIP_TRY(hipEventRecord(gate->done, st));
@@ -919,6 +938,7 @@
     gsize = std::min(gsize, m);
     dh::msm_geom g = geom_for(gsize, parts);
     g.half_stride = (uint32_t)n;
+    g.split = level == 0 && iso_late ? 1 : 0;
     const size_t ngroups = (m + gsize - 1) / gsize;
     fit_segments(g, ngroups, 2);
     const bool pre = level == 0 && presorted;
@@ -977,6 +997,14 @@
       HIP_TRY(hipMemcpyAsync(&nbad, (uint8_t*)w->sub_pass.p + 4, 4, hipMemcpyDeviceToHost, st));
       HIP_TRY(hipStreamSynchronize(st));
       if ((double)nbad * 2000 > (double)n) w->sub_fused_left = sub_backoff();
+    }
+    if (level == 0 && iso_late && nfail32) {
+      HIP_TRY(T.run("k_msm_prep28<fp>", [&] {
+        hipError_t e = dh::launch_iso_late_fallback(n, w->status.as<uint8_t>(), w->q28.as<uint32_t>(), w->q_pts.as<uint32_t>(), st);
+        if (e != hipSuccess) return e;
+        return dh::launch_msm_prep28(0, n, w->status.as<uint8_t>(), w->sig_aff.as<uint32_t>(), w->q_pts.as<uint32_t>(),
+                                     w->s28.as<uint32_t>(), w->q28.as<uint32_t>(), st, 3, parts);
+      }));
     }
     level++;
     const size_t nfail = nfail32;
@@ -2497,6 +2525,39 @@
   return DH_OK;
 }
 
+int dh_g1_round_prep_late_debug(const uint8_t* us, const uint8_t* sigs, size_t n, uint8_t* status_out, uint8_t* sig_out,
+                                uint8_t* hash_out) {
+  if (!us || !sigs || !status_out || !sig_out || !hash_out) return fail(DH_EINVAL, "null argument");
+  if (n == 0) return DH_OK;
+  for (size_t i = 0; i < 2 * n; i++)
+    if (!fp_bytes_canonical(us + 48 * i)) return fail(DH_EINVAL, "field element %zu is not below p", i);
+  lease L;
+  if (L.rc) return L.rc;
+  worker* w = L.w;
+  int rc = set_device_and_stream(w);
+  if (rc) return rc;
+  hipStream_t st = w->stream;
+  HIP_TRY(w->in_prevs.ensure(n * 96));
+  HIP_TRY(w->in_sigs.ensure(n * 48));
+  HIP_TRY(w->status.ensure(n));
+  HIP_TRY(w->sig_aff.ensure(n * JAC_WORDS_G1 * 2 / 3 * 4));
+  HIP_TRY(w->q_pts.ensure(n * JAC_WORDS_G1 * 4));
+  HIP_TRY(w->s28.ensure(n * 32 * 4));
+  HIP_TRY(w->q28.ensure(n * 32 * 4));
+  HIP_TRY(w->out_rand.ensure(n * 192));
+  HIP_TRY(hipMemcpyAsync(w->in_prevs.p, us, n * 96, hipMemcpyHostToDevice, st));
+  HIP_TRY(hipMemcpyAsync(w->in_sigs.p, sigs, n * 48, hipMemcpyHostToDevice, st));
+  uint8_t* out = w->out_rand.as<uint8_t>();
+  HIP_TRY(dh::launch_round_g1_ride_late_debug(w->in_prevs.as<uint8_t>(), w->in_sigs.as<uint8_t>(), n, w->status.as<uint8_t>(),
+                                              w->sig_aff.as<uint32_t>(), w->q_pts.as<uint32_t>(), w->s28.as<uint32_t>(),
+                                              w->q28.as<uint32_t>(), out, out + n * 96, st));
+  HIP_TRY(hipMemcpyAsync(status_out, w->status.p, n, hipMemcpyDeviceToHost, st));
+  HIP_TRY(hipMemcpyAsync(sig_out, out, n * 96, hipMemcpyDeviceToHost, st));
+  HIP_TRY(hipMemcpyAsync(hash_out, out + n * 96, n * 96, hipMemcpyDeviceToHost, st));
+  HIP_TRY(hipStreamSynchronize(st));
+  return DH_OK;
+}
+
 int dh_public_key(int scheme, const uint8_t* sk32, uint8_t* key_out) {
   int kl = dh_key_len(scheme);
   if (kl < 0) return kl;
diff --git a/drand_amd/csrc/fp28.hpp b/drand_amd/csrc/fp28.hpp
--- a/drand_amd/csrc/fp28.hpp
+++ b/drand_amd/csrc/fp28.hpp
@@ -234,6 +234,39 @@
   return r;
 }
 
+DH_DEV j28 j28_dbl_a(const j28& p, const f28& a28) {
+  const f28 a = f28_sqr(p.x);
+  const f28 b = f28_sqr(p.y);
+  const f28 c = f28_sqr(b);
+  const f28 t = f28_sqr(f28_add(p.x, b));
+  const f28 d = f28_lin3<8>(t, 2, a, -2, c, -2);
+  const f28 az4 = f28_mul(a28, f28_sqr(f28_sqr(p.z)));
+  const f28 e = f28_lin<0>(a, 3, az4, 1);
+  const f28 f = f28_sqr(e);
+  j28 r;
+  r.x = f28_lin<24>(f, 1, d, -2);
+  const f28 m = f28_mul(e, f28_sub<26>(d, r.x));
+  r.y = f28_lin<16>(m, 1, c, -8);
+  r.z = f28_scale(f28_mul(p.y, p.z), 2);
+  r.inf = p.inf;
+  return r;
+}
+DH_DEV f28 f28_e1p_a() {
+  const uint32_t k[14] = {0x5effb65u, 0x7b0e9afu, 0x2c3688cu, 0x2e2fbe8u, 0xf093be0u, 0x4e56b8eu, 0x51e099cu,
+                          0x22aa2e7u, 0xbb7ea2bu, 0x50194edu, 0xaee9f0bu, 0x4130e5du, 0x3ac15b2u, 0x0019762u};
+  f28 r;
+#pragma unroll
+  for (int i = 0; i < 14; i++) r.l[i] = k[i];
+  return r;
+}
+struct j28_on_e1 {
+  DH_DEV static j28 dbl(const j28& p) { return j28_dbl(p); }
+};
+struct j28_on_e1p {
+  DH_DEV static j28 dbl(const j28& p) { return j28_dbl_a(p, f28_e1p_a()); }
+};
+
+template <class CURVE = j28_on_e1>
 DH_DEV j28 j28_madd(const j28& p, const f28& qx, const f28& qy) {
   if (p.inf) return j28{qx, qy, f28_one(), false};
   const f28 z1z1 = f28_sqr(p.z);
@@ -242,7 +275,7 @@
   const f28 h = f28_sub<26>(u2, p.x);
   const f28 rr = f28_sub<18>(s2, p.y);
   if (f28_zero(h)) {
-    if (f28_zero(rr)) return j28_dbl(p);
+    if (f28_zero(rr)) return CURVE::dbl(p);
     return j28_inf();
   }
   const f28 hh = f28_sqr(h);
@@ -259,6 +292,7 @@
   return r;
 }
 
+template <class CURVE = j28_on_e1>
 DH_DEV j28 j28_add(const j28& p, const j28& q) {
   if (p.inf) return q;
   if (q.inf) return p;
@@ -269,7 +303,7 @@
   const f28 h = f28_sub<2>(u2, u1);
   const f28 rr = f28_sub<2>(s2, s1);
   if (f28_zero(h)) {
-    if (f28_zero(rr)) return j28_dbl(p);
+    if (f28_zero(rr)) return CURVE::dbl(p);
     return j28_inf();
   }
   const f28 i = f28_sqr(f28_scale(h, 2));
diff --git a/drand_amd/csrc/h2c.hpp b/drand_amd/csrc/h2c.hpp
--- a/drand_amd/csrc/h2c.hpp
+++ b/drand_amd/csrc/h2c.hpp
@@ -153,6 +153,18 @@
   return r;
 }
 
+DH_DEV aff<fp> e1p_dbl_aff(const swu_out<fp>& p) {
+  const fp xd2 = fp_sqr(p.xd), y2 = fp_dbl(p.y);
+  const fp ic = fp_inv(fp_mul(y2, xd2));
+  const fp xn2 = fp_sqr(p.xn);
+  const fp lam = fp_mul(fp_add(fp_add(fp_dbl(xn2), xn2), fp_mul(fp_c(cst::SSWU1_A), xd2)), ic);
+  const fp x = fp_mul(p.xn, fp_mul(fp_mul(y2, p.xd), ic));
+  aff<fp> r;
+  r.x = fp_sub(fp_sqr(lam), fp_dbl(x));
+  r.y = fp_sub(fp_mul(lam, fp_sub(x, r.x)), p.y);
+  return r;
+}
+
 DH_DEV jac<fp> iso11_aff(const aff<fp>& p) {
   using namespace cst;
   const f28 X = f28_from_fp(p.x);
diff --git a/drand_amd/csrc/k_msm.hip b/drand_amd/csrc/k_msm.hip
--- a/drand_amd/csrc/k_msm.hip
+++ b/drand_amd/csrc/k_msm.hip
@@ -1,3 +1,4 @@
+#include <type_traits>
 #include "kcommon.hpp"
 
 namespace dh {
@@ -30,6 +31,10 @@
   if (g.halves == 4) return make_uint4(h == 0 ? s.x : h == 1 ? s.y : h == 2 ? s.z : s.w, 0, 0, 0);
   return h ? make_uint4(s.z, s.w, 0, 0) : make_uint4(s.x, s.y, 0, 0);
 }
+DH_DEV size_t key_row(const msm_geom& g, size_t gi, uint32_t h, int w) {
+  return gi * msm_rows(g) + (g.split ? h * (uint32_t)g.nwin : 0u) + (uint32_t)w;
+}
+DH_DEV uint32_t half_point(const msm_geom& g, uint32_t idx0, uint32_t h) { return g.split ? idx0 : idx0 + h * g.half_stride; }
 DH_DEV uint32_t round_of(uint32_t idx, uint32_t nround) { return idx < nround ? idx : idx % nround; }
 
 __global__ void k_msm_hist(const uint32_t* __restrict__ pidx, const uint32_t* __restrict__ sidx,
@@ -44,7 +49,7 @@
     uint32_t carry = 0;
     for (int w = 0; w < g.nwin; w++) {
       const int32_t d = signed_digit(sh, w, g, carry);
-      if (d) atomicAdd(&cnt[(gi * g.nwin + w) * g.nbuck + (uint32_t)(d < 0 ? -d : d)], 1u);
+      if (d) atomicAdd(&cnt[key_row(g, gi, h, w) * g.nbuck + (uint32_t)(d < 0 ? -d : d)], 1u);
     }
   }
 }
@@ -59,12 +64,12 @@
   const size_t gi = entry_group(grp, e, g.gsize);
   for (uint32_t h = 0; h < g.halves; h++) {
     const uint4 sh = half_scalar(s, h, g);
-    const uint32_t idx = idx0 + h * g.half_stride;
+    const uint32_t idx = half_point(g, idx0, h);
     uint32_t carry = 0;
     for (int w = 0; w < g.nwin; w++) {
       const int32_t d = signed_digit(sh, w, g, carry);
       if (d) {
-        uint32_t pos = atomicAdd(&cursor[(gi * g.nwin + w) * g.nbuck + (uint32_t)(d < 0 ? -d : d)], 1u);
+        uint32_t pos = atomicAdd(&cursor[key_row(g, gi, h, w) * g.nbuck + (uint32_t)(d < 0 ? -d : d)], 1u);
         list[pos] = d < 0 ? (idx | NEG_BIT) : idx;
       }
     }
@@ -80,25 +85,33 @@
                                                          uint32_t* __restrict__ gcnt, uint32_t* __restrict__ list) {
   extern __shared__ uint32_t h[];
   const size_t e0 = (size_t)blockIdx.x * tile, e1 = min(m, e0 + tile);
-  const size_t rowkeys = (size_t)g.nwin * g.nbuck;
+  const size_t rowkeys = (size_t)msm_rows(g) * g.nbuck;
   const size_t kb = grp ? 0 : (e0 / g.gsize) * rowkeys, ke = grp ? nk : min(nk, ((e1 - 1) / g.gsize + 1) * rowkeys);
   const size_t K0 = kb + (size_t)blockIdx.y * slab;
   if (K0 >= ke) return;
   const uint32_t ns = (uint32_t)min((size_t)slab, ke - K0);
   for (uint32_t k = threadIdx.x; k < ns; k += SORT_T) h[k] = 0;
   __syncthreads();
+  uint32_t h_lo = 0, h_hi = g.halves - 1;
+  if (g.split) {
+    const size_t r0 = K0 / g.nbuck, r1 = (K0 + ns - 1) / g.nbuck, R = msm_rows(g);
+    if (r0 / R == r1 / R) {
+      h_lo = (uint32_t)(r0 % R) / (uint32_t)g.nwin;
+      h_hi = (uint32_t)(r1 % R) / (uint32_t)g.nwin;
+    }
+  }
   auto each = [&](auto&& f) {
     for (size_t e = e0 + threadIdx.x; e < e1; e += SORT_T) {
       const uint32_t idx0 = pidx[e];
       const uint4 s = scal[sidx ? sidx[e] : idx0];
       const size_t gi = entry_group(grp, e, g.gsize);
-      for (uint32_t hh = 0; hh < g.halves; hh++) {
+      for (uint32_t hh = h_lo; hh <= h_hi; hh++) {
         const uint4 sh = half_scalar(s, hh, g);
-        const uint32_t idx = idx0 + hh * g.half_stride;
+        const uint32_t idx = half_point(g, idx0, hh);
         uint32_t carry = 0;
         for (int w = 0; w < g.nwin; w++) {
           const int32_t d = signed_digit(sh, w, g, carry);
-          const size_t key = (gi * g.nwin + w) * g.nbuck + (uint32_t)(d < 0 ? -d : d);
+          const size_t key = key_row(g, gi, hh, w) * g.nbuck + (uint32_t)(d < 0 ? -d : d);
           if (d && key - K0 < ns) f((uint32_t)(key - K0), d < 0 ? (idx | NEG_BIT) : idx);
         }
       }
@@ -257,7 +270,8 @@
 
 hipError_t launch_msm_sort(const msm_geom& g, const uint32_t* pidx, const uint32_t* sidx, const uint32_t* grp, size_t m,
                            size_t ngroups, const uint4* scal, msm_ws& ws, hipStream_t st) {
-  size_t nk = ngroups * g.nwin * (size_t)g.nbuck;
+  if (g.split && g.halves != 2) return hipErrorInvalidValue;
+  size_t nk = ngroups * msm_rows(g) * (size_t)g.nbuck;
   ws.max_entries = msm_entries(g, m);
   hipError_t e = hipMemsetAsync(ws.cnt, 0, nk * sizeof(uint32_t), st);
   if (e != hipSuccess) return e;
@@ -274,7 +288,7 @@
       const long d = v ? atol(v) : 0;
       return (size_t)(d >= 1 && d <= 256 ? d : 8);
     }();
-    const size_t digits = (size_t)g.halves * g.nwin, rowkeys = (size_t)g.nwin * g.nbuck;
+    const size_t digits = (size_t)(g.split ? 1 : g.halves) * g.nwin, rowkeys = (size_t)msm_rows(g) * g.nbuck;
     static const size_t slab_max = [] {
       const char* v = getenv("DRANDHIP_SORT_SLAB");
       const long d = v ? atol(v) : 0;
@@ -305,26 +319,6 @@
   return hipGetLastError();
 }
 
-constexpr int W28 = 16;
-DH_DEV f28 ld28(const uint32_t* p) {
-  const uint4* q = (const uint4*)p;
-  f28 a;
-#pragma unroll
-  for (int i = 0; i < 4; i++) {
-    const uint4 t = q[i];
-    a.l[4 * i] = t.x;
-    a.l[4 * i + 1] = t.y;
-    if (4 * i + 2 < 14) a.l[4 * i + 2] = t.z;
-    if (4 * i + 3 < 14) a.l[4 * i + 3] = t.w;
-  }
-  return a;
-}
-DH_DEV void st28(uint32_t* p, const f28& a) {
-  uint4* q = (uint4*)p;
-#pragma unroll
-  for (int i = 0; i < 4; i++)
-    q[i] = make_uint4(a.l[4 * i], a.l[4 * i + 1], 4 * i + 2 < 14 ? a.l[4 * i + 2] : 0u, 4 * i + 3 < 14 ? a.l[4 * i + 3] : 0u);
-}
 DH_DEV void ld28(f28& a, const uint32_t* p) { a = ld28(p); }
 DH_DEV void st28(uint32_t* p, const f28& a, int) { st28(p, a); }
 DH_DEV void ld28(f228& a, const uint32_t* p) {
@@ -389,6 +383,22 @@
   DH_DEV static E endo_x(const E& x);
   DH_DEV static E endo_y(const E& y) { return y; }
 };
+struct c28_g1p : c28_g1 {
+  DH_DEV static P madd(const P& a, const E& x, const E& y) { return j28_madd<j28_on_e1p>(a, x, y); }
+  DH_DEV static P add(const P& a, const P& b) { return j28_add<j28_on_e1p>(a, b); }
+  template <bool EXACT>
+  DH_DEV static P add_mem(const P& a, const uint32_t* q) {
+    j28 b;
+    b.x = ld28(q);
+    b.y = ld28(q + W28);
+    b.z = ld28(q + 2 * W28);
+    b.inf = z_all_zero(b.z);
+    return EXACT ? j28_add<j28_on_e1p>(a, b) : j28_add_fast(a, b);
+  }
+  template <bool EXACT>
+  DH_DEV static P addx(const P& a, const P& b) { return EXACT ? j28_add<j28_on_e1p>(a, b) : j28_add_fast(a, b); }
+  DH_DEV static P dbl(const P& a) { return j28_on_e1p::dbl(a); }
+};
 struct c28_g2 {
   static constexpr int OCC = 1;
   static constexpr bool IS_G2 = true;
@@ -426,6 +436,24 @@
   DH_DEV static E psi2_x(const E& x) { return f2_red({f28_mul(x.c0, f28_c(PSI2_X28)), f28_mul(x.c1, f28_c(PSI2_X28))}); }
   DH_DEV static E psi2_y(const E& y) { return f2_red({f28_mul(y.c0, f28_c(PSI2_Y28)), f28_mul(y.c1, f28_c(PSI2_Y28))}); }
 };
+
+template <class C>
+struct prime_of {
+  using T = C;
+};
+template <>
+struct prime_of<c28_g1> {
+  using T = c28_g1p;
+};
+constexpr size_t NO_PRIME = ~(size_t)0;
+template <class C, class FN>
+DH_DEV typename C::P on_curve(bool prime, FN&& f) {
+  using CP = typename prime_of<C>::T;
+  if constexpr (!std::is_same<C, CP>::value) {
+    if (prime) return f(CP{});
+  }
+  return f(C{});
+}
 
 template <class C>
 DH_DEV typename C::P ldj28(const uint32_t* base, size_t i) {
@@ -739,7 +767,7 @@
   return add_lds<C, true>(lds_get_pt<C>(buf, nthr, i), buf, nthr, j);
 }
 template <class C>
-DH_DEV typename C::P wave_tree(typename C::P acc, uint32_t* buf, uint32_t span) {
+DH_DEV typename C::P wave_tree(typename C::P acc, uint32_t* buf, uint32_t span, bool prime = false) {
   const int nthr = blockDim.x, i = threadIdx.x, lane = i & 63;
 #pragma unroll 1
   for (uint32_t step = 1; step < span; step <<= 1) {
@@ -749,7 +777,11 @@
       typename C::P s = add_lds<C, false>(acc, buf, nthr, i + (int)step);
       if (C::poisoned(s)) {
         if constexpr (C::IS_G2) s = add_lds_exact<C>(buf, nthr, i, i + (int)step);
-        else s = add_lds<C, true>(lds_get_pt<C>(buf, nthr, i), buf, nthr, i + (int)step);
+        else
+          s = on_curve<C>(prime, [&](auto k) {
+            using K = decltype(k);
+            return add_lds<K, true>(lds_get_pt<K>(buf, nthr, i), buf, nthr, i + (int)step);
+          });
       }
       acc = s;
     }
@@ -761,7 +793,7 @@
 template <class C>
 __global__ __launch_bounds__(256, C::OCC) void k_msm_segsum28(const uint32_t* __restrict__ buckets, const uint32_t* __restrict__ off,
                                                               msm_geom g, size_t ngw, size_t rows_per_set, uint32_t* __restrict__ segs,
-                                                              uint32_t* __restrict__ runs) {
+                                                              uint32_t* __restrict__ runs, size_t prime_from) {
   const size_t t = gtid();
   if (t >= ngw * g.nseg) return;
   const size_t gw = t / g.nseg;
@@ -772,7 +804,11 @@
   const size_t krow = (gw % rows_per_set) * g.nbuck, brow = gw * g.nbuck;
   typename C::P run, tot;
   seg_run<C, false>(buckets, off, krow, brow, a, last, run, tot);
-  if (C::poisoned(run) || C::poisoned(tot)) seg_run<C, true>(buckets, off, krow, brow, a, last, run, tot);
+  if (C::poisoned(run) || C::poisoned(tot))
+    on_curve<C>(gw >= prime_from, [&](auto k) {
+      seg_run<decltype(k), true>(buckets, off, krow, brow, a, last, run, tot);
+      return tot;
+    });
   stj28<C>(segs, t, tot);
   stj28<C>(runs, t, run);
 }
@@ -788,7 +824,7 @@
 }
 template <class C>
 __global__ __launch_bounds__(256, C::OCC) void k_msm_segoff28(msm_geom g, size_t ngw, uint32_t* __restrict__ segs,
-                                                              const uint32_t* __restrict__ runs) {
+                                                              const uint32_t* __restrict__ runs, size_t prime_from) {
   const size_t t = gtid();
   if (t >= ngw * g.nseg) return;
   const uint32_t k = (t % g.nseg) * g.seglen;
@@ -796,47 +832,55 @@
   const uint32_t* run = runs + (size_t)3 * C::EW * t;
   if (ldj28<C>(runs, t).inf) return;
   uint32_t* tot = segs + (size_t)3 * C::EW * t;
-  typename C::P r = seg_off<C, false>(run, k, tot);
-  if (C::poisoned(r)) r = seg_off<C, true>(run, k, tot);
+  const typename C::P r = on_curve<C>(t / g.nseg >= prime_from, [&](auto c) {
+    using K = decltype(c);
+    typename C::P v = seg_off<K, false>(run, k, tot);
+    if (K::poisoned(v)) v = seg_off<K, true>(run, k, tot);
+    return v;
+  });
   stj28<C>(segs, t, r);
 }
 
 template <class C>
 __global__ __launch_bounds__(256, C::OCC) void k_msm_rowtree28(const uint32_t* __restrict__ segs, uint32_t nseg, uint32_t G,
-                                                               size_t ngw, uint32_t lpr, uint32_t span, uint32_t* __restrict__ out) {
+                                                               size_t ngw, uint32_t lpr, uint32_t span, uint32_t* __restrict__ out,
+                                                               size_t prime_from) {
   __shared__ uint32_t buf[lds_words<C>() * 256];
   const size_t t = gtid();
   typename C::P acc = C::inf();
+  const bool prime = t / lpr >= prime_from;
   if (t < ngw * lpr) {
     const size_t row = t / lpr;
     const uint32_t s0 = (uint32_t)(t % lpr) * G;
     const uint32_t* p = segs + (size_t)3 * C::EW * (row * nseg + s0);
     const uint32_t cnt = s0 >= nseg ? 0 : min(G, nseg - s0);
     acc = run_mem<C, false>(p, cnt);
-    if (C::poisoned(acc)) acc = run_mem<C, true>(p, cnt);
-  }
-  acc = wave_tree<C>(acc, buf, span);
+    if (C::poisoned(acc)) acc = on_curve<C>(prime, [&](auto k) { return run_mem<decltype(k), true>(p, cnt); });
+  }
+  acc = wave_tree<C>(acc, buf, span, prime);
   if (t < ngw * lpr && (t & (span - 1)) == 0) stj28<C>(out, t / span, acc);
 }
 template <class C>
 __global__ __launch_bounds__(64) void k_msm_rowred28(const uint32_t* __restrict__ parts_in, uint32_t parts, uint32_t span,
-                                                     uint32_t* __restrict__ rowsum) {
+                                                     uint32_t* __restrict__ rowsum, size_t prime_from) {
   __shared__ uint32_t buf[lds_words<C>() * 64];
   const size_t row = blockIdx.x;
+  const bool prime = row >= prime_from;
   typename C::P acc = run_mem<C, false>(parts_in, row * parts, parts);
-  if (C::poisoned(acc)) acc = run_mem<C, true>(parts_in, row * parts, parts);
-  acc = wave_tree<C>(acc, buf, span);
+  if (C::poisoned(acc))
+    acc = on_curve<C>(prime, [&](auto k) { return run_mem<decltype(k), true>(parts_in, row * parts, parts); });
+  acc = wave_tree<C>(acc, buf, span, prime);
   if (threadIdx.x == 0) stj28<C>(rowsum, row, acc);
 }
 
 template <class C, bool EXACT>
-DH_DEV typename C::P horner28(const uint32_t* __restrict__ rowsum, const msm_geom& g, size_t t) {
-  typename C::P acc = ldj28<C>(rowsum, t * g.nwin + g.nwin - 1);
+DH_DEV typename C::P horner28(const uint32_t* __restrict__ rowsum, const msm_geom& g, size_t row0) {
+  typename C::P acc = ldj28<C>(rowsum, row0 + g.nwin - 1);
 #pragma unroll 1
   for (int w = g.nwin - 2; w >= 0; w--) {
 #pragma unroll 1
     for (int k = 0; k < g.c; k++) acc = C::dbl(acc);
-    acc = C::template add_mem<EXACT>(acc, rowsum + (size_t)3 * C::EW * (t * g.nwin + w));
+    acc = C::template add_mem<EXACT>(acc, rowsum + (size_t)3 * C::EW * (row0 + w));
   }
   return acc;
 }
@@ -846,8 +890,8 @@
                                                       uint32_t* __restrict__ out) {
   const size_t t = gtid();
   if (t >= ngroups) return;
-  typename C::P acc = horner28<C, false>(rowsum, g, t);
-  if (C::poisoned(acc)) acc = horner28<C, true>(rowsum, g, t);
+  typename C::P acc = horner28<C, false>(rowsum, g, t * g.nwin);
+  if (C::poisoned(acc)) acc = horner28<C, true>(rowsum, g, t * g.nwin);
   jac<typename C::F> r = jac_inf<typename C::F>();
   if (!acc.inf) {
     r.x = C::out(acc.x);
@@ -855,6 +899,42 @@
     r.z = C::out(acc.z);
   }
   st_jac_aos<typename C::F>(out, t, r);
+}
+
+__global__ __launch_bounds__(64) void k_msm_iso_rows28(uint32_t* __restrict__ rowsum, size_t first, size_t nrows) {
+  const size_t t = gtid();
+  if (t >= nrows) return;
+  const j28 p = ldj28<c28_g1>(rowsum, first + t);
+  if (p.inf) return;
+  const jac<fp> q = iso11_jac(jac<fp>{f28_to_fp(p.x), f28_to_fp(p.y), f28_to_fp(p.z)});
+  j28 r = j28_inf();
+  if (!fp_is_zero(q.z)) r = j28{f28_from_fp(q.x), f28_from_fp(q.y), f28_from_fp(q.z), false};
+  stj28<c28_g1>(rowsum, first + t, r);
+}
+template <class C>
+__global__ __launch_bounds__(64) void k_msm_windows28_split(const uint32_t* __restrict__ rowsum, msm_geom g, size_t nsg,
+                                                            uint32_t* __restrict__ out) {
+  __shared__ uint32_t buf[lds_words<C>() * 64];
+  const size_t t = gtid(), u = t >> 1;
+  const bool half = t & 1;
+  typename C::P acc = C::inf();
+  if (u < nsg) {
+    const size_t row0 = u * msm_rows(g) + (half ? g.nwin : 0);
+    acc = horner28<C, false>(rowsum, g, row0);
+    if (C::poisoned(acc)) acc = horner28<C, true>(rowsum, g, row0);
+    if (half && !acc.inf) acc.x = C::endo_x(acc.x);
+  }
+  if (half) lds_put_pt<C>(buf, 64, threadIdx.x, acc);
+  __syncthreads();
+  if (half || u >= nsg) return;
+  acc = C::add(acc, lds_get_pt<C>(buf, 64, threadIdx.x + 1));
+  jac<typename C::F> r = jac_inf<typename C::F>();
+  if (!acc.inf) {
+    r.x = C::out(acc.x);
+    r.y = C::out(acc.y);
+    r.z = C::out(acc.z);
+  }
+  st_jac_aos<typename C::F>(out, u, r);
 }
 
 hipError_t launch_msm_prep28(int sig_g2, size_t n, uint8_t* status, const uint32_t* sig_aff, const uint32_t* q_pts,
@@ -878,7 +958,9 @@
 template <class C>
 static hipError_t msm28(const msm_geom& g, size_t ngroups, const uint32_t* S, const uint32_t* Q, msm_ws& ws, hipStream_t st,
                         const uint8_t* skip, int nsets = 2) {
-  const size_t nk = ngroups * g.nwin * (size_t)g.nbuck;
+  using CQ = typename prime_of<C>::T;
+  if (g.split && (std::is_same<C, CQ>::value || nsets != 2 || g.halves != 2)) return hipErrorInvalidValue;
+  const size_t nk = ngroups * msm_rows(g) * (size_t)g.nbuck;
   constexpr size_t jw = 3 * C::EW;
   uint32_t* bB = ws.buckets + nk * jw;
   uint32_t* pB = ws.part + msm_nchunks(ws.max_entries) * 2 * jw;
@@ -888,18 +970,23 @@
     hipLaunchKernelGGL((k_msm_bucket28<C, true>), dim3(nblk(nch, 256)), dim3(256), 0, st, ws.off, ws.list, nk, L, S, ws.buckets,
                        ws.part, ws.meta, skip, g.half_stride);
     hipLaunchKernelGGL(k_msm_bucket_fix28<C>, dim3(nblk(nch, 256)), dim3(256), 0, st, ws.off, nk, L, ws.meta, ws.part, ws.buckets);
-    if (nsets == 2) {
+    if (nsets == 2 && !g.split) {
       hipLaunchKernelGGL((k_msm_bucket28<C, true>), dim3(nblk(nch, 256)), dim3(256), 0, st, ws.off, ws.list, nk, L, Q, bB, pB,
                          ws.meta, skip, g.half_stride);
       hipLaunchKernelGGL(k_msm_bucket_fix28<C>, dim3(nblk(nch, 256)), dim3(256), 0, st, ws.off, nk, L, ws.meta, pB, bB);
+    } else if (nsets == 2) {
+      hipLaunchKernelGGL((k_msm_bucket28<CQ, true>), dim3(nblk(nch, 256)), dim3(256), 0, st, ws.off, ws.list, nk, L, Q, bB, pB,
+                         ws.meta, skip, g.half_stride);
+      hipLaunchKernelGGL(k_msm_bucket_fix28<CQ>, dim3(nblk(nch, 256)), dim3(256), 0, st, ws.off, nk, L, ws.meta, pB, bB);
     }
   }
-  const size_t rows = ngroups * g.nwin, ngw = (size_t)nsets * rows;
+  const size_t rows = ngroups * msm_rows(g), ngw = (size_t)nsets * rows;
+  const size_t prime_from = g.split ? rows : NO_PRIME;
   const unsigned sb = few_waves_block(ngw * g.nseg);
   hipLaunchKernelGGL(k_msm_segsum28<C>, dim3(nblk(ngw * g.nseg, sb)), dim3(sb), 0, st, ws.buckets, ws.off, g, ngw, rows, ws.segs,
-                     ws.runs);
+                     ws.runs, prime_from);
   if (g.nseg > 1)
-    hipLaunchKernelGGL(k_msm_segoff28<C>, dim3(nblk(ngw * g.nseg, sb)), dim3(sb), 0, st, g, ngw, ws.segs, ws.runs);
+    hipLaunchKernelGGL(k_msm_segoff28<C>, dim3(nblk(ngw * g.nseg, sb)), dim3(sb), 0, st, g, ngw, ws.segs, ws.runs, prime_from);
   uint32_t G = g.nseg <= 64 ? 1 : (ngw * g.nseg >= ((size_t)1 << 17) ? 8 : 2);
   if (G == 2 && g.nseg / 2 > 64 && (g.nseg / 2) % 64) G = 8;
   uint32_t lpr = (g.nseg + G - 1) / G, span = 64;
@@ -912,15 +999,23 @@
   const uint32_t* rowsum = ws.runs;
   if (g.nseg > 1)
     hipLaunchKernelGGL(k_msm_rowtree28<C>, dim3(nblk(ngw * lpr, few_waves_block(ngw * lpr))), dim3(few_waves_block(ngw * lpr)), 0,
-                       st, ws.segs, g.nseg, G, ngw, lpr, span, ws.runs);
+                       st, ws.segs, g.nseg, G, ngw, lpr, span, ws.runs, prime_from);
   else
     rowsum = ws.segs;
   if (lpr > 64) {
     const uint32_t parts = lpr / 64;
     uint32_t pspan = 1;
     while (pspan < parts) pspan *= 2;
-    hipLaunchKernelGGL(k_msm_rowred28<C>, dim3((unsigned)ngw), dim3(64), 0, st, ws.runs, parts, pspan, ws.segs);
+    hipLaunchKernelGGL(k_msm_rowred28<C>, dim3((unsigned)ngw), dim3(64), 0, st, ws.runs, parts, pspan, ws.segs, prime_from);
     rowsum = ws.segs;
+  }
+  if constexpr (!std::is_same<C, CQ>::value) {
+    if (g.split) {
+      hipLaunchKernelGGL(k_msm_iso_rows28, dim3(nblk(rows, 64)), dim3(64), 0, st, const_cast<uint32_t*>(rowsum), rows, rows);
+      hipLaunchKernelGGL(k_msm_windows28_split<C>, dim3(nblk(2 * nsets * ngroups, 64)), dim3(64), 0, st, rowsum, g,
+                         (size_t)nsets * ngroups, ws.out2);
+      return hipGetLastError();
+    }
   }
   hipLaunchKernelGGL(k_msm_windows28<C>, dim3(nblk(nsets * ngroups, 64)), dim3(64), 0, st, rowsum, g, nsets * ngroups, ws.out2);
   return hipGetLastError();
@@ -1013,7 +1108,7 @@
   hipLaunchKernelGGL(k_sub_bits28<C>, dim3(nblk(nlanes, blk)), dim3(blk), 0, st, ws.buckets, ws.off, g, lpp, ws.sub);
   uint32_t pspan = 1;
   while (pspan < parts) pspan *= 2;
-  hipLaunchKernelGGL(k_msm_rowred28<C>, dim3(npairs), dim3(64), 0, st, ws.sub, parts, pspan, tpts);
+  hipLaunchKernelGGL(k_msm_rowred28<C>, dim3(npairs), dim3(64), 0, st, ws.sub, parts, pspan, tpts, NO_PRIME);
   hipLaunchKernelGGL(k_sub_test28<C>, dim3(nblk(npairs, 64)), dim3(64), 0, st, tpts, npairs, pass, sub_pass);
   return hipGetLastError();
 }
diff --git a/drand_amd/csrc/k_prep.hip b/drand_amd/csrc/k_prep.hip
--- a/drand_amd/csrc/k_prep.hip
+++ b/drand_amd/csrc/k_prep.hip
@@ -210,9 +210,10 @@
   st_jac_aos<fp>(q_out, i, h2c_g1_noclear(d, dst_id));
 }
 
+template <bool LATE>
 DH_DEV void round_g1_ride(const fp& u0, const fp& u1, bool msg_ok, const uint8_t* __restrict__ s, size_t i,
                           uint8_t* __restrict__ status, uint32_t* __restrict__ sig_aff, uint8_t* __restrict__ rand_out,
-                          uint32_t* __restrict__ q_out) {
+                          uint32_t* __restrict__ q_out, uint32_t* __restrict__ s28, uint32_t* __restrict__ q28) {
   st_f<fp>(q_out + 36 * i, u0);
   st_f<fp>(q_out + 36 * i + 12, u1);
   g1_sum_mid m;
@@ -231,23 +232,50 @@
     }
     status[i] = msg_ok ? st : (uint8_t)DEC_BAD;
     st_aff_aos<fp>(sig_aff, i, a);
-  }
-  if (distinct) {
-    st_jac_aos<fp>(q_out, i, iso11_aff(g1_sum_post(m, inv_c)));
+    if constexpr (LATE) {
+      st28(s28 + 2 * W28 * i, f28_from_fp(a.x));
+      st28(s28 + 2 * W28 * i + W28, f28_from_fp(a.y));
+    }
+  }
+  if constexpr (LATE) {
+    aff<fp> q;
+    if (distinct) {
+      q = g1_sum_post(m, inv_c);
+    } else {
+      fp v0, v1;
+      ld_f<fp>(v0, q_out + 36 * i);
+      ld_f<fp>(v1, q_out + 36 * i + 12);
+      const swu_out<fp> p0 = sswu_g1(v0);
+      const fp y1 = sswu_g1(v1).y;
+      if (fp_eq(p0.y, y1)) {
+        q = e1p_dbl_aff(p0);
+      } else {
+        q = aff<fp>{fp{}, fp{}};
+        status[i] = DEC_BAD;
+      }
+    }
+    st28(q28 + 2 * W28 * i, f28_from_fp(q.x));
+    st28(q28 + 2 * W28 * i + W28, f28_from_fp(q.y));
   } else {
-    fp v0, v1;
-    ld_f<fp>(v0, q_out + 36 * i);
-    ld_f<fp>(v1, q_out + 36 * i + 12);
-    st_jac_aos<fp>(q_out, i, h2c_g1_map(v0, v1));
-  }
-}
-
+    if (distinct) {
+      st_jac_aos<fp>(q_out, i, iso11_aff(g1_sum_post(m, inv_c)));
+    } else {
+      fp v0, v1;
+      ld_f<fp>(v0, q_out + 36 * i);
+      ld_f<fp>(v1, q_out + 36 * i + 12);
+      st_jac_aos<fp>(q_out, i, h2c_g1_map(v0, v1));
+    }
+  }
+}
+
+template <bool LATE>
 __global__ __launch_bounds__(256, occ<fp>::W) void k_round_g1_ride(const uint64_t* __restrict__ rounds, const uint8_t* __restrict__ prevs,
                                                               size_t prev_stride, const uint32_t* __restrict__ prev_lens,
                                                               const uint8_t* __restrict__ msgs32, size_t n, int chained, int dst_id,
                                                               const uint8_t* __restrict__ sigs, size_t stride,
                                                               uint8_t* __restrict__ status, uint32_t* __restrict__ sig_aff,
-                                                              uint8_t* __restrict__ rand_out, uint32_t* __restrict__ q_out) {
+                                                              uint8_t* __restrict__ rand_out, uint32_t* __restrict__ q_out,
+                                                              uint32_t* __restrict__ s28, uint32_t* __restrict__ q28) {
   size_t i = gtid();
   if (i >= n) return;
   sha_h d;
@@ -256,20 +284,22 @@
   else msg_ok = beacon_digest(d, rounds, prevs, prev_stride, prev_lens, chained, i);
   uint32_t b[4][8];
   xmd32<4>(b, d, dst_id);
-  round_g1_ride(fp_from_be512(b[0], b[1]), fp_from_be512(b[2], b[3]), msg_ok, sigs + i * stride, i, status, sig_aff, rand_out,
-                q_out);
-}
-
+  round_g1_ride<LATE>(fp_from_be512(b[0], b[1]), fp_from_be512(b[2], b[3]), msg_ok, sigs + i * stride, i, status, sig_aff,
+                      rand_out, q_out, s28, q28);
+}
+
+template <bool LATE>
 __global__ __launch_bounds__(256, occ<fp>::W) void k_round_g1_ride_debug(const uint8_t* __restrict__ u, size_t n,
                                                                     const uint8_t* __restrict__ sigs, size_t stride,
                                                                     uint8_t* __restrict__ status, uint32_t* __restrict__ sig_aff,
-                                                                    uint32_t* __restrict__ q_out) {
+                                                                    uint32_t* __restrict__ q_out, uint32_t* __restrict__ s28,
+                                                                    uint32_t* __restrict__ q28) {
   size_t i = gtid();
   if (i >= n) return;
   fp u0, u1;
   be48_words(u0.v, u + 96 * i, false);
   be48_words(u1.v, u + 96 * i + 48, false);
-  round_g1_ride(fp_to_mont(u0), fp_to_mont(u1), true, sigs + i * stride, i, status, sig_aff, nullptr, q_out);
+  round_g1_ride<LATE>(fp_to_mont(u0), fp_to_mont(u1), true, sigs + i * stride, i, status, sig_aff, nullptr, q_out, s28, q28);
 }
 __global__ __launch_bounds__(64) void k_round_g1_debug_out(size_t n, const uint32_t* __restrict__ sig_aff,
                                                            const uint32_t* __restrict__ q_pts, uint8_t* __restrict__ sig_out,
@@ -284,6 +314,25 @@
   if (!jac_is_inf(q)) a = jac_to_aff(q);
   st_be48(q_out + 96 * i, fp_from_mont(a.x));
   st_be48(q_out + 96 * i + 48, fp_from_mont(a.y));
+}
+
+__global__ __launch_bounds__(64) void k_round_g1_late_debug_out(size_t n, const uint32_t* __restrict__ s28,
+                                                                const uint32_t* __restrict__ q28, uint8_t* __restrict__ sig_out,
+                                                                uint8_t* __restrict__ q_out) {
+  size_t i = gtid();
+  if (i >= n) return;
+  st_be48(sig_out + 96 * i, fp_from_mont(f28_to_fp(ld28(s28 + 2 * W28 * i))));
+  st_be48(sig_out + 96 * i + 48, fp_from_mont(f28_to_fp(ld28(s28 + 2 * W28 * i + W28))));
+  st_be48(q_out + 96 * i, fp_from_mont(f28_to_fp(ld28(q28 + 2 * W28 * i))));
+  st_be48(q_out + 96 * i + 48, fp_from_mont(f28_to_fp(ld28(q28 + 2 * W28 * i + W28))));
+}
+
+__global__ __launch_bounds__(256, occ<fp>::W) void k_iso_late_fallback(size_t n, const uint8_t* __restrict__ status,
+                                                                  const uint32_t* __restrict__ q28, uint32_t* __restrict__ q_pts) {
+  size_t i = gtid();
+  if (i >= n || status[i] != DEC_OK) return;
+  const aff<fp> q{f28_to_fp(ld28(q28 + 2 * W28 * i)), f28_to_fp(ld28(q28 + 2 * W28 * i + W28))};
+  st_jac_aos<fp>(q_pts, i, iso11_aff(q));
 }
 
 __global__ __launch_bounds__(256) void k_h2f_g2(const uint64_t* __restrict__ rounds, const uint8_t* __restrict__ prevs,
@@ -495,17 +544,45 @@
                                 const uint8_t* msgs32, size_t n, int chained, int dst_id, const uint8_t* sigs, size_t stride,
                                 uint8_t* status, uint32_t* sig_aff, uint8_t* rand_out, uint32_t* q_out, hipStream_t st) {
   if (!n) return hipSuccess;
-  hipLaunchKernelGGL(k_round_g1_ride, dim3(nblk(n, 256)), dim3(256), 0, st, rounds, prevs, prev_stride, prev_lens, msgs32, n,
-                     chained, dst_id, sigs, stride, status, sig_aff, rand_out, q_out);
+  hipLaunchKernelGGL(k_round_g1_ride<false>, dim3(nblk(n, 256)), dim3(256), 0, st, rounds, prevs, prev_stride, prev_lens, msgs32, n,
+                     chained, dst_id, sigs, stride, status, sig_aff, rand_out, q_out, (uint32_t*)nullptr, (uint32_t*)nullptr);
+  return hipGetLastError();
+}
+
+hipError_t launch_round_g1_ride_late(const uint64_t* rounds, const uint8_t* prevs, size_t prev_stride, const uint32_t* prev_lens,
+                                     const uint8_t* msgs32, size_t n, int chained, int dst_id, const uint8_t* sigs, size_t stride,
+                                     uint8_t* status, uint32_t* sig_aff, uint8_t* rand_out, uint32_t* q_out, uint32_t* s28,
+                                     uint32_t* q28, hipStream_t st) {
+  if (!n) return hipSuccess;
+  hipLaunchKernelGGL(k_round_g1_ride<true>, dim3(nblk(n, 256)), dim3(256), 0, st, rounds, prevs, prev_stride, prev_lens, msgs32, n,
+                     chained, dst_id, sigs, stride, status, sig_aff, rand_out, q_out, s28, q28);
+  return hipGetLastError();
+}
+
+hipError_t launch_iso_late_fallback(size_t n, const uint8_t* status, const uint32_t* q28, uint32_t* q_pts, hipStream_t st) {
+  if (!n) return hipSuccess;
+  hipLaunchKernelGGL(k_iso_late_fallback, dim3(nblk(n, 256)), dim3(256), 0, st, n, status, q28, q_pts);
   return hipGetLastError();
 }
 
 hipError_t launch_round_g1_ride_debug(const uint8_t* u, const uint8_t* sigs, size_t n, uint8_t* status, uint32_t* sig_aff,
                                       uint32_t* q_pts, uint8_t* sig_out, uint8_t* q_out, hipStream_t st) {
   if (!n) return hipSuccess;
-  hipLaunchKernelGGL(k_round_g1_ride_debug, dim3(nblk(n, 256)), dim3(256), 0, st, u, n, sigs, (size_t)48, status, sig_aff, q_pts);
+  hipLaunchKernelGGL(k_round_g1_ride_debug<false>, dim3(nblk(n, 256)), dim3(256), 0, st, u, n, sigs, (size_t)48, status, sig_aff,
+                     q_pts, (uint32_t*)nullptr, (uint32_t*)nullptr);
   hipLaunchKernelGGL(k_round_g1_debug_out, dim3(nblk(n, 64)), dim3(64), 0, st, n, (const uint32_t*)sig_aff,
                      (const uint32_t*)q_pts, sig_out, q_out);
+  return hipGetLastError();
+}
+
+hipError_t launch_round_g1_ride_late_debug(const uint8_t* u, const uint8_t* sigs, size_t n, uint8_t* status, uint32_t* sig_aff,
+                                           uint32_t* q_pts, uint32_t* s28, uint32_t* q28, uint8_t* sig_out, uint8_t* q_out,
+                                           hipStream_t st) {
+  if (!n) return hipSuccess;
+  hipLaunchKernelGGL(k_round_g1_ride_debug<true>, dim3(nblk(n, 256)), dim3(256), 0, st, u, n, sigs, (size_t)48, status, sig_aff,
+                     q_pts, s28, q28);
+  hipLaunchKernelGGL(k_round_g1_late_debug_out, dim3(nblk(n, 64)), dim3(64), 0, st, n, (const uint32_t*)s28, (const uint32_t*)q28,
+                     sig_out, q_out);
   return hipGetLastError();
 }
 
diff --git a/drand_amd/csrc/kcommon.hpp b/drand_amd/csrc/kcommon.hpp
--- a/drand_amd/csrc/kcommon.hpp
+++ b/drand_amd/csrc/kcommon.hpp
@@ -74,6 +74,27 @@
   uint32_t* p = base + (size_t)2 * N * i;
   st_f<F>(p, a.x);
   st_f<F>(p + N, a.y);
+}
+
+constexpr int W28 = 16;
+DH_DEV f28 ld28(const uint32_t* p) {
+  const uint4* q = (const uint4*)p;
+  f28 a;
+#pragma unroll
+  for (int i = 0; i < 4; i++) {
+    const uint4 t = q[i];
+    a.l[4 * i] = t.x;
+    a.l[4 * i + 1] = t.y;
+    if (4 * i + 2 < 14) a.l[4 * i + 2] = t.z;
+    if (4 * i + 3 < 14) a.l[4 * i + 3] = t.w;
+  }
+  return a;
+}
+DH_DEV void st28(uint32_t* p, const f28& a) {
+  uint4* q = (uint4*)p;
+#pragma unroll
+  for (int i = 0; i < 4; i++)
+    q[i] = make_uint4(a.l[4 * i], a.l[4 * i + 1], 4 * i + 2 < 14 ? a.l[4 * i + 2] : 0u, 4 * i + 3 < 14 ? a.l[4 * i + 3] : 0u);
 }
 
 DH_DEV bool jac_add_distinct_mem(jac<fp2>& r, const uint32_t* P, const uint32_t* Q) {
diff --git a/drand_amd/csrc/kernels.hpp b/drand_amd/csrc/kernels.hpp
--- a/drand_amd/csrc/kernels.hpp
+++ b/drand_amd/csrc/kernels.hpp
@@ -15,8 +15,10 @@
   uint32_t seglen;
   uint32_t halves;
   uint32_t half_stride;
+  uint32_t split = 0;
 };
 inline size_t msm_entries(const msm_geom& g, size_t m) { return m * (size_t)g.nwin * g.halves; }
+__host__ __device__ inline uint32_t msm_rows(const msm_geom& g) { return (uint32_t)g.nwin * (g.split ? g.halves : 1u); }
 
 struct msm_ws {
   uint32_t* cnt;
@@ -67,8 +69,16 @@
 hipError_t launch_round_g1_ride(const uint64_t* rounds, const uint8_t* prevs, size_t prev_stride, const uint32_t* prev_lens,
                                 const uint8_t* msgs32, size_t n, int chained, int dst_id, const uint8_t* sigs, size_t stride,
                                 uint8_t* status, uint32_t* sig_aff, uint8_t* rand_out, uint32_t* q_out, hipStream_t st);
+hipError_t launch_round_g1_ride_late(const uint64_t* rounds, const uint8_t* prevs, size_t prev_stride, const uint32_t* prev_lens,
+                                     const uint8_t* msgs32, size_t n, int chained, int dst_id, const uint8_t* sigs, size_t stride,
+                                     uint8_t* status, uint32_t* sig_aff, uint8_t* rand_out, uint32_t* q_out, uint32_t* s28,
+                                     uint32_t* q28, hipStream_t st);
+hipError_t launch_iso_late_fallback(size_t n, const uint8_t* status, const uint32_t* q28, uint32_t* q_pts, hipStream_t st);
 hipError_t launch_round_g1_ride_debug(const uint8_t* u, const uint8_t* sigs, size_t n, uint8_t* status, uint32_t* sig_aff,
                                       uint32_t* q_pts, uint8_t* sig_out, uint8_t* q_out, hipStream_t st);
+hipError_t launch_round_g1_ride_late_debug(const uint8_t* u, const uint8_t* sigs, size_t n, uint8_t* status, uint32_t* sig_aff,
+                                           uint32_t* q_pts, uint32_t* s28, uint32_t* q28, uint8_t* sig_out, uint8_t* q_out,
+                                           hipStream_t st);
 hipError_t launch_hash_var(int sig_g2, const uint8_t* msgs, const uint32_t* msg_off, size_t n, int dst_id, uint32_t* q_out,
                            uint32_t* tmp, hipStream_t st);
 hipError_t launch_scalars(const uint32_t* seed_words, size_t n, const uint8_t* status, uint4* scal, int parts, hipStream_t st);
diff --git a/include/drandhip.h b/include/drandhip.h
--- a/include/drandhip.h
+++ b/include/drandhip.h
@@ -125,6 +125,9 @@
 int dh_g1_round_prep_debug(const uint8_t* us, const uint8_t* sigs, size_t n, uint8_t* status_out, uint8_t* sig_out,
                            uint8_t* hash_out);
 
+int dh_g1_round_prep_late_debug(const uint8_t* us, const uint8_t* sigs, size_t n, uint8_t* status_out, uint8_t* sig_out,
+                                uint8_t* hash_out);
+
 int dh_profile(int enable);
 int dh_profile_read(char* buf, size_t cap);
 
```
